# Chris10M/Lip2Speech

Measured on AMD Instinct MI355X. Metric: mel-frames/sec at LRW batch=32, 29-frame clips (Lip2Speech.inference, S=300), higher is better.
Workload: dtype f32; 1 GPU; LRW single-word, batch=32 per step, 29x96x96 RGB mouth crops, S=300 decode steps, speaker embedding supplied (encoding=voice), random-init weights; every step is one full pass over one B=32 batch; frames=29, decode_steps=300, library=libl2s_hip.so, parallelism=dp1 (clip sharding, no collective), batches_per_launch_chain=8, launch_chains_in_flight_per_gpu=3, distinct_batches_per_gpu=24, ranks=1

## Files before the change

### lip2speech_amd/csrc/encoder_kernels.hip

```cpp
#include "l2s_common.h"
#include <type_traits>

namespace l2s {

constexpr int FE_PR = 6;
constexpr int FE_CR = 2 * FE_PR + 1;
constexpr int FE_XROWS = 2 * (FE_CR - 1) + 7 + 1;
constexpr int FE_XLD = 104;
constexpr int FE_KP = 50;
constexpr int FE_CO = 24;

template <int HW, int MODE>
__global__ __launch_bounds__(256, 3) void frontend3d_kernel(const FrontendW w, const FrameSrc vsrc,
                                                            int T, float* __restrict__ out, float* __restrict__ zout) {
    constexpr bool SAVE_Z = MODE == 1;
    constexpr int H = HW, W = HW, Hc = H / 2, Wc = W / 2, Hp = Hc / 2, Wp = Wc / 2;
    constexpr int P = FE_CR * Wc;
    constexpr int NT = (P + 31) / 32;
    constexpr int TPW = (NT + 3) / 4;
    constexpr int XS = FE_XROWS * FE_XLD;
    constexpr int WS = FE_KP * 32;
    constexpr int CS = MODE == 2 ? 0 : P * (FE_CO / 2);
    constexpr int SMEM = (XS + WS) > CS ? (XS + WS) : CS;
    __shared__ __attribute__((aligned(16))) float smem[SMEM];
// ... 493 lines not shown
                        if ((nt == 0 && !on0) || (nt == 2 && !on1)) continue;
                        f32x4 a = acc[j][nt];
                        a = __builtin_amdgcn_mfma_f32_16x16x32_bf16(al, bh[nt], a, 0, 0, 0);
                        a = __builtin_amdgcn_mfma_f32_16x16x32_bf16(ah, bl[nt], a, 0, 0, 0);
                        a = __builtin_amdgcn_mfma_f32_16x16x32_bf16(am, bm[nt], a, 0, 0, 0);
                        a = __builtin_amdgcn_mfma_f32_16x16x32_bf16(am, bh[nt], a, 0, 0, 0);
                        a = __builtin_amdgcn_mfma_f32_16x16x32_bf16(ah, bm[nt], a, 0, 0, 0);
                        a = __builtin_amdgcn_mfma_f32_16x16x32_bf16(ah, bh[nt], a, 0, 0, 0);
                        acc[j][nt] = a;
                    }
                }
            }
        }
        sl = nxt; ++nslab;
    }
    __syncthreads();

    float* Cs = reinterpret_cast<float*>(smem);
    constexpr int CH = FE_CO / 2;
    float sc[3], sh[3], slp[3];
#pragma unroll
    for (int nt = 0; nt < 3; ++nt) {
        const int q = nt * 16 + li, ch = q >= FE_CO ? q - FE_CO : q;
        sc[nt] = w.scale[ch]; sh[nt] = w.shift[ch]; slp[nt] = w.slope[ch];
    }
    for (int pass = 0; pass < (has1 ? 4 : 2); ++pass) {
        const int o = pass >> 1, half = pass & 1;
#pragma unroll
        for (int nt = 0; nt < 3; ++nt) {
            const int q = nt * 16 + li, qo = q >= FE_CO ? 1 : 0, ch = q - FE_CO * qo;
            if (qo == o && ch >= half * CH && ch < (half + 1) * CH) {
#pragma unroll
                for (int j = 0; j < TPW; ++j) {
                    if (wave + 4 * j < PT) {
#pragma unroll
                        for (int r = 0; r < 4; ++r) {
                            const int p = (wave + 4 * j) * 16 + 4 * kg + r;
                            if (p < P) {
                                float v = acc[j][nt][r] * sc[nt] + sh[nt];
                                v = v >= 0.f ? v : slp[nt] * v;
                                Cs[p * CH + (ch - half * CH)] = v;
                            }
                        }
                    }
                }
            }
        }
        __syncthreads();
        const int f = bg * T + t0 + o;
        for (int i = tid; i < FE_PR * Wp * CH; i += 256) {
            const int ch = i % CH;
            const int pw = (i / CH) % Wp;
            const int prl = i / (CH * Wp);
            const int pr = p0 + prl;
            if (pr >= Hp) continue;
            float m = -INFINITY;
#pragma unroll
            for (int dr = 0; dr < 3; ++dr) {
                const int crow = 2 * pr - 1 + dr;
                if (crow < 0 || crow >= Hc) continue;
                const int lrow = 2 * prl + dr;
#pragma unroll
                for (int dc = -1; dc <= 1; ++dc) {
                    const int cc = 2 * pw + dc;
                    if (cc < 0 || cc >= Wc) continue;
                    m = fmaxf(m, Cs[(lrow * Wc + cc) * CH + ch]);
                }
            }
            out[(((int64_t)f * Hp + pr) * Wp + pw) * FE_CO + half * CH + ch] = m;
        }
        __syncthreads();
    }
}

template <int HW>
__global__ __launch_bounds__(256, 2) void frontend3d_x3q_kernel(const FrontendW w, const FrameSrc vsrc, int T, float* __restrict__ out) {
    const int NPAIR = (T + 1) / 2;
    const int bg = blockIdx.y / NPAIR, t0 = 2 * (blockIdx.y - bg * NPAIR);
    const bool has1 = t0 + 1 < T;
    const int grp = bg / vsrc.per, b = bg - grp * vsrc.per;
    const float* __restrict__ video = vsrc.p[grp];
#define FE_X3Q_PITCH T
#define FE_X3Q_FRAME0 (bg * T)
#include "frontend_x3q_block.inc"
#undef FE_X3Q_PITCH
#undef FE_X3Q_FRAME0
}

template <int HW>
__global__ __launch_bounds__(256, 2) void frontend3d_x3q_ragged_kernel(const FrontendW w, const FrameSrc vsrc, const RaggedClip* __restrict__ clips,
                                                                       const int* __restrict__ pair_clip, float* __restrict__ out) {
    const RaggedClip k = clips[pair_clip[blockIdx.y]];
    const int T = k.len;
    const int t0 = 2 * ((int)blockIdx.y - k.pair0);
    const bool has1 = t0 + 1 < T;
    const int b = k.row;
    const float* __restrict__ video = vsrc.p[0];
#pragma unroll
    for (int g = 1; g < MAX_GROUP; ++g) video = k.g == g ? vsrc.p[g] : video;
#define FE_X3Q_PITCH k.T
#define FE_X3Q_FRAME0 k.frame0
#include "frontend_x3q_block.inc"
#undef FE_X3Q_PITCH
#undef FE_X3Q_FRAME0
}

int launch_frontend(const FrontendW& w, const FrameSrc& video, int B, int T, int H, int W, float* out, hipStream_t s, float* zout) {
    L2S_REQUIRE(H == W && (H == 96 || H == 88), "frontend supports 96x96 and 88x88 mouth crops");
    L2S_REQUIRE(video.per >= 1 && (B + video.per - 1) / video.per <= MAX_GROUP, "too many frame tensors in one launch");
    for (int g = 0; g < (B + video.per - 1) / video.per; ++g)
        L2S_REQUIRE(video.p[g] && (reinterpret_cast<uintptr_t>(video.p[g]) & 15u) == 0, "video must be non-null and 16-byte aligned");
    const int Hp = H / 4;
    dim3 grid((Hp + FE_PR - 1) / FE_PR, B * T);
    ProfScope ps("frontend3d_conv_bn_prelu_pool", s);
    if (!zout && w.w1) {
        if (H == 96) hipLaunchKernelGGL((frontend3d_x3_kernel<96, 1>), grid, dim3(256), 0, s, w, video, T, out);
        else hipLaunchKernelGGL((frontend3d_x3_kernel<88, 1>), grid, dim3(256), 0, s, w, video, T, out);
    } else if (!zout && w.w3 && w.pair) {
        dim3 gp((Hp + FE_PR - 1) / FE_PR, B * ((T + 1) / 2));
        if (w.pipe) {
            const unsigned pad = w.solo ? 4096u : 0u;
            if (H == 96) hipLaunchKernelGGL((frontend3d_x3q_kernel<96>), gp, dim3(256), pad, s, w, video, T, out);
            else hipLaunchKernelGGL((frontend3d_x3q_kernel<88>), gp, dim3(256), pad, s, w, video, T, out);
        } else if (H == 96) hipLaunchKernelGGL((frontend3d_x3p_kernel<96>), gp, dim3(256), 0, s, w, video, T, out);
        else hipLaunchKernelGGL((frontend3d_x3p_kernel<88>), gp, dim3(256), 0, s, w, video, T, out);
    } else if (!zout && w.w3) {
        if (H == 96) hipLaunchKernelGGL((frontend3d_x3_kernel<96, 3>), grid, dim3(256), 0, s, w, video, T, out);
        else hipLaunchKernelGGL((frontend3d_x3_kernel<88, 3>), grid, dim3(256), 0, s, w, video, T, out);
    } else if (zout) {
        if (H == 96) hipLaunchKernelGGL((frontend3d_kernel<96, 1>), grid, dim3(256), 0, s, w, video, T, out, zout);
        else hipLaunchKernelGGL((frontend3d_kernel<88, 1>), grid, dim3(256), 0, s, w, video, T, out, zout);
    } else {
        if (H == 96) hipLaunchKernelGGL((frontend3d_kernel<96, 0>), grid, dim3(256), 0, s, w, video, T, out, zout);
        else hipLaunchKernelGGL((frontend3d_kernel<88, 0>), grid, dim3(256), 0, s, w, video, T, out, zout);
    }
    L2S_CHECK_HIP(hipGetLastError());
    return 0;
}

int launch_frontend_ragged(const FrontendW& w, const FrameSrc& video, const RaggedTab& rg, int H, int W, float* out, hipStream_t s) {
    L2S_REQUIRE(H == W && (H == 96 || H == 88), "frontend supports 96x96 and 88x88 mouth crops");
    L2S_REQUIRE(w.w3 && !w.w1 && w.pair && w.pipe && !w.solo, "the ragged front-end exists in the default form only (frontend_x3 = 3, no infer_bf16)");
    L2S_REQUIRE(rg.clips && rg.pair_clip && rg.NP >= 1 && rg.NF >= 1, "ragged front-end: empty table");
    const int Hp = H / 4;
    dim3 gp((Hp + FE_PR - 1) / FE_PR, rg.NP);
    prof_count("frontend3d_ragged_pair_blocks", rg.NP);
    ProfScope ps("frontend3d_conv_bn_prelu_pool_ragged", s);
    if (H == 96) hipLaunchKernelGGL((frontend3d_x3q_ragged_kernel<96>), gp, dim3(256), 0, s, w, video, rg.clips, rg.pair_clip, out);
    else hipLaunchKernelGGL((frontend3d_x3q_ragged_kernel<88>), gp, dim3(256), 0, s, w, video, rg.clips, rg.pair_clip, out);
    L2S_CHECK_HIP(hipGetLastError());
    return 0;
}

__global__ __launch_bounds__(256) void frontend_pool_kernel(const float* __restrict__ z, const float* __restrict__ slope, int NF, int Hc, int Wc, float* __restrict__ out) {
    const int Hp = Hc / 2, Wp = Wc / 2;
    const unsigned total = (unsigned)NF * Hp * Wp * FE_CO;
    for (unsigned idx = blockIdx.x * 256u + threadIdx.x; idx < total; idx += gridDim.x * 256u) {
        const int ch = idx % FE_CO;
        unsigned r = idx / FE_CO;
        const int pw = r % Wp; r /= Wp;
        const int pr = r % Hp;
        const unsigned f = r / Hp;
        const float sl = slope[ch];
        float m = -INFINITY;
#pragma unroll
        for (int dr = -1; dr <= 1; ++dr) {
            const int crow = 2 * pr + dr;
            if (crow < 0 || crow >= Hc) continue;
#pragma unroll
            for (int dc = -1; dc <= 1; ++dc) {
                const int cc = 2 * pw + dc;
                if (cc < 0 || cc >= Wc) continue;
                float v = z[((size_t)(f * Hc + crow) * Wc + cc) * FE_CO + ch];
                v = v >= 0.f ? v : sl * v;
                m = fmaxf(m, v);
            }
        }
        out[idx] = m;
    }
}
int launch_frontend_pool(const float* z, const float* slope, int NF, int Hc, int Wc, float* out, hipStream_t s) {
    const int64_t total = (int64_t)NF * (Hc / 2) * (Wc / 2) * FE_CO;
    L2S_REQUIRE(total < (int64_t)1 << 31, "front-end pool: map too large for 32-bit indexing");
    ProfScope ps("train_frontend_prelu_pool", s);
    hipLaunchKernelGGL(frontend_pool_kernel, dim3((unsigned)std::min<int64_t>((total + 255) / 256, 16384)), dim3(256), 0, s, z, slope, NF, Hc, Wc, out);
    L2S_CHECK_HIP(hipGetLastError());
    return 0;
}

int launch_frontend_stats(const FrontendW& w, const float* video1, int B, int T, int H, int W, float* partials, int* nblocks, hipStream_t s, float* raw_out) {
    L2S_REQUIRE(H == W && (H == 96 || H == 88), "frontend supports 96x96 and 88x88 mouth crops");
    FrameSrc video{}; video.p[0] = video1; video.per = B;
    const int Hp = H / 4;
    dim3 grid((Hp + FE_PR - 1) / FE_PR, B * T);
    *nblocks = (int)(grid.x * grid.y);
    ProfScope ps("train_frontend3d_stats", s);
    if (H == 96) hipLaunchKernelGGL((frontend3d_kernel<96, 2>), grid, dim3(256), 0, s, w, video, T, raw_out, partials);
    else hipLaunchKernelGGL((frontend3d_kernel<88, 2>), grid, dim3(256), 0, s, w, video, T, raw_out, partials);
    L2S_CHECK_HIP(hipGetLastError());
    return 0;
}

struct ClipTab { int64_t off[MAX_COLLATE_CLIPS]; int frames[MAX_COLLATE_CLIPS]; };

__global__ __launch_bounds__(256) void normalise_pad_kernel(const uint8_t* __restrict__ packed, const ClipTab tab, int b0, int T, int HW4,
                                                            float* __restrict__ video) {
    const int q = blockIdx.x * 256 + threadIdx.x, t = blockIdx.y, bl = blockIdx.z;
    if (q >= HW4) return;
    const int b = b0 + bl;
    const int64_t plane = (int64_t)HW4 * 4;
    float* out = video + (((int64_t)b * 3) * T + t) * plane + (int64_t)q * 4;
    float4 r = make_float4(0.f, 0.f, 0.f, 0.f), g = r, bl4 = r;
    if (t < tab.frames[bl]) {
        const uint32_t* src = reinterpret_cast<const uint32_t*>(packed + tab.off[bl] + ((int64_t)t * plane + (int64_t)q * 4) * 3);
        const uint32_t w0 = src[0], w1 = src[1], w2 = src[2];
        const float mean[3] = {0.485f, 0.456f, 0.406f}, stdv[3] = {0.229f, 0.224f, 0.225f};
        auto nrm = [&](uint32_t byte, int c) { return __fdiv_rn(__fsub_rn(__fdiv_rn((float)byte, 255.0f), mean[c]), stdv[c]); };
        r = make_float4(nrm(w0 & 255u, 0), nrm(w0 >> 24, 0), nrm((w1 >> 16) & 255u, 0), nrm((w2 >> 8) & 255u, 0));
        g = make_float4(nrm((w0 >> 8) & 255u, 1), nrm(w1 & 255u, 1), nrm(w1 >> 24, 1), nrm((w2 >> 16) & 255u, 1));
        bl4 = make_float4(nrm((w0 >> 16) & 255u, 2), nrm((w1 >> 8) & 255u, 2), nrm(w2 & 255u, 2), nrm(w2 >> 24, 2));
    }
    *reinterpret_cast<float4*>(out) = r;
    *reinterpret_cast<float4*>(out + (int64_t)T * plane) = g;
    *reinterpret_cast<float4*>(out + 2 * (int64_t)T * plane) = bl4;
}

int launch_normalise_pad(const uint8_t* packed, const int64_t* offsets, const int* frames, int B, int T, int H, int W, float* video, hipStream_t s) {
    L2S_REQUIRE((H * W) % 4 == 0 && (reinterpret_cast<uintptr_t>(packed) & 3u) == 0 && (reinterpret_cast<uintptr_t>(video) & 15u) == 0,
                "frames: H*W must be a multiple of 4, buffers aligned");
    const int HW4 = H * W / 4;
    ProfScope ps("normalise_pad_frames", s);
    for (int b0 = 0; b0 < B; b0 += MAX_COLLATE_CLIPS) {
        const int nb = B - b0 < MAX_COLLATE_CLIPS ? B - b0 : MAX_COLLATE_CLIPS;
        ClipTab tab{};
        for (int i = 0; i < nb; ++i) {
            L2S_REQUIRE(frames[b0 + i] >= 0 && frames[b0 + i] <= T && offsets[b0 + i] % 4 == 0, "clip table: 0 <= frames <= T, 4-byte aligned offsets");
            tab.off[i] = offsets[b0 + i]; tab.frames[i] = frames[b0 + i];
        }
        hipLaunchKernelGGL(normalise_pad_kernel, dim3((HW4 + 255) / 256, T, nb), dim3(256), 0, s, packed, tab, b0, T, HW4, video);
    }
    L2S_CHECK_HIP(hipGetLastError());
    return 0;
}

__global__ __launch_bounds__(256) void dwconv3x3_kernel(const float* __restrict__ in, int N, int Hi, int Wi, int ldi,
                                                        int ci_off, int C, int stride, const float* __restrict__ w9,
                                                        const float* __restrict__ scale, const float* __restrict__ shift,
                                                        float* __restrict__ out, int Ho, int Wo, int ldo, int co_off) {
    const int64_t total = (int64_t)N * Ho * Wo * C;
    for (int64_t idx = (int64_t)blockIdx.x * 256 + threadIdx.x; idx < total; idx += (int64_t)gridDim.x * 256) {
        const int c = idx % C;
        int64_t r = idx / C;
        const int ow = r % Wo;
        r /= Wo;
        const int oh = r % Ho;
        const int n = r / Ho;
        float acc = 0.f;
#pragma unroll
        for (int kh = 0; kh < 3; ++kh) {
            const int ih = oh * stride + kh - 1;
            if (ih < 0 || ih >= Hi) continue;
#pragma unroll
            for (int kw = 0; kw < 3; ++kw) {
                const int iw = ow * stride + kw - 1;
                if (iw < 0 || iw >= Wi) continue;
                acc = fmaf(in[(((int64_t)n * Hi + ih) * Wi + iw) * ldi + ci_off + c], w9[(kh * 3 + kw) * C + c], acc);
            }
        }
        out[(((int64_t)n * Ho + oh) * Wo + ow) * ldo + co_off + c] = acc * scale[c] + shift[c];
    }
}

int launch_dwconv(const float* in, int N, int Hi, int Wi, int ldi, int ci_off, int C, int stride, const float* w9,
                  const float* scale, const float* shift, float* out, int ldo, int co_off, hipStream_t s) {
    const int Ho = (Hi + 2 - 3) / stride + 1, Wo = (Wi + 2 - 3) / stride + 1;
    const int64_t total = (int64_t)N * Ho * Wo * C;
    int blocks = (int)((total + 255) / 256);
    if (blocks > 8192) blocks = 8192;
    ProfScope ps("dwconv3x3_bn", s);
    hipLaunchKernelGGL(dwconv3x3_kernel, dim3(blocks), dim3(256), 0, s, in, N, Hi, Wi, ldi, ci_off, C, stride, w9, scale,
                       shift, out, Ho, Wo, ldo, co_off);
    L2S_CHECK_HIP(hipGetLastError());
    return 0;
}


__device__ __forceinline__ f32x4 su_mfma4(const float4& a, const float4& w, f32x4 acc) {
    acc = __builtin_amdgcn_mfma_f32_16x16x4f32(a.x, w.x, acc, 0, 0, 0);
    acc = __builtin_amdgcn_mfma_f32_16x16x4f32(a.y, w.y, acc, 0, 0, 0);
    acc = __builtin_amdgcn_mfma_f32_16x16x4f32(a.z, w.z, acc, 0, 0, 0);
    acc = __builtin_amdgcn_mfma_f32_16x16x4f32(a.w, w.w, acc, 0, 0, 0);
    return acc;
}

constexpr int su_pad16(int v) { return (v + 15) / 16 * 16; }
constexpr int su_group(int mt) { return (mt + (mt + 4) / 5 - 1) / ((mt + 4) / 5); }

template <int N_, int NC_, int MT_>
struct SuGemm {
    static constexpr int N = N_, NC = NC_, MT = MT_, G = su_group(MT_);
    static constexpr int NT = (N + 15) / 16, MG = (MT + G - 1) / G, ITEMS = NT * MG, IT = (ITEMS + 7) / 8;
};

template <class GM, int LDA>
__device__ __forceinline__ void su_gemm(float* __restrict__ buf, const float* __restrict__ Wf,
                                        const float* __restrict__ scale, const float* __restrict__ shift) {
    constexpr int NC = GM::NC, G = GM::G, IT = GM::IT, NT = GM::NT;
    const int lane = threadIdx.x & 63;
    const int wave = __builtin_amdgcn_readfirstlane(threadIdx.x >> 6);
    const int li = lane & 15, lg = lane >> 4;
    f32x4 acc[IT][G];
#pragma unroll
    for (int it = 0; it < IT; ++it) {
        const int item = wave + 8 * it;
#pragma unroll
        for (int j = 0; j < G; ++j) acc[it][j] = {0.f, 0.f, 0.f, 0.f};
        if (item < GM::ITEMS) {
            const int nt = item % NT, mg = item / NT;
            const int mt0 = min(mg * G, GM::MT - G);
            const float4* wb = reinterpret_cast<const float4*>(Wf) + nt * (NC * 64) + lane;
            const float* ab = buf + (mt0 * 16 + li) * LDA + 4 * lg;
            float4 b4[NC];
#pragma unroll
            for (int c = 0; c < NC; ++c) b4[c] = wb[c * 64];
#pragma unroll
            for (int c = 0; c < NC; ++c) {
#pragma unroll
                for (int j = 0; j < G; ++j) {
                    const float4 a4 = *reinterpret_cast<const float4*>(ab + j * 16 * LDA + 16 * c);
                    acc[it][j] = su_mfma4(a4, b4[c], acc[it][j]);
                }
                __builtin_amdgcn_sched_barrier(0);
            }
        }
    }
    __syncthreads();
#pragma unroll
    for (int it = 0; it < IT; ++it) {
        const int item = wave + 8 * it;
        if (item < GM::ITEMS) {
            const int nt = item % NT, mg = item / NT;
            const int mt0 = min(mg * G, GM::MT - G);
            const int n = nt * 16 + li;
            if (n < GM::N) {
                const float sc = scale[n], sh = shift[n];
#pragma unroll
                for (int j = 0; j < G; ++j) {
#pragma unroll
                    for (int r = 0; r < 4; ++r) {
                        const float v = acc[it][j][r] * sc + sh;
                        buf[((mt0 + j) * 16 + 4 * lg + r) * LDA + n] = v > 0.f ? v : 0.f;
                    }
                }
            }
        }
    }
    __syncthreads();
}

template <int H, int HALF, int F>
struct S1Geo {
    static constexpr int HH = H * H, C = 2 * HALF, KP = su_pad16(HALF), LDA = KP + 4, PX = F * HH;
    static constexpr int MT = (PX + 15) / 16, ROWS = MT * 16, PPW = (PX + 7) / 8, CIT = (C + 63) / 64, CH = (HALF + 63) / 64;
    using GM = SuGemm<HALF, KP / 16, MT>;
    static constexpr size_t SMEM = (size_t)ROWS * LDA * sizeof(float);
};

#ifdef L2S_DIAG
static unsigned long long* g_su_ts = nullptr;
static int g_su_ts_h = 0;
void shuffle_set_timeline(unsigned long long* ts, int h) { g_su_ts = ts; g_su_ts_h = h; }
#endif
#define SU_STAMP(k) do { if (TIMED && threadIdx.x == 0) ts[blockIdx.x * 10 + (k)] = wall_clock64(); } while (0)

template <int H, int HALF, int F, bool TIMED>
__global__ __launch_bounds__(512, 4) void shuffle_s1_kernel(const ShuffleS1P p, unsigned long long* __restrict__ ts) {
    using Q = S1Geo<H, HALF, F>;
    constexpr int HH = Q::HH, C = Q::C, KP = Q::KP, LDA = Q::LDA, ROWS = Q::ROWS, PPW = Q::PPW, CIT = Q::CIT;
    extern __shared__ __attribute__((aligned(16))) float su_smem[];
    const int tid = threadIdx.x, lane = tid & 63;
    const int wave = __builtin_amdgcn_readfirstlane(tid >> 6);
    SU_STAMP(0);
    const int f0 = blockIdx.x * F;
    const int Mv = min(F, p.NF - f0) * HH;
    float* buf = su_smem;
    const float* xb = p.x + (int64_t)f0 * HH * C;
    float* ob = p.out + (int64_t)f0 * HH * C;

    const __amdgpu_buffer_rsrc_t rsrc = __builtin_amdgcn_make_buffer_rsrc(const_cast<float*>(xb), 0, Mv * C * 4, 0x00020000);
    int voff[CIT];
#pragma unroll
    for (int j = 0; j < CIT; ++j) voff[j] = (lane + 64 * j < C) ? (lane + 64 * j) * 4 : 0x7ffffff0;
    float xr[PPW][CIT];
#pragma unroll
    for (int i = 0; i < PPW; ++i) {
        const int soff = (wave + 8 * i) * C * 4;
#pragma unroll
        for (int j = 0; j < CIT; ++j)
            xr[i][j] = __builtin_bit_cast(float, __builtin_amdgcn_raw_buffer_load_b32(rsrc, voff[j], soff, 0));
    }
    if (KP > HALF) {
        for (int idx = tid; idx < ROWS * (KP - HALF); idx += 512) {
            const int m = idx / (KP - HALF), k = HALF + idx - m * (KP - HALF);
            buf[m * LDA + k] = 0.f;
        }
    }
    for (int idx = tid; idx < (ROWS - Mv) * HALF; idx += 512) {
        const int m = Mv + idx / HALF, k = idx - (m - Mv) * HALF;
        buf[m * LDA + k] = 0.f;
    }
#pragma unroll
    for (int i = 0; i < PPW; ++i) {
        const int m = wave + 8 * i;
#pragma unroll
        for (int j = 0; j < CIT; ++j) {
            const int c = lane + 64 * j;
            if (m < Mv && c >= HALF && c < C) buf[m * LDA + (c - HALF)] = xr[i][j];
        }
    }
    SU_STAMP(1);
    __syncthreads();
    SU_STAMP(2);
    su_gemm<typename Q::GM, LDA>(buf, p.w1f, p.s1, p.b1);
    SU_STAMP(3);
    constexpr bool PAIRS = HALF > 64;
    constexpr int NROW = F * H, RPW = (NROW + 7) / 8;
    typedef float su_f2 __attribute__((ext_vector_type(2)));
    using DV = std::conditional_t<PAIRS, su_f2, float>;
    constexpr int DW = PAIRS ? 2 : 1;
    constexpr int CHD = (HALF + 64 * DW - 1) / (64 * DW);
    DV dv[CHD][RPW][H];
    const DV zero = DV{};
#pragma unroll
    for (int jc = 0; jc < CHD; ++jc) {
        const int c = min(DW * lane + 64 * DW * jc, HALF - DW);
        DV wk[9];
#pragma unroll
        for (int t = 0; t < 9; ++t) wk[t] = *reinterpret_cast<const DV*>(p.wd + t * HALF + c);
        const DV sd = *reinterpret_cast<const DV*>(p.sd + c), bd = *reinterpret_cast<const DV*>(p.bd + c);
#pragma unroll
        for (int r = 0; r < RPW; ++r) {
            const int R = wave + 8 * r;
            if (R * H < Mv) {
                const int y = R % H;
                const bool up = y > 0, dn = y < H - 1;
                const float* rm = buf + (R * H) * LDA + c;
                const float* ru = rm - (up ? H * LDA : 0);
                const float* rd = rm + (dn ? H * LDA : 0);
                DV wu[3], wdn[3];
#pragma unroll
                for (int k = 0; k < 3; ++k) { wu[k] = up ? wk[k] : zero; wdn[k] = dn ? wk[6 + k] : zero; }
                DV a0 = zero, a1 = zero, a2 = zero;
                DV b0 = *reinterpret_cast<const DV*>(ru), b1 = *reinterpret_cast<const DV*>(rm), b2 = *reinterpret_cast<const DV*>(rd);
                DV c0 = zero, c1 = zero, c2 = zero;
                if constexpr (H > 1) { c0 = *reinterpret_cast<const DV*>(ru + LDA); c1 = *reinterpret_cast<const DV*>(rm + LDA); c2 = *reinterpret_cast<const DV*>(rd + LDA); }
#pragma unroll
                for (int x = 0; x < H; ++x) {
                    DV acc = zero;
                    if (x > 0) acc = __builtin_elementwise_fma(a0, wu[0], acc);
                    acc = __builtin_elementwise_fma(b0, wu[1], acc);
                    if (x < H - 1) acc = __builtin_elementwise_fma(c0, wu[2], acc);
                    if (x > 0) acc = __builtin_elementwise_fma(a1, wk[3], acc);
                    acc = __builtin_elementwise_fma(b1, wk[4], acc);
                    if (x < H - 1) acc = __builtin_elementwise_fma(c1, wk[5], acc);
                    if (x > 0) acc = __builtin_elementwise_fma(a2, wdn[0], acc);
                    acc = __builtin_elementwise_fma(b2, wdn[1], acc);
                    if (x < H - 1) acc = __builtin_elementwise_fma(c2, wdn[2], acc);
                    dv[jc][r][x] = acc * sd + bd;
                    a0 = b0; a1 = b1; a2 = b2; b0 = c0; b1 = c1; b2 = c2;
                    if (x + 2 < H) {
                        c0 = *reinterpret_cast<const DV*>(ru + (x + 2) * LDA); c1 = *reinterpret_cast<const DV*>(rm + (x + 2) * LDA);
                        c2 = *reinterpret_cast<const DV*>(rd + (x + 2) * LDA);
                    }
                }
            }
        }
    }
    SU_STAMP(4);
    __syncthreads();
#pragma unroll
    for (int jc = 0; jc < CHD; ++jc) {
        const int c = DW * lane + 64 * DW * jc;
#pragma unroll
        for (int r = 0; r < RPW; ++r) {
            const int R = wave + 8 * r;
            if (R * H < Mv && c < HALF) {
#pragma unroll
                for (int x = 0; x < H; ++x) *reinterpret_cast<DV*>(buf + (R * H + x) * LDA + c) = dv[jc][r][x];
            }
        }
    }
    __syncthreads();
    SU_STAMP(5);
    su_gemm<typename Q::GM, LDA>(buf, p.w2f, p.s2, p.b2);
    SU_STAMP(6);
#pragma unroll
    for (int i = 0; i < PPW; ++i) {
        const int m = wave + 8 * i;
#pragma unroll
        for (int j = 0; j < CIT; ++j) {
            const int c = lane + 64 * j;
            if (m < Mv && c < HALF) {
                float2 o;
                o.x = xr[i][j];
                o.y = buf[m * LDA + c];
                *reinterpret_cast<float2*>(ob + (int64_t)m * C + 2 * c) = o;
            }
        }
    }
    if (TIMED) {
        __builtin_amdgcn_s_waitcnt(0);
        SU_STAMP(7);
        unsigned hw;
        asm volatile("s_getreg_b32 %0, hwreg(HW_REG_HW_ID)" : "=s"(hw));
        unsigned xcc;
        asm volatile("s_getreg_b32 %0, hwreg(HW_REG_XCC_ID)" : "=s"(xcc));
        if (threadIdx.x == 0) { ts[blockIdx.x * 10 + 8] = hw; ts[blockIdx.x * 10 + 9] = xcc; }
    }
}

template <int H, int HALF, int F>
static int launch_s1_inst(const ShuffleS1P& p, hipStream_t s) {
    using Q = S1Geo<H, HALF, F>;
    static_assert(Q::SMEM <= 80 * 1024, "two blocks per CU");
    static bool attr_set = false;
    if (!attr_set) {
        L2S_CHECK_HIP(hipFuncSetAttribute(reinterpret_cast<const void*>(shuffle_s1_kernel<H, HALF, F, false>),
                                          hipFuncAttributeMaxDynamicSharedMemorySize, (int)Q::SMEM));
#ifdef L2S_DIAG
        L2S_CHECK_HIP(hipFuncSetAttribute(reinterpret_cast<const void*>(shuffle_s1_kernel<H, HALF, F, true>),
                                          hipFuncAttributeMaxDynamicSharedMemorySize, (int)Q::SMEM));
#endif
        attr_set = true;
    }
#ifdef L2S_DIAG
    if (g_su_ts && g_su_ts_h == H) hipLaunchKernelGGL((shuffle_s1_kernel<H, HALF, F, true>), dim3((p.NF + F - 1) / F), dim3(512), Q::SMEM, s, p, g_su_ts);
    else
#endif
    hipLaunchKernelGGL((shuffle_s1_kernel<H, HALF, F, false>), dim3((p.NF + F - 1) / F), dim3(512), Q::SMEM, s, p, (unsigned long long*)nullptr);
    return 0;
}

typedef __bf16 su_bf16x8 __attribute__((ext_vector_type(8)));
constexpr int su_pad32(int v) { return (v + 31) / 32 * 32; }
constexpr int su_pitch(int kp32) { return kp32 * 2 + 32; }
__device__ __forceinline__ void su_split2(float a, float b, unsigned& hi, unsigned& mid, unsigned& lo) {
    const unsigned xa = __float_as_uint(a), xb = __float_as_uint(b);
    const float ra = a - __uint_as_float(xa & 0xFFFF0000u), rb = b - __uint_as_float(xb & 0xFFFF0000u);
    const float qa = ra - __uint_as_float(__float_as_uint(ra) & 0xFFFF0000u), qb = rb - __uint_as_float(__float_as_uint(rb) & 0xFFFF0000u);
    hi = __builtin_amdgcn_perm(xb, xa, 0x07060302u);
    mid = __builtin_amdgcn_perm(__float_as_uint(rb), __float_as_uint(ra), 0x07060302u);
    lo = __builtin_amdgcn_perm(__float_as_uint(qb), __float_as_uint(qa), 0x07060302u);
}

__global__ __launch_bounds__(256) void su_planes_kernel(const float* __restrict__ W, int N, int K, int NT, int NCH, uint4* __restrict__ out) {
    const int idx = blockIdx.x * 256 + threadIdx.x;
    if (idx >= NT * NCH * 64) return;
    const int lane = idx & 63, ch = (idx >> 6) % NCH, nt = (idx >> 6) / NCH;
    const int n = nt * 16 + (lane & 15), k0 = ch * 32 + 8 * (lane >> 4);
    unsigned h[4], m[4], l[4];
#pragma unroll
    for (int e = 0; e < 4; ++e) {
        const int k = k0 + 2 * e;
        const float a = (n < N && k < K) ? W[(int64_t)n * K + k] : 0.f, b = (n < N && k + 1 < K) ? W[(int64_t)n * K + k + 1] : 0.f;
        su_split2(a, b, h[e], m[e], l[e]);
    }
    uint4* o = out + ((int64_t)(nt * NCH + ch) * 3) * 64 + lane;
    o[0] = make_uint4(h[0], h[1], h[2], h[3]);
    o[64] = make_uint4(m[0], m[1], m[2], m[3]);
    o[128] = make_uint4(l[0], l[1], l[2], l[3]);
}
int64_t su_planes_bytes(int N, int K) { return (int64_t)((N + 15) / 16) * (su_pad32(K) / 32) * 3 * 1024; }
int launch_su_planes(const float* W, int N, int K, void* out, hipStream_t s) {
    const int NT = (N + 15) / 16, NCH = su_pad32(K) / 32;
    ProfScope ps("shuffle_unit_weight_planes", s);
    hipLaunchKernelGGL(su_planes_kernel, dim3((NT * NCH * 64 + 255) / 256), dim3(256), 0, s, W, N, K, NT, NCH, reinterpret_cast<uint4*>(out));
    L2S_CHECK_HIP(hipGetLastError());
    return 0;
}

template <class GM, int NCH, int PITCH, int PLANE, int LDA, bool OPQ = false>
__device__ __forceinline__ void su_gemm_x3(unsigned char* __restrict__ pl, const uint4* __restrict__ Wp,
                                           const float* __restrict__ scale, const float* __restrict__ shift, int mrows = 1 << 30) {
    constexpr int G = GM::G, IT = GM::IT, NT = GM::NT, BD = NCH <= 4 ? NCH : 3;
    int tx = threadIdx.x;
    if constexpr (OPQ) asm volatile("" : "+v"(tx));
    const int lane = tx & 63;
    const int wave = __builtin_amdgcn_readfirstlane(threadIdx.x >> 6);
    const int li = lane & 15, lg = lane >> 4;
    float* const buf = reinterpret_cast<float*>(pl);
    f32x4 acc[IT][G];
#pragma unroll
    for (int it = 0; it < IT; ++it) {
        const int item = wave + 8 * it;
#pragma unroll
        for (int j = 0; j < G; ++j) acc[it][j] = {0.f, 0.f, 0.f, 0.f};
        if (item < GM::ITEMS) {
            const int nt = item % NT, mg = item / NT;
            const int mt0 = min(mg * G, GM::MT - G);
            const uint4* wb = Wp + (int64_t)nt * NCH * 192 + lane;
            const unsigned char* ab = pl + (mt0 * 16 + li) * PITCH + 16 * lg;
            uint4 b[BD][3];
#pragma unroll
            for (int c = 0; c < BD; ++c) {
#pragma unroll
                for (int q = 0; q < 3; ++q) b[c][q] = wb[(c * 3 + q) * 64];
            }
#pragma unroll
            for (int c = 0; c < NCH; ++c) {
                const int sl = c % BD;
                const su_bf16x8 bh = __builtin_bit_cast(su_bf16x8, b[sl][0]), bm = __builtin_bit_cast(su_bf16x8, b[sl][1]), bl = __builtin_bit_cast(su_bf16x8, b[sl][2]);
#pragma unroll
                for (int j = 0; j < G; ++j) {
                    const unsigned char* ap = ab + j * 16 * PITCH + 64 * c;
                    const su_bf16x8 ah = *reinterpret_cast<const su_bf16x8*>(ap), am = *reinterpret_cast<const su_bf16x8*>(ap + PLANE),
                                    al = *reinterpret_cast<const su_bf16x8*>(ap + 2 * PLANE);
                    f32x4 a = acc[it][j];
                    a = __builtin_amdgcn_mfma_f32_16x16x32_bf16(al, bh, a, 0, 0, 0);
                    a = __builtin_amdgcn_mfma_f32_16x16x32_bf16(ah, bl, a, 0, 0, 0);
                    a = __builtin_amdgcn_mfma_f32_16x16x32_bf16(am, bm, a, 0, 0, 0);
                    a = __builtin_amdgcn_mfma_f32_16x16x32_bf16(am, bh, a, 0, 0, 0);
                    a = __builtin_amdgcn_mfma_f32_16x16x32_bf16(ah, bm, a, 0, 0, 0);
                    a = __builtin_amdgcn_mfma_f32_16x16x32_bf16(ah, bh, a, 0, 0, 0);
                    acc[it][j] = a;
                }
                __builtin_amdgcn_sched_barrier(0);
                if (c + BD < NCH) {
#pragma unroll
                    for (int q = 0; q < 3; ++q) b[sl][q] = wb[((c + BD) * 3 + q) * 64];
                }
            }
        }
    }
    __syncthreads();
#pragma unroll
    for (int it = 0; it < IT; ++it) {
        const int item = wave + 8 * it;
        if (item < GM::ITEMS) {
            const int nt = item % NT, mg = item / NT;
            const int mt0 = min(mg * G, GM::MT - G);
            const int n = nt * 16 + li;
            if (n < GM::N) {
                const float sc = scale[n], sh = shift[n];
#pragma unroll
                for (int j = 0; j < G; ++j) {
#pragma unroll
                    for (int r = 0; r < 4; ++r) {
                        const float v = acc[it][j][r] * sc + sh;
                        const int row = (mt0 + j) * 16 + 4 * lg + r;
                        if (row < mrows) buf[row * LDA + n] = v > 0.f ? v : 0.f;
                    }
                }
            }
        }
    }
    __syncthreads();
}

template <int H, int HALF, int F>
struct S1XGeo {
    static constexpr int HH = H * H, C = 2 * HALF, KP = su_pad16(HALF), LDA = KP + 4, PX = F * HH;
    static constexpr int MT = (PX + 15) / 16, ROWS = MT * 16;
    static constexpr int KP32 = su_pad32(HALF), NCH = KP32 / 32, PITCH = su_pitch(KP32), PLANE = ROWS * PITCH;
    static constexpr int NPAIR = HALF / 2, KPAIR = KP32 / 2;
    static constexpr int PPI = KPAIR <= 32 ? 2 : 1;
    static constexpr int QIT = PPI == 2 ? 1 : KPAIR / 64, PPW = (PX + 8 * PPI - 1) / (8 * PPI);
    using GM = SuGemm<HALF, KP / 16, MT>;
    static constexpr size_t SMEM = 3 * (size_t)PLANE > (size_t)ROWS * LDA * 4 ? 3 * (size_t)PLANE : (size_t)ROWS * LDA * 4;
    static_assert(HALF % 2 == 0 && (PPI == 2 || KPAIR % 64 == 0), "channel pairs; a pixel's pairs fill whole wave instructions");
};

template <int H, int HALF, int F, bool TIMED>
__global__ __launch_bounds__(512, 4) void shuffle_s1x_kernel(const ShuffleS1P p, unsigned long long* __restrict__ ts) {
    using Q = S1XGeo<H, HALF, F>;
    constexpr int HH = Q::HH, C = Q::C, LDA = Q::LDA, PPW = Q::PPW, QIT = Q::QIT, PPI = Q::PPI, PITCH = Q::PITCH, PLANE = Q::PLANE;
    extern __shared__ __attribute__((aligned(16))) float su_smem[];
    const int tid = threadIdx.x, lane = tid & 63;
    const int wave = __builtin_amdgcn_readfirstlane(tid >> 6);
    SU_STAMP(0);
    const int f0 = blockIdx.x * F;
    const int Mv = min(F, p.NF - f0) * HH;
    float* buf = su_smem;
    unsigned char* const pl = reinterpret_cast<unsigned char*>(su_smem);
    const float* xb = p.x + (int64_t)f0 * HH * C;
    float* ob = p.out + (int64_t)f0 * HH * C;

    const __amdgpu_buffer_rsrc_t rsrc = __builtin_amdgcn_make_buffer_rsrc(const_cast<float*>(xb), 0, Mv * C * 4, 0x00020000);
    const int sub = PPI == 2 ? lane >> 5 : 0;
    typedef unsigned su_u2 __attribute__((ext_vector_type(2)));
    float2 xr[PPW][QIT];
    su_u2 br[PPW][QIT];
#pragma unroll
    for (int i = 0; i < PPW; ++i) {
        const int soff = (wave + 8 * i) * PPI * C * 4;
#pragma unroll
        for (int j = 0; j < QIT; ++j) {
            const int q = PPI == 2 ? (lane & 31) : lane + 64 * j;
            const int voff = q < Q::NPAIR ? (sub * C + 2 * q) * 4 : 0x7ffffff0;
            const su_u2 a = __builtin_amdgcn_raw_buffer_load_b64(rsrc, voff, soff, 0);
            br[i][j] = __builtin_amdgcn_raw_buffer_load_b64(rsrc, q < Q::NPAIR ? voff + HALF * 4 : 0x7ffffff0, soff, 0);
            xr[i][j] = make_float2(__uint_as_float(a.x), __uint_as_float(a.y));
        }
    }
#pragma unroll
    for (int i = 0; i < PPW; ++i) {
        const int m = (wave + 8 * i) * PPI + sub;
#pragma unroll
        for (int j = 0; j < QIT; ++j) {
            const int q = PPI == 2 ? (lane & 31) : lane + 64 * j;
            unsigned hi, mid, lo;
            su_split2(__uint_as_float(br[i][j].x), __uint_as_float(br[i][j].y), hi, mid, lo);
            if (m < Q::ROWS) {
                unsigned* d = reinterpret_cast<unsigned*>(pl + m * PITCH + q * 4);
                d[0] = hi; d[PLANE / 4] = mid; d[2 * (PLANE / 4)] = lo;
            }
        }
    }
    SU_STAMP(1);
    __syncthreads();
    SU_STAMP(2);
    su_gemm_x3<typename Q::GM, Q::NCH, PITCH, PLANE, LDA>(pl, reinterpret_cast<const uint4*>(p.w1p), p.s1, p.b1);
    SU_STAMP(3);
    constexpr bool PAIRS = HALF > 64;
    constexpr int NROW = F * H, RPW = (NROW + 7) / 8;
    typedef float su_f2 __attribute__((ext_vector_type(2)));
    using DV = std::conditional_t<PAIRS, su_f2, float>;
    constexpr int DW = PAIRS ? 2 : 1;
    constexpr int CHD = Q::KP32 / (64 * DW);
    DV dv[CHD][RPW][H];
    const DV zero = DV{};
#pragma unroll
    for (int jc = 0; jc < CHD; ++jc) {
        const int c = min(DW * lane + 64 * DW * jc, HALF - DW);
        DV wk[9];
#pragma unroll
        for (int t = 0; t < 9; ++t) wk[t] = *reinterpret_cast<const DV*>(p.wd + t * HALF + c);
        const DV sd = *reinterpret_cast<const DV*>(p.sd + c), bd = *reinterpret_cast<const DV*>(p.bd + c);
#pragma unroll
        for (int r = 0; r < RPW; ++r) {
            const int R = wave + 8 * r;
            if (R * H < Mv) {
                const int y = R % H;
                const bool up = y > 0, dn = y < H - 1;
                const float* rm = buf + (R * H) * LDA + c;
                const float* ru = rm - (up ? H * LDA : 0);
                const float* rd = rm + (dn ? H * LDA : 0);
                DV wu[3], wdn[3];
#pragma unroll
                for (int k = 0; k < 3; ++k) { wu[k] = up ? wk[k] : zero; wdn[k] = dn ? wk[6 + k] : zero; }
                DV a0 = zero, a1 = zero, a2 = zero;
                DV b0 = *reinterpret_cast<const DV*>(ru), b1 = *reinterpret_cast<const DV*>(rm), b2 = *reinterpret_cast<const DV*>(rd);
                DV c0 = zero, c1 = zero, c2 = zero;
                if constexpr (H > 1) { c0 = *reinterpret_cast<const DV*>(ru + LDA); c1 = *reinterpret_cast<const DV*>(rm + LDA); c2 = *reinterpret_cast<const DV*>(rd + LDA); }
#pragma unroll
                for (int x = 0; x < H; ++x) {
                    DV acc = zero;
                    if (x > 0) acc = __builtin_elementwise_fma(a0, wu[0], acc);
                    acc = __builtin_elementwise_fma(b0, wu[1], acc);
                    if (x < H - 1) acc = __builtin_elementwise_fma(c0, wu[2], acc);
                    if (x > 0) acc = __builtin_elementwise_fma(a1, wk[3], acc);
                    acc = __builtin_elementwise_fma(b1, wk[4], acc);
                    if (x < H - 1) acc = __builtin_elementwise_fma(c1, wk[5], acc);
                    if (x > 0) acc = __builtin_elementwise_fma(a2, wdn[0], acc);
                    acc = __builtin_elementwise_fma(b2, wdn[1], acc);
                    if (x < H - 1) acc = __builtin_elementwise_fma(c2, wdn[2], acc);
                    dv[jc][r][x] = acc * sd + bd;
                    a0 = b0; a1 = b1; a2 = b2; b0 = c0; b1 = c1; b2 = c2;
                    if (x + 2 < H) {
                        c0 = *reinterpret_cast<const DV*>(ru + (x + 2) * LDA); c1 = *reinterpret_cast<const DV*>(rm + (x + 2) * LDA);
                        c2 = *reinterpret_cast<const DV*>(rd + (x + 2) * LDA);
                    }
                }
            }
        }
    }
    SU_STAMP(4);
    __syncthreads();
#pragma unroll
    for (int jc = 0; jc < CHD; ++jc) {
        const int c = DW * lane + 64 * DW * jc;
#pragma unroll
        for (int r = 0; r < RPW; ++r) {
            const int R = wave + 8 * r;
            if (R * H < Mv) {
#pragma unroll
                for (int x = 0; x < H; ++x) {
                    unsigned char* d = pl + (R * H + x) * PITCH + c * 2;
                    if constexpr (PAIRS) {
                        unsigned hi, mid, lo;
                        su_split2(c < HALF ? dv[jc][r][x][0] : 0.f, c < HALF ? dv[jc][r][x][1] : 0.f, hi, mid, lo);
                        *reinterpret_cast<unsigned*>(d) = hi; *reinterpret_cast<unsigned*>(d + PLANE) = mid; *reinterpret_cast<unsigned*>(d + 2 * PLANE) = lo;
                    } else {
                        const float v = c < HALF ? dv[jc][r][x] : 0.f;
                        const float r1 = v - __uint_as_float(__float_as_uint(v) & 0xFFFF0000u);
                        const float r2 = r1 - __uint_as_float(__float_as_uint(r1) & 0xFFFF0000u);
                        *reinterpret_cast<unsigned short*>(d) = (unsigned short)(__float_as_uint(v) >> 16);
                        *reinterpret_cast<unsigned short*>(d + PLANE) = (unsigned short)(__float_as_uint(r1) >> 16);
                        *reinterpret_cast<unsigned short*>(d + 2 * PLANE) = (unsigned short)(__float_as_uint(r2) >> 16);
                    }
                }
            }
        }
    }
    __syncthreads();
    SU_STAMP(5);
    su_gemm_x3<typename Q::GM, Q::NCH, PITCH, PLANE, LDA>(pl, reinterpret_cast<const uint4*>(p.w2p), p.s2, p.b2);
    SU_STAMP(6);
#pragma unroll
    for (int i = 0; i < PPW; ++i) {
        const int m = (wave + 8 * i) * PPI + sub;
#pragma unroll
        for (int j = 0; j < QIT; ++j) {
            const int q = PPI == 2 ? (lane & 31) : lane + 64 * j;
            if (m < Mv && q < Q::NPAIR) {
                const float2 bv = *reinterpret_cast<const float2*>(buf + m * LDA + 2 * q);
                *reinterpret_cast<float4*>(ob + (int64_t)m * C + 4 * q) = make_float4(xr[i][j].x, bv.x, xr[i][j].y, bv.y);
            }
        }
    }
    if (TIMED) {
        __builtin_amdgcn_s_waitcnt(0);
        SU_STAMP(7);
        unsigned hw;
        asm volatile("s_getreg_b32 %0, hwreg(HW_REG_HW_ID)" : "=s"(hw));
        unsigned xcc;
        asm volatile("s_getreg_b32 %0, hwreg(HW_REG_XCC_ID)" : "=s"(xcc));
        if (threadIdx.x == 0) { ts[blockIdx.x * 10 + 8] = hw; ts[blockIdx.x * 10 + 9] = xcc; }
    }
}

template <int H, int HALF, int F>
static int launch_s1x_inst(const ShuffleS1P& p, hipStream_t s) {
    using Q = S1XGeo<H, HALF, F>;
    static_assert(Q::SMEM <= 80 * 1024, "two blocks per CU");
    static bool attr_set = false;
    if (!attr_set) {
        L2S_CHECK_HIP(hipFuncSetAttribute(reinterpret_cast<const void*>(shuffle_s1x_kernel<H, HALF, F, false>),
                                          hipFuncAttributeMaxDynamicSharedMemorySize, (int)Q::SMEM));
#ifdef L2S_DIAG
        L2S_CHECK_HIP(hipFuncSetAttribute(reinterpret_cast<const void*>(shuffle_s1x_kernel<H, HALF, F, true>),
                                          hipFuncAttributeMaxDynamicSharedMemorySize, (int)Q::SMEM));
#endif
        attr_set = true;
    }
#ifdef L2S_DIAG
    if (g_su_ts && g_su_ts_h == H) hipLaunchKernelGGL((shuffle_s1x_kernel<H, HALF, F, true>), dim3((p.NF + F - 1) / F), dim3(512), Q::SMEM, s, p, g_su_ts);
    else
#endif
    hipLaunchKernelGGL((shuffle_s1x_kernel<H, HALF, F, false>), dim3((p.NF + F - 1) / F), dim3(512), Q::SMEM, s, p, (unsigned long long*)nullptr);
    return 0;
}

struct S1UnitW {
    const void* w1p; const float* s1; const float* b1;
    const float* wd; const float* sd; const float* bd;
    const void* w2p; const float* s2; const float* b2;
};
struct ShuffleS1ChainP {
    const float* x; float* out;
    int NF, n;
    S1UnitW u[S1_CHAIN_MAX];
};

template <int H, int HALF, int F>
__global__ __launch_bounds__(512, 4) void shuffle_s1xc_kernel(const ShuffleS1ChainP p) {
    using Q = S1XGeo<H, HALF, F>;
    constexpr int HH = Q::HH, C = Q::C, LDA = Q::LDA, PPW = Q::PPW, QIT = Q::QIT, PPI = Q::PPI, PITCH = Q::PITCH, PLANE = Q::PLANE;
    static_assert(HALF % 2 == 0 && (Q::KPAIR - Q::NPAIR) <= 32, "a lane's four output channels are two whole pairs; the K padding is at most 32 pairs");
    extern __shared__ __attribute__((aligned(16))) float su_smem[];
    const int tid = threadIdx.x, lane = tid & 63;
    const int wave = __builtin_amdgcn_readfirstlane(tid >> 6);
    const int f0 = blockIdx.x * F;
    const int Mv = min(F, p.NF - f0) * HH;
    float* buf = su_smem;
    unsigned char* const pl = reinterpret_cast<unsigned char*>(su_smem);
    const float* xb = p.x + (int64_t)f0 * HH * C;
    float* ob = p.out + (int64_t)f0 * HH * C;
    const int nu = p.n;

    const __amdgpu_buffer_rsrc_t rsrc = __builtin_amdgcn_make_buffer_rsrc(const_cast<float*>(xb), 0, Mv * C * 4, 0x00020000);
    const int sub = PPI == 2 ? lane >> 5 : 0;
    typedef unsigned su_u2 __attribute__((ext_vector_type(2)));
    float2 xr[PPW][QIT];
    {
        su_u2 br[PPW][QIT];
#pragma unroll
        for (int i = 0; i < PPW; ++i) {
            const int soff = (wave + 8 * i) * PPI * C * 4;
#pragma unroll
            for (int j = 0; j < QIT; ++j) {
                const int q = PPI == 2 ? (lane & 31) : lane + 64 * j;
                const int voff = q < Q::NPAIR ? (sub * C + 2 * q) * 4 : 0x7ffffff0;
                const su_u2 a = __builtin_amdgcn_raw_buffer_load_b64(rsrc, voff, soff, 0);
                br[i][j] = __builtin_amdgcn_raw_buffer_load_b64(rsrc, q < Q::NPAIR ? voff + HALF * 4 : 0x7ffffff0, soff, 0);
                xr[i][j] = make_float2(__uint_as_float(a.x), __uint_as_float(a.y));
            }
        }
#pragma unroll
        for (int i = 0; i < PPW; ++i) {
            const int m = (wave + 8 * i) * PPI + sub;
#pragma unroll
            for (int j = 0; j < QIT; ++j) {
                const int q = PPI == 2 ? (lane & 31) : lane + 64 * j;
                unsigned hi, mid, lo;
                su_split2(__uint_as_float(br[i][j].x), __uint_as_float(br[i][j].y), hi, mid, lo);
                if (m < Q::ROWS) {
                    unsigned* d = reinterpret_cast<unsigned*>(pl + m * PITCH + q * 4);
                    d[0] = hi; d[PLANE / 4] = mid; d[2 * (PLANE / 4)] = lo;
                }
            }
        }
    }
    __syncthreads();

    for (int u = 0; u < nu; ++u) {
        const S1UnitW& U = p.u[u];
        const void* const w1p = U.w1p; const float* const s1 = U.s1; const float* const b1 = U.b1;
        const float* const wd = U.wd; const float* const sdp = U.sd; const float* const bdp = U.bd;
        const void* const w2p = U.w2p; const float* const s2 = U.s2; const float* const b2 = U.b2;
        su_gemm_x3<typename Q::GM, Q::NCH, PITCH, PLANE, LDA, true>(pl, reinterpret_cast<const uint4*>(w1p), s1, b1);
        {
            constexpr bool PAIRS = HALF > 64;
            constexpr int NROW = F * H, RPW = (NROW + 7) / 8;
            typedef float su_f2 __attribute__((ext_vector_type(2)));
            using DV = std::conditional_t<PAIRS, su_f2, float>;
            constexpr int DW = PAIRS ? 2 : 1;
            constexpr int CHD = Q::KP32 / (64 * DW);
            DV dv[CHD][RPW][H];
            const DV zero = DV{};
            int lane_d = lane;
            asm volatile("" : "+v"(lane_d));
#pragma unroll
            for (int jc = 0; jc < CHD; ++jc) {
                const int c = min(DW * lane_d + 64 * DW * jc, HALF - DW);
                DV wk[9];
#pragma unroll
                for (int t = 0; t < 9; ++t) wk[t] = *reinterpret_cast<const DV*>(wd + t * HALF + c);
                const DV sd = *reinterpret_cast<const DV*>(sdp + c), bd = *reinterpret_cast<const DV*>(bdp + c);
#pragma unroll
                for (int r = 0; r < RPW; ++r) {
                    const int R = wave + 8 * r;
                    if (R * H < Mv) {
                        const int y = R % H;
                        const bool up = y > 0, dn = y < H - 1;
                        const float* rm = buf + (R * H) * LDA + c;
                        const float* ru = rm - (up ? H * LDA : 0);
                        const float* rd = rm + (dn ? H * LDA : 0);
                        DV wu[3], wdn[3];
#pragma unroll
                        for (int k = 0; k < 3; ++k) { wu[k] = up ? wk[k] : zero; wdn[k] = dn ? wk[6 + k] : zero; }
                        DV a0 = zero, a1 = zero, a2 = zero;
                        DV b0 = *reinterpret_cast<const DV*>(ru), b1v = *reinterpret_cast<const DV*>(rm), b2v = *reinterpret_cast<const DV*>(rd);
                        DV c0 = zero, c1 = zero, c2 = zero;
                        if constexpr (H > 1) { c0 = *reinterpret_cast<const DV*>(ru + LDA); c1 = *reinterpret_cast<const DV*>(rm + LDA); c2 = *reinterpret_cast<const DV*>(rd + LDA); }
#pragma unroll
                        for (int x = 0; x < H; ++x) {
                            DV acc = zero;
                            if (x > 0) acc = __builtin_elementwise_fma(a0, wu[0], acc);
                            acc = __builtin_elementwise_fma(b0, wu[1], acc);
                            if (x < H - 1) acc = __builtin_elementwise_fma(c0, wu[2], acc);
                            if (x > 0) acc = __builtin_elementwise_fma(a1, wk[3], acc);
                            acc = __builtin_elementwise_fma(b1v, wk[4], acc);
                            if (x < H - 1) acc = __builtin_elementwise_fma(c1, wk[5], acc);
                            if (x > 0) acc = __builtin_elementwise_fma(a2, wdn[0], acc);
                            acc = __builtin_elementwise_fma(b2v, wdn[1], acc);
                            if (x < H - 1) acc = __builtin_elementwise_fma(c2, wdn[2], acc);
                            dv[jc][r][x] = acc * sd + bd;
                            a0 = b0; a1 = b1v; a2 = b2v; b0 = c0; b1v = c1; b2v = c2;
                            if (x + 2 < H) {
                                c0 = *reinterpret_cast<const DV*>(ru + (x + 2) * LDA); c1 = *reinterpret_cast<const DV*>(rm + (x + 2) * LDA);
                                c2 = *reinterpret_cast<const DV*>(rd + (x + 2) * LDA);
                            }
                        }
                    }
                }
            }
            __syncthreads();
#pragma unroll
            for (int jc = 0; jc < CHD; ++jc) {
                const int c = DW * lane_d + 64 * DW * jc;
#pragma unroll
                for (int r = 0; r < RPW; ++r) {
                    const int R = wave + 8 * r;
                    if (R * H < Mv) {
#pragma unroll
                        for (int x = 0; x < H; ++x) {
                            unsigned char* d = pl + (R * H + x) * PITCH + c * 2;
                            if constexpr (PAIRS) {
                                unsigned hi, mid, lo;
                                su_split2(c < HALF ? dv[jc][r][x][0] : 0.f, c < HALF ? dv[jc][r][x][1] : 0.f, hi, mid, lo);
                                *reinterpret_cast<unsigned*>(d) = hi; *reinterpret_cast<unsigned*>(d + PLANE) = mid; *reinterpret_cast<unsigned*>(d + 2 * PLANE) = lo;
                            } else {
                                const float v = c < HALF ? dv[jc][r][x] : 0.f;
                                const float r1 = v - __uint_as_float(__float_as_uint(v) & 0xFFFF0000u);
                                const float r2 = r1 - __uint_as_float(__float_as_uint(r1) & 0xFFFF0000u);
                                *reinterpret_cast<unsigned short*>(d) = (unsigned short)(__float_as_uint(v) >> 16);
                                *reinterpret_cast<unsigned short*>(d + PLANE) = (unsigned short)(__float_as_uint(r1) >> 16);
                                *reinterpret_cast<unsigned short*>(d + 2 * PLANE) = (unsigned short)(__float_as_uint(r2) >> 16);
                            }
                        }
                    }
                }
            }
            __syncthreads();
        }
        su_gemm_x3<typename Q::GM, Q::NCH, PITCH, PLANE, LDA, true>(pl, reinterpret_cast<const uint4*>(w2p), s2, b2);
        if (u + 1 == nu) {
#pragma unroll
            for (int i = 0; i < PPW; ++i) {
                const int m = (wave + 8 * i) * PPI + sub;
#pragma unroll
                for (int j = 0; j < QIT; ++j) {
                    const int q = PPI == 2 ? (lane & 31) : lane + 64 * j;
                    if (m < Mv && q < Q::NPAIR) {
                        const float2 bv = *reinterpret_cast<const float2*>(buf + m * LDA + 2 * q);
                        *reinterpret_cast<float4*>(ob + (int64_t)m * C + 4 * q) = make_float4(xr[i][j].x, bv.x, xr[i][j].y, bv.y);
                    }
                }
            }
        } else {
            int lane_v = lane;
            asm volatile("" : "+v"(lane_v));
            const int sub_v = PPI == 2 ? lane_v >> 5 : 0;
            float2 bv[PPW][QIT];
#pragma unroll
            for (int i = 0; i < PPW; ++i) {
                const int m = (wave + 8 * i) * PPI + sub_v;
#pragma unroll
                for (int j = 0; j < QIT; ++j) {
                    const int q = PPI == 2 ? (lane_v & 31) : lane_v + 64 * j;
                    bv[i][j] = make_float2(0.f, 0.f);
                    if (m < Q::ROWS && q < Q::NPAIR) bv[i][j] = *reinterpret_cast<const float2*>(buf + m * LDA + 2 * q);
                }
            }
            __syncthreads();
#pragma unroll
            for (int i = 0; i < PPW; ++i) {
                const int m = (wave + 8 * i) * PPI + sub_v;
#pragma unroll
                for (int j = 0; j < QIT; ++j) {
                    const int q = PPI == 2 ? (lane_v & 31) : lane_v + 64 * j;
                    if (m < Q::ROWS && q < Q::NPAIR) {
#pragma unroll
                        for (int e = 0; e < 2; ++e) {
                            const int c = 4 * q + 2 * e;
                            if (c >= HALF) {
                                unsigned hi, mid, lo;
                                su_split2(e ? xr[i][j].y : xr[i][j].x, e ? bv[i][j].y : bv[i][j].x, hi, mid, lo);
                                unsigned* d = reinterpret_cast<unsigned*>(pl + m * PITCH + (c - HALF) * 2);
                                d[0] = hi; d[PLANE / 4] = mid; d[2 * (PLANE / 4)] = lo;
                            }
                        }
                    }
                    if (j == 0 && m < Q::ROWS && q < Q::KPAIR - Q::NPAIR) {
                        unsigned* d = reinterpret_cast<unsigned*>(pl + m * PITCH + (Q::NPAIR + q) * 4);
                        d[0] = 0u; d[PLANE / 4] = 0u; d[2 * (PLANE / 4)] = 0u;
                    }
                }
                float2 nx[QIT];
#pragma unroll
                for (int j = 0; j < QIT; ++j) {
                    const int q = PPI == 2 ? (lane_v & 31) : lane_v + 64 * j;
                    const int srcq = q >> 1;
                    const int src = PPI == 2 ? ((lane_v & 32) | srcq) : srcq;
                    const float ex = __shfl(xr[i][0].x, src), ey = __shfl(bv[i][0].x, src), ez = __shfl(xr[i][0].y, src), ew = __shfl(bv[i][0].y, src);
                    nx[j] = (q & 1) ? make_float2(ez, ew) : make_float2(ex, ey);
                }
#pragma unroll
                for (int j = 0; j < QIT; ++j) xr[i][j] = nx[j];
            }
            __syncthreads();
        }
    }
}

template <int H, int HALF, int F>
static int launch_s1xc_inst(const ShuffleS1ChainP& p, hipStream_t s) {
    using Q = S1XGeo<H, HALF, F>;
    static_assert(Q::SMEM <= 80 * 1024, "two blocks per CU");
    static bool attr_set = false;
    if (!attr_set) {
        L2S_CHECK_HIP(hipFuncSetAttribute(reinterpret_cast<const void*>(shuffle_s1xc_kernel<H, HALF, F>), hipFuncAttributeMaxDynamicSharedMemorySize, (int)Q::SMEM));
        attr_set = true;
    }
    hipLaunchKernelGGL((shuffle_s1xc_kernel<H, HALF, F>), dim3((p.NF + F - 1) / F), dim3(512), Q::SMEM, s, p);
    return 0;
}

int launch_shuffle_s1_chain(const ShuffleS1P* units, int n, hipStream_t s) {
    L2S_REQUIRE(n >= 1 && n <= S1_CHAIN_MAX, "shuffle_s1 chain: 1..7 units");
    ShuffleS1ChainP c{};
    c.x = units[0].x; c.out = units[n - 1].out; c.NF = units[0].NF; c.n = n;
    const int h = units[0].h, half = units[0].half;
    for (int i = 0; i < n; ++i) {
        const ShuffleS1P& p = units[i];
        L2S_REQUIRE(p.w1p && p.w2p && p.h == h && p.half == half && p.NF == c.NF && p.Kpad == su_pad16(p.half), "shuffle_s1 chain: units of one stage with operand planes");
        c.u[i] = S1UnitW{p.w1p, p.s1, p.b1, p.wd, p.sd, p.bd, p.w2p, p.s2, p.b2};
    }
    ProfScope ps(h >= 11 ? "shuffle_stage_s1_chain_h12" : h == 6 ? "shuffle_stage_s1_chain_h6" : "shuffle_stage_s1_chain_h3", s);
    int rc = 1;
    if (h == 12 && half == 58) rc = launch_s1xc_inst<12, 58, 1>(c, s);
    else if (h == 11 && half == 58) rc = launch_s1xc_inst<11, 58, 1>(c, s);
    else if (h == 6 && half == 116) rc = launch_s1xc_inst<6, 116, 2>(c, s);
    else if (h == 3 && half == 232) rc = c.NF >= 2048 ? launch_s1xc_inst<3, 232, 5>(c, s) : launch_s1xc_inst<3, 232, 2>(c, s);
    else set_error("shuffle_s1 chain: unsupported unit geometry");
    if (rc) return 1;
    L2S_CHECK_HIP(hipGetLastError());
    return 0;
}

int launch_shuffle_s1(const ShuffleS1P& p, hipStream_t s) {
    L2S_REQUIRE(p.Kpad == su_pad16(p.half), "shuffle_s1: weight fragments are packed for K = pad16(half)");
    ProfScope ps(p.h >= 11 ? "shuffle_unit_s1_fused_h12" : p.h == 6 ? "shuffle_unit_s1_fused_h6" : "shuffle_unit_s1_fused_h3", s);
    int rc = 1;
    if (p.w1p && p.w2p) {
        if (p.h == 12 && p.half == 58) rc = launch_s1x_inst<12, 58, 1>(p, s);
        else if (p.h == 11 && p.half == 58) rc = launch_s1x_inst<11, 58, 1>(p, s);
        else if (p.h == 6 && p.half == 116) rc = launch_s1x_inst<6, 116, 2>(p, s);
        else if (p.h == 3 && p.half == 232) rc = p.NF >= 2048 ? launch_s1x_inst<3, 232, 5>(p, s) : launch_s1x_inst<3, 232, 2>(p, s);
        else set_error("shuffle_s1: unsupported unit geometry");
    }
    else if (p.h == 12 && p.half == 58) rc = launch_s1_inst<12, 58, 1>(p, s);
    else if (p.h == 11 && p.half == 58) rc = launch_s1_inst<11, 58, 1>(p, s);
    else if (p.h == 6 && p.half == 116) rc = launch_s1_inst<6, 116, 2>(p, s);
    else if (p.h == 3 && p.half == 232) rc = p.NF >= 2048 ? launch_s1_inst<3, 232, 5>(p, s) : launch_s1_inst<3, 232, 2>(p, s);
    else set_error("shuffle_s1: unsupported unit geometry");
    if (rc) return 1;
    L2S_CHECK_HIP(hipGetLastError());
    return 0;
}

template <int H, int CIN, int HALF, int RO>
struct S2Geo {
    static constexpr int HO = (H + 1) / 2, KIN = su_pad16(CIN), KH = su_pad16(HALF), LDA = (KIN > KH ? KIN : KH) + 4;
    static constexpr int RIN = 2 * RO + 1, MTI = (RIN * H + 15) / 16, MTO = (RO * HO + 15) / 16, STRIPS = (HO + RO - 1) / RO;
    using G1 = SuGemm<HALF, KIN / 16, MTI>;
    using G2 = SuGemm<HALF, KIN / 16, MTO>;
    using G3 = SuGemm<HALF, KH / 16, MTO>;
    static constexpr size_t SMEM = (size_t)(MTI + 2 * MTO) * 16 * LDA * sizeof(float);
    static_assert(CIN % 4 == 0 && CIN <= HALF, "float4 tile rows; pw1 runs in place over the input tile");
};

template <int H, int HO, int LDA, int CN, int PITCH = 0, int PLANE = 0>
__device__ __forceinline__ void su_dw_s2(const float* __restrict__ src, float* __restrict__ dst, int iy0, int outv,
                                         const float* __restrict__ w9, const float* __restrict__ sc, const float* __restrict__ sh) {
    const int lane = threadIdx.x & 63;
    const int wave = __builtin_amdgcn_readfirstlane(threadIdx.x >> 6);
    if constexpr (CN > 64) {
        typedef float su_f2 __attribute__((ext_vector_type(2)));
        static_assert(CN % 2 == 0 && LDA % 2 == 0, "channel pairs");
#pragma unroll
        for (int jc = 0; jc < (CN + 127) / 128; ++jc) {
            const int c = 2 * lane + 128 * jc;
            if (c < CN) {
                su_f2 wk[9];
#pragma unroll
                for (int t = 0; t < 9; ++t) wk[t] = *reinterpret_cast<const su_f2*>(w9 + t * CN + c);
                const su_f2 s = *reinterpret_cast<const su_f2*>(sc + c), b = *reinterpret_cast<const su_f2*>(sh + c);
                const su_f2 zero2 = {0.f, 0.f};
                for (int m = wave; m < outv; m += 8) {
                    const int oyl = m / HO, ox = m - oyl * HO;
                    su_f2 acc = zero2;
#pragma unroll
                    for (int ky = 0; ky < 3; ++ky) {
#pragma unroll
                        for (int kx = 0; kx < 3; ++kx) {
                            const int r = 2 * oyl + ky, iy = iy0 + r, ix = 2 * ox + kx - 1;
                            const bool in = (unsigned)iy < (unsigned)H && (unsigned)ix < (unsigned)H;
                            const su_f2 v = *reinterpret_cast<const su_f2*>(src + (in ? r * H + ix : (2 * oyl + 1) * H + 2 * ox) * LDA + c);
                            acc = __builtin_elementwise_fma(v, in ? wk[ky * 3 + kx] : zero2, acc);
                        }
                    }
                    const su_f2 o = acc * s + b;
                    if constexpr (PITCH > 0) {
                        unsigned hi, mid, lo;
                        su_split2(o[0], o[1], hi, mid, lo);
                        unsigned char* d = reinterpret_cast<unsigned char*>(dst) + m * PITCH + c * 2;
                        *reinterpret_cast<unsigned*>(d) = hi; *reinterpret_cast<unsigned*>(d + PLANE) = mid; *reinterpret_cast<unsigned*>(d + 2 * PLANE) = lo;
                    } else {
                        *reinterpret_cast<su_f2*>(dst + m * LDA + c) = o;
                    }
                }
            }
        }
        return;
    }
#pragma unroll
    for (int jc = 0; jc < (CN + 63) / 64; ++jc) {
        const int c = lane + 64 * jc;
        if (c < CN) {
            float wk[9];
#pragma unroll
            for (int t = 0; t < 9; ++t) wk[t] = w9[t * CN + c];
            const float s = sc[c], b = sh[c];
            for (int m = wave; m < outv; m += 8) {
                const int oyl = m / HO, ox = m - oyl * HO;
                float acc = 0.f;
#pragma unroll
                for (int ky = 0; ky < 3; ++ky) {
#pragma unroll
                    for (int kx = 0; kx < 3; ++kx) {
                        const int r = 2 * oyl + ky, iy = iy0 + r, ix = 2 * ox + kx - 1;
                        const bool in = (unsigned)iy < (unsigned)H && (unsigned)ix < (unsigned)H;
                        acc = fmaf(src[(in ? r * H + ix : (2 * oyl + 1) * H + 2 * ox) * LDA + c], in ? wk[ky * 3 + kx] : 0.f, acc);
                    }
                }
                const float o = acc * s + b;
                if constexpr (PITCH > 0) {
                    const float r1 = o - __uint_as_float(__float_as_uint(o) & 0xFFFF0000u);
                    const float r2 = r1 - __uint_as_float(__float_as_uint(r1) & 0xFFFF0000u);
                    unsigned char* d = reinterpret_cast<unsigned char*>(dst) + m * PITCH + c * 2;
                    *reinterpret_cast<unsigned short*>(d) = (unsigned short)(__float_as_uint(o) >> 16);
                    *reinterpret_cast<unsigned short*>(d + PLANE) = (unsigned short)(__float_as_uint(r1) >> 16);
                    *reinterpret_cast<unsigned short*>(d + 2 * PLANE) = (unsigned short)(__float_as_uint(r2) >> 16);
                } else {
                    dst[m * LDA + c] = o;
                }
            }
        }
    }
}

#define S2_STAMP(k) do { if (TIMED && threadIdx.x == 0) ts[(blockIdx.y * gridDim.x + blockIdx.x) * 10 + (k)] = wall_clock64(); } while (0)
template <int H, int CIN, int HALF, int RO, bool TIMED>
__global__ __launch_bounds__(512, 4) void shuffle_s2_kernel(const ShuffleS2P p, unsigned long long* __restrict__ ts) {
    using Q = S2Geo<H, CIN, HALF, RO>;
    constexpr int HO = Q::HO, KIN = Q::KIN, KH = Q::KH, LDA = Q::LDA, MTI = Q::MTI, MTO = Q::MTO, CIN4 = CIN / 4;
    extern __shared__ __attribute__((aligned(16))) float su_smem[];
    const int tid = threadIdx.x, lane = tid & 63;
    const int wave = __builtin_amdgcn_readfirstlane(tid >> 6);
    const int f = blockIdx.y;
    const int oy0 = blockIdx.x * RO;
    const int ro = min(RO, HO - oy0);
    const int iy0 = 2 * oy0 - 1;
    const int outv = ro * HO;
    float* X = su_smem;
    float* D1 = X + MTI * 16 * LDA;
    float* D2 = D1 + MTO * 16 * LDA;
    S2_STAMP(0);

    const int iy_lo = max(iy0, 0), iy_hi = min(iy0 + 2 * ro + 1, H);
    const int n4 = (iy_hi - iy_lo) * (H * CIN4);
    const float4* src4 = reinterpret_cast<const float4*>(p.x + ((int64_t)f * H + iy_lo) * (H * CIN));
    float* xt = X + (iy_lo - iy0) * (H * LDA);
    constexpr int NLD = (Q::RIN * H * CIN4 + 511) / 512;
    float4 xin[NLD];
#pragma unroll
    for (int i = 0; i < NLD; ++i) {
        const int idx = tid + 512 * i;
        xin[i] = idx < n4 ? src4[idx] : make_float4(0.f, 0.f, 0.f, 0.f);
    }
#pragma unroll
    for (int i = 0; i < NLD; ++i) {
        const int idx = tid + 512 * i;
        if (idx < n4) {
            const int px = idx / CIN4, c4 = idx - px * CIN4;
            *reinterpret_cast<float4*>(xt + px * LDA + 4 * c4) = xin[i];
        }
    }
    if (KIN > CIN) {
        for (int idx = tid; idx < (MTI + MTO) * 16 * (KIN - CIN); idx += 512) {
            const int m = idx / (KIN - CIN), k = CIN + idx - m * (KIN - CIN);
            X[m * LDA + k] = 0.f;
        }
    }
    if (KH > HALF) {
        for (int idx = tid; idx < MTO * 16 * (KH - HALF); idx += 512) {
            const int m = idx / (KH - HALF), k = HALF + idx - m * (KH - HALF);
            D2[m * LDA + k] = 0.f;
        }
    }
    S2_STAMP(1);
    __syncthreads();
    S2_STAMP(2);
    su_dw_s2<H, HO, LDA, CIN>(X, D1, iy0, outv, p.wd1, p.sd1, p.bd1);
    S2_STAMP(3);
    su_gemm<typename Q::G1, LDA>(X, p.w1f, p.s1, p.b1);
    S2_STAMP(4);
    su_dw_s2<H, HO, LDA, HALF>(X, D2, iy0, outv, p.wd, p.sd, p.bd);
    __syncthreads();
    S2_STAMP(5);
    su_gemm<typename Q::G2, LDA>(D1, p.wb1f, p.sb1, p.bb1);
    S2_STAMP(6);
    su_gemm<typename Q::G3, LDA>(D2, p.w2f, p.s2, p.b2);
    S2_STAMP(7);
    float* ob = p.out + ((int64_t)f * HO + oy0) * (HO * 2 * HALF);
    for (int m = wave; m < outv; m += 8) {
#pragma unroll
        for (int jc = 0; jc < (HALF + 63) / 64; ++jc) {
            const int c = lane + 64 * jc;
            if (c < HALF) {
                float2 o;
                o.x = D1[m * LDA + c];
                o.y = D2[m * LDA + c];
                *reinterpret_cast<float2*>(ob + m * (2 * HALF) + 2 * c) = o;
            }
        }
    }
    if (TIMED) { __builtin_amdgcn_s_waitcnt(0); S2_STAMP(8); }
}

template <int H, int CIN, int HALF, int RO>
struct S2XGeo {
    using B = S2Geo<H, CIN, HALF, RO>;
    static constexpr int HO = B::HO, LDA = B::LDA, MTI = B::MTI, MTO = B::MTO, RX = B::RIN * H;
    static constexpr int KI32 = su_pad32(CIN), KH32 = su_pad32(HALF), PIN = su_pitch(KI32), PH = su_pitch(KH32);
    static constexpr int RV = RO * HO;
    static constexpr int XPLANE = RX * PIN, D1PLANE = RV * PIN, D2PLANE = RV * PH;
    static constexpr int XBYTES = 3 * XPLANE > MTI * 16 * LDA * 4 ? 3 * XPLANE : MTI * 16 * LDA * 4;
    static constexpr int TAIL = (MTO * 16 - RV) * PIN + 16;
    static constexpr size_t SMEM = (size_t)XBYTES + 3 * D2PLANE + 3 * D1PLANE + TAIL;
    static_assert(3 * D1PLANE >= RV * LDA * 4 && 3 * D2PLANE >= RV * LDA * 4, "a GEMM's fp32 rows fit in place of its operand planes");
    static_assert(XBYTES % 16 == 0 && D1PLANE % 16 == 0 && D2PLANE % 16 == 0 && TAIL % 16 == 0, "16-byte aligned regions");
    using G1 = SuGemm<HALF, 1, MTI>;
    using G2 = SuGemm<HALF, 1, MTO>;
};

template <int H, int CIN, int HALF, int RO, bool TIMED>
__global__ __launch_bounds__(512, 4) void shuffle_s2x_kernel(const ShuffleS2P p, unsigned long long* __restrict__ ts) {
    using Q = S2XGeo<H, CIN, HALF, RO>;
    constexpr int HO = Q::HO, LDA = Q::LDA, CIN4 = CIN / 4, PIN = Q::PIN, PH = Q::PH;
    extern __shared__ __attribute__((aligned(16))) float su_smem[];
    const int tid = threadIdx.x, lane = tid & 63;
    const int wave = __builtin_amdgcn_readfirstlane(tid >> 6);
    const int f = blockIdx.y;
    const int oy0 = blockIdx.x * RO;
    const int ro = min(RO, HO - oy0);
    const int iy0 = 2 * oy0 - 1;
    const int outv = ro * HO;
    float* X = su_smem;
    unsigned char* const XP = reinterpret_cast<unsigned char*>(su_smem);
    unsigned char* const D2P = XP + Q::XBYTES;
    unsigned char* const D1P = D2P + 3 * Q::D2PLANE;
    float* D1 = reinterpret_cast<float*>(D1P);
    float* D2 = reinterpret_cast<float*>(D2P);
    S2_STAMP(0);

    const int iy_lo = max(iy0, 0), iy_hi = min(iy0 + 2 * ro + 1, H);
    const int n4 = (iy_hi - iy_lo) * (H * CIN4);
    const int row0 = (iy_lo - iy0) * H;
    const float4* src4 = reinterpret_cast<const float4*>(p.x + ((int64_t)f * H + iy_lo) * (H * CIN));
    float* xt = X + row0 * LDA;
    constexpr int NLD = (Q::RX * CIN4 + 511) / 512;
    float4 xin[NLD];
#pragma unroll
    for (int i = 0; i < NLD; ++i) {
        const int idx = tid + 512 * i;
        xin[i] = idx < n4 ? src4[idx] : make_float4(0.f, 0.f, 0.f, 0.f);
    }
    for (int idx = tid; idx < (3 * Q::D1PLANE + 3 * Q::D2PLANE + Q::TAIL) / 16; idx += 512) reinterpret_cast<uint4*>(D2P)[idx] = make_uint4(0u, 0u, 0u, 0u);
#pragma unroll
    for (int i = 0; i < NLD; ++i) {
        const int idx = tid + 512 * i;
        if (idx < n4) {
            const int px = idx / CIN4, c4 = idx - px * CIN4;
            *reinterpret_cast<float4*>(xt + px * LDA + 4 * c4) = xin[i];
        }
    }
    S2_STAMP(1);
    __syncthreads();
    S2_STAMP(2);
    su_dw_s2<H, HO, LDA, CIN, PIN, Q::D1PLANE>(X, D1, iy0, outv, p.wd1, p.sd1, p.bd1);
    __syncthreads();
#pragma unroll
    for (int i = 0; i < NLD; ++i) {
        const int idx = tid + 512 * i;
        if (idx < n4) {
            const int px = idx / CIN4, c4 = idx - px * CIN4;
            unsigned h0, m0, l0, h1, m1, l1;
            su_split2(xin[i].x, xin[i].y, h0, m0, l0);
            su_split2(xin[i].z, xin[i].w, h1, m1, l1);
            unsigned char* d = XP + (row0 + px) * PIN + c4 * 8;
            *reinterpret_cast<uint2*>(d) = make_uint2(h0, h1);
            *reinterpret_cast<uint2*>(d + Q::XPLANE) = make_uint2(m0, m1);
            *reinterpret_cast<uint2*>(d + 2 * Q::XPLANE) = make_uint2(l0, l1);
        }
    }
    if constexpr (Q::KI32 > CIN) {
        constexpr int PS = (Q::KI32 - CIN) / 4;
        for (int idx = tid; idx < Q::RX * PS; idx += 512) {
            const int m = idx / PS, k4 = idx - m * PS;
            unsigned char* d = XP + m * PIN + (CIN4 + k4) * 8;
            *reinterpret_cast<uint2*>(d) = make_uint2(0u, 0u);
            *reinterpret_cast<uint2*>(d + Q::XPLANE) = make_uint2(0u, 0u);
            *reinterpret_cast<uint2*>(d + 2 * Q::XPLANE) = make_uint2(0u, 0u);
        }
    }
    S2_STAMP(3);
    __syncthreads();
    su_gemm_x3<typename Q::G1, Q::KI32 / 32, PIN, Q::XPLANE, LDA>(XP, reinterpret_cast<const uint4*>(p.w1p), p.s1, p.b1);
    S2_STAMP(4);
    su_dw_s2<H, HO, LDA, HALF, PH, Q::D2PLANE>(X, D2, iy0, outv, p.wd, p.sd, p.bd);
    __syncthreads();
    S2_STAMP(5);
    su_gemm_x3<typename Q::G2, Q::KI32 / 32, PIN, Q::D1PLANE, LDA>(D1P, reinterpret_cast<const uint4*>(p.wb1p), p.sb1, p.bb1, Q::RV);
    S2_STAMP(6);
    su_gemm_x3<typename Q::G2, Q::KH32 / 32, PH, Q::D2PLANE, LDA>(D2P, reinterpret_cast<const uint4*>(p.w2p), p.s2, p.b2, Q::RV);
    S2_STAMP(7);
    float* ob = p.out + ((int64_t)f * HO + oy0) * (HO * 2 * HALF);
    for (int m = wave; m < outv; m += 8) {
#pragma unroll
        for (int jc = 0; jc < (HALF + 63) / 64; ++jc) {
            const int c = lane + 64 * jc;
            if (c < HALF) {
                float2 o;
                o.x = D1[m * LDA + c];
                o.y = D2[m * LDA + c];
                *reinterpret_cast<float2*>(ob + m * (2 * HALF) + 2 * c) = o;
            }
        }
    }
    if (TIMED) { __builtin_amdgcn_s_waitcnt(0); S2_STAMP(8); }
}

template <int H, int CIN, int HALF, int RO>
static int launch_s2x_inst(const ShuffleS2P& p, hipStream_t s) {
    using Q = S2XGeo<H, CIN, HALF, RO>;
    static_assert(Q::SMEM <= 80 * 1024, "two blocks per CU");
    static bool attr_set = false;
    if (!attr_set) {
        L2S_CHECK_HIP(hipFuncSetAttribute(reinterpret_cast<const void*>(shuffle_s2x_kernel<H, CIN, HALF, RO, false>),
                                          hipFuncAttributeMaxDynamicSharedMemorySize, (int)Q::SMEM));
#ifdef L2S_DIAG
        L2S_CHECK_HIP(hipFuncSetAttribute(reinterpret_cast<const void*>(shuffle_s2x_kernel<H, CIN, HALF, RO, true>),
                                          hipFuncAttributeMaxDynamicSharedMemorySize, (int)Q::SMEM));
#endif
        attr_set = true;
    }
#ifdef L2S_DIAG
    if (g_su_ts && g_su_ts_h == -H) hipLaunchKernelGGL((shuffle_s2x_kernel<H, CIN, HALF, RO, true>), dim3(Q::B::STRIPS, p.NF), dim3(512), Q::SMEM, s, p, g_su_ts);
    else
#endif
    hipLaunchKernelGGL((shuffle_s2x_kernel<H, CIN, HALF, RO, false>), dim3(Q::B::STRIPS, p.NF), dim3(512), Q::SMEM, s, p, (unsigned long long*)nullptr);
    return 0;
}

template <int H, int CIN, int HALF, int RO>
static int launch_s2_inst(const ShuffleS2P& p, hipStream_t s) {
    using Q = S2Geo<H, CIN, HALF, RO>;
    static_assert(Q::SMEM <= 80 * 1024, "two blocks per CU");
    static bool attr_set = false;
    if (!attr_set) {
        L2S_CHECK_HIP(hipFuncSetAttribute(reinterpret_cast<const void*>(shuffle_s2_kernel<H, CIN, HALF, RO, false>),
                                          hipFuncAttributeMaxDynamicSharedMemorySize, (int)Q::SMEM));
#ifdef L2S_DIAG
        L2S_CHECK_HIP(hipFuncSetAttribute(reinterpret_cast<const void*>(shuffle_s2_kernel<H, CIN, HALF, RO, true>),
                                          hipFuncAttributeMaxDynamicSharedMemorySize, (int)Q::SMEM));
#endif
        attr_set = true;
    }
#ifdef L2S_DIAG
    if (g_su_ts && g_su_ts_h == -H) hipLaunchKernelGGL((shuffle_s2_kernel<H, CIN, HALF, RO, true>), dim3(Q::STRIPS, p.NF), dim3(512), Q::SMEM, s, p, g_su_ts);
    else
#endif
    hipLaunchKernelGGL((shuffle_s2_kernel<H, CIN, HALF, RO, false>), dim3(Q::STRIPS, p.NF), dim3(512), Q::SMEM, s, p, (unsigned long long*)nullptr);
    return 0;
}

int launch_shuffle_s2(const ShuffleS2P& p, hipStream_t s) {
    L2S_REQUIRE(p.Kin == su_pad16(p.cin) && p.Kh == su_pad16(p.half) && p.ho == (p.h + 1) / 2, "shuffle_s2: fragment packing / geometry mismatch");
    L2S_REQUIRE((reinterpret_cast<uintptr_t>(p.x) & 15u) == 0, "shuffle_s2 input must be 16-byte aligned");
    ProfScope ps(p.cin == 24 ? "shuffle_unit_s2_fused_st2" : p.cin == 116 ? "shuffle_unit_s2_fused_st3" : "shuffle_unit_s2_fused_st4", s);
    int rc = 1;
    const bool x3 = p.w1p && p.w2p && p.wb1p && p.cin != 232;
    if (x3 && p.h == 24 && p.cin == 24 && p.half == 58) rc = launch_s2x_inst<24, 24, 58, 2>(p, s);
    else if (x3 && p.h == 22 && p.cin == 24 && p.half == 58) rc = launch_s2x_inst<22, 24, 58, 2>(p, s);
    else if (x3 && p.h == 12 && p.cin == 116 && p.half == 116) rc = launch_s2x_inst<12, 116, 116, 2>(p, s);
    else if (x3 && p.h == 11 && p.cin == 116 && p.half == 116) rc = launch_s2x_inst<11, 116, 116, 2>(p, s);
    else if (p.h == 24 && p.cin == 24 && p.half == 58) rc = launch_s2_inst<24, 24, 58, 2>(p, s);
    else if (p.h == 22 && p.cin == 24 && p.half == 58) rc = launch_s2_inst<22, 24, 58, 2>(p, s);
    else if (p.h == 12 && p.cin == 116 && p.half == 116) rc = launch_s2_inst<12, 116, 116, 2>(p, s);
    else if (p.h == 11 && p.cin == 116 && p.half == 116) rc = launch_s2_inst<11, 116, 116, 2>(p, s);
    else if (p.h == 6 && p.cin == 232 && p.half == 232) rc = launch_s2_inst<6, 232, 232, 3>(p, s);
    else set_error("shuffle_s2: unsupported unit geometry");
    if (rc) return 1;
    L2S_CHECK_HIP(hipGetLastError());
    return 0;
}

__global__ __launch_bounds__(256) void copy_cols_kernel(const float* __restrict__ in, int ldi, int off_i,
                                                        float* __restrict__ out, int ldo, int off_o, int cs_o,
                                                        int64_t rows, int cols) {
    const int64_t total = rows * cols;
    for (int64_t idx = (int64_t)blockIdx.x * 256 + threadIdx.x; idx < total; idx += (int64_t)gridDim.x * 256) {
        const int c = idx % cols;
        const int64_t r = idx / cols;
        out[r * ldo + off_o + (int64_t)c * cs_o] = in[r * ldi + off_i + c];
    }
}

int launch_copy_cols(const float* in, int ldi, int off_i, float* out, int ldo, int off_o, int cs_o, int64_t rows,
                     int cols, hipStream_t s) {
    const int64_t total = rows * cols;
    int blocks = (int)((total + 255) / 256);
    if (blocks > 8192) blocks = 8192;
    if (blocks < 1) blocks = 1;
    ProfScope ps("copy_cols", s);
    hipLaunchKernelGGL(copy_cols_kernel, dim3(blocks), dim3(256), 0, s, in, ldi, off_i, out, ldo, off_o, cs_o, rows, cols);
    L2S_CHECK_HIP(hipGetLastError());
    return 0;
}

__device__ __forceinline__ void pool_norm_cat_frame(const float* __restrict__ x, int P, int C, const float* __restrict__ emb, int E, int b, int fin, int fout,
                                                    float* __restrict__ vis, int ldv, float* __restrict__ feat) {
    const int tid = threadIdx.x;
    __shared__ float red[4];
    float vals[4];
    float ss = 0.f;
    int cnt = 0;
    for (int c = tid; c < C; c += 256, ++cnt) {
        float acc = 0.f;
        for (int p = 0; p < P; ++p) acc += x[((int64_t)fin * P + p) * C + c];
        acc = acc / (float)P;
        vals[cnt] = acc;
        ss += acc * acc;
    }
#pragma unroll
    for (int o = 32; o > 0; o >>= 1) ss += __shfl_xor(ss, o);
    if ((tid & 63) == 0) red[tid >> 6] = ss;
    __syncthreads();
    const float tot = red[0] + red[1] + red[2] + red[3];
    const float denom = fmaxf(sqrtf(tot), 1e-12f);
    cnt = 0;
    for (int c = tid; c < C; c += 256, ++cnt) {
        const float v = vals[cnt] / denom;
        if (vis) vis[(int64_t)fout * ldv + c] = v;
        if (feat) feat[(int64_t)fout * C + c] = v;
    }
    if (vis && emb)
        for (int e = tid; e < E; e += 256) vis[(int64_t)fout * ldv + C + e] = emb[(int64_t)b * E + e];
}

__global__ __launch_bounds__(256) void pool_norm_cat_kernel(const float* __restrict__ x, int P, int C,
                                                            const float* __restrict__ emb, int E, int T,
                                                            float* __restrict__ vis, int ldv, float* __restrict__ feat) {
    const int f = blockIdx.x;
    pool_norm_cat_frame(x, P, C, emb, E, f / T, f, f, vis, ldv, feat);
}

__global__ __launch_bounds__(256) void pool_norm_cat_ragged_kernel(const float* __restrict__ x, const RaggedClip* __restrict__ clips, int Tmax, int P, int C,
                                                                   const float* __restrict__ emb, int E, float* __restrict__ vis, int ldv) {
    const int row = blockIdx.x, c = row / Tmax, t = row - c * Tmax;
    const RaggedClip k = clips[c];
    if (t < k.len) {
        pool_norm_cat_frame(x, P, C, emb, E, c, k.frame0 + t, row, vis, ldv, nullptr);
    } else {
        for (int i = threadIdx.x; i < ldv; i += 256) vis[(int64_t)row * ldv + i] = 0.f;
    }
}

int launch_pool_norm_cat(const float* x, int NF, int P, int C, const float* emb, int E, int T, float* vis, int ldv,
                         float* feat, hipStream_t s) {
    L2S_REQUIRE(C <= 1024, "pool_norm_cat: C <= 1024");
    ProfScope ps("avgpool_l2norm_cat", s);
    hipLaunchKernelGGL(pool_norm_cat_kernel, dim3(NF), dim3(256), 0, s, x, P, C, emb, E, T, vis, ldv, feat);
    L2S_CHECK_HIP(hipGetLastError());
    return 0;
}

int launch_pool_norm_cat_ragged(const float* x, const RaggedTab& rg, int P, int C, const float* emb, int E, float* vis, int ldv, hipStream_t s) {
    L2S_REQUIRE(C <= 1024 && C + E <= ldv && x && emb && vis && rg.clips, "pool_norm_cat (ragged): bad arguments");
    ProfScope ps("avgpool_l2norm_cat_ragged", s);
    hipLaunchKernelGGL(pool_norm_cat_ragged_kernel, dim3(rg.N * rg.Tmax), dim3(256), 0, s, x, rg.clips, rg.Tmax, P, C, emb, E, vis, ldv);
    L2S_CHECK_HIP(hipGetLastError());
    return 0;
}

}
```

### lip2speech_amd/csrc/l2s_api.hip

```cpp
#include "../../include/l2s.h"
#ifdef L2S_DIAG
#include "../../include/l2s_diag.h"
#endif
#include "l2s_common.h"
#include "l2s_model.h"
#include "pdecode.h"

#include <algorithm>
#include <cmath>
#include <cstdio>
#include <cstdlib>
#ifdef L2S_DIAG
#include <cxxabi.h>
#include <dlfcn.h>
#endif
#include <functional>
#include <cstring>
#include <map>
#include <memory>
#include <mutex>
#include <string>
#include <unordered_map>
#include <vector>

namespace l2s {

static thread_local std::string g_err;
void set_error(const std::string& msg) { g_err = msg; }

static Options g_default_opt;
int set_option_field(Options& o, const char* name, int value) {
    struct Row { const char* name; int Options::*field; };
    static const Row product[] = {
        {"persist_decode", &Options::persist}, {"use_graph", &Options::graph}, {"fold_step_weights", &Options::fold}, {"refresh_map", &Options::refresh_map},
        {"infer_bf16", &Options::infer_bf16}, {"train_bf16", &Options::train_bf16}, {"gemm_x3", &Options::gemm_x3}, {"frontend_x3", &Options::frontend_x3},
        {"trunk_x3", &Options::trunk_x3}, {"lstm_x3", &Options::lstm_x3}, {"early_stop", &Options::early_stop},
        {"persist_frames", &Options::persist_frames}, {"persist_masked", &Options::persist_masked}};
    for (auto& t : product)
        if (!std::strcmp(name, t.name)) { o.*(t.field) = value; return 0; }
#ifdef L2S_DIAG
    static const Row diag[] = {
        {"overlap_postnet", &Options::overlap_postnet}, {"fuse_trunk", &Options::fuse_trunk}, {"fuse_s2", &Options::fuse_s2},
        {"skinny_static", &Options::skinny_static}, {"skinny_sized", &Options::skinny_sized}, {"skinny_split", &Options::skinny_split},
        {"skinny_split8", &Options::skinny_split8}, {"skinny_rc", &Options::rc_shape}, {"skinny_rc_jb", &Options::rc_jb}, {"skinny_rc_multi", &Options::rc_shape_multi},
        {"skinny_flat", &Options::skinny_flat}, {"hoist_vproj", &Options::hoist_vproj}, {"attn_lds", &Options::attn_lds}, {"flat_half", &Options::flat_half},
        {"half_min_mts", &Options::half_min_mts}, {"gemm_x3_dma", &Options::gemm_x3_dma}, {"trunk_chain", &Options::trunk_chain}, {"frontend_solo", &Options::frontend_solo}, {"flat_xcd", &Options::flat_xcd}, {"attn_skip0", &Options::attn_skip0}};
    for (auto& t : diag)
        if (!std::strcmp(name, t.name)) { o.*(t.field) = value; return 0; }
#endif
    return 1;
}

struct ProfEntry { std::string name; int64_t launches = 0; double total_ms = 0; std::vector<std::pair<hipEvent_t, hipEvent_t>> pending; };
bool g_prof_on = false;
static std::vector<ProfEntry> g_prof;
static std::map<std::string, int> g_prof_idx;
static thread_local int g_prof_cur = -1;
static thread_local hipEvent_t g_prof_start;
static std::mutex g_prof_mu;

void prof_begin(const char* name, hipStream_t s) {
    if (!g_prof_on) return;
    std::lock_guard<std::mutex> lk(g_prof_mu);
    auto it = g_prof_idx.find(name);
    int idx;
    if (it == g_prof_idx.end()) {
        idx = (int)g_prof.size();
        g_prof.push_back(ProfEntry{name});
        g_prof_idx[name] = idx;
    } else {
        idx = it->second;
    }
    g_prof_cur = idx;
    (void)hipEventCreate(&g_prof_start);
    (void)hipEventRecord(g_prof_start, s);
}
void prof_end(hipStream_t s) {
    if (!g_prof_on || g_prof_cur < 0) return;
    hipEvent_t stop;
    (void)hipEventCreate(&stop);
    (void)hipEventRecord(stop, s);
    std::lock_guard<std::mutex> lk(g_prof_mu);
    g_prof[g_prof_cur].pending.emplace_back(g_prof_start, stop);
    g_prof[g_prof_cur].launches++;
    g_prof_cur = -1;
}
void prof_count(const char* name, int64_t n) {
    if (!g_prof_on) return;
    std::lock_guard<std::mutex> lk(g_prof_mu);
    auto it = g_prof_idx.find(name);
    if (it == g_prof_idx.end()) {
        g_prof_idx[name] = (int)g_prof.size();
        g_prof.push_back(ProfEntry{name});
        it = g_prof_idx.find(name);
    }
    g_prof[it->second].launches += n;
}
static void prof_drain() {
    std::lock_guard<std::mutex> lk(g_prof_mu);
    for (auto& e : g_prof) {
        for (auto& pr : e.pending) {
            (void)hipEventSynchronize(pr.second);
            float ms = 0.f;
            if (hipEventElapsedTime(&ms, pr.first, pr.second) == hipSuccess) e.total_ms += ms;
            (void)hipEventDestroy(pr.first);
            (void)hipEventDestroy(pr.second);
        }
        e.pending.clear();
    }
}

}

namespace l2s {

struct EncPlan {
    int NF, Hp;
    int64_t act_a, act_b, t1, t2, last;
};
static EncPlan enc_plan(int NF, int H) {
    EncPlan p{};
    p.NF = NF;
    p.Hp = H / 4;
    int64_t hw = (int64_t)p.Hp * p.Hp;
    int64_t amax = (int64_t)p.NF * hw * STAGE_CH[0], t1 = 0, t2 = 0;
    int cin = STAGE_CH[0];
    int h = p.Hp;
    for (int st = 0; st < 3; ++st) {
        int cout = STAGE_CH[st + 1], half = cout / 2;
        int ho = (h + 1) / 2;
        int64_t in_px = (int64_t)p.NF * h * h, out_px = (int64_t)p.NF * ho * ho;
        t1 = std::max(t1, std::max(in_px * half, out_px * half));
        t2 = std::max(t2, std::max(out_px * cin, out_px * half));
        amax = std::max(amax, out_px * cout);
        cin = cout;
        h = ho;
    }
    p.act_a = amax; p.act_b = amax; p.t1 = t1; p.t2 = t2;
    p.last = (int64_t)p.NF * h * h * LAST_CH;
    return p;
}
static int64_t enc_ws_floats(int NF, int H) {
    EncPlan p = enc_plan(NF, H);
    return p.act_a + p.act_b + p.t1 + p.t2 + p.last + 64 * 8;
}

static int64_t prologue_ws_floats(int B, int T) {
    int L[4];
    int m = content_lens(T, L);
    int64_t BT = (int64_t)B * T, n = 0;
    n += BT * 4096;
    n += BT * 1024;
    n += BT * 512;
    n += (int64_t)B * 512 * 2;
    n += (int64_t)pad16(B) * 512 * 6;
    n += (int64_t)B * 1024;
    n += BT * 4608;
    for (int j = 0; j < 4; ++j) n += (int64_t)B * L[j] * 512;
    n += (int64_t)B * m * 2560;
    n += (int64_t)B * m * 256 * 4;
    n += (int64_t)B * m * (VOC + VOCP);
    n += 8 * std::max((int64_t)B * m * 256, (int64_t)B * 512);
    for (int j = 1; j < 4; ++j) n += (int64_t)CT_KS[j] * B * L[j] * 512;
    n += 8 * BT * 512;
    if (B <= 2) n += pbilstm_ws_bytes() / 4 + 64;
    return n + 64 * 44;
}
static int64_t decode_ws_floats(int B) {
    int64_t Bp = pad16(B);
    return Bp * (512 * 4 + 512 * 2 + 512 + 256 * 4 + 96) + (int64_t)B * (512 + 256 + 256) + 64 * 24 + (B + 2 + 64)  + (B <= 8 ? pdecode_ws_bytes(B) / 4 + 64 : 0);
}
constexpr int POST_TAPSPLIT_ROWS = 640;
static int64_t postnet_ws_floats(int B, int S) { return (int64_t)B * S * 512 * ((int64_t)B * S <= POST_TAPSPLIT_ROWS * MAX_GROUP ? 9 : 4) + 64 * 7; }


static GemmP pw_gemm(const float* A, int lda, int a_off, const ConvW& c, float* C, int ldc, int c_off, int cstride,
                     int64_t M, int N, int K, int act) {
    GemmP p = gemm_plain(A + a_off, lda, c.W, C + c_off, ldc, (int)M, N, K);
    p.scale = c.scale; p.shift = c.shift; p.actw = c.actw; p.act = act; p.c_cstride = cstride;
    p.W3 = c.W3;
    return p;
}

static FrameSrc frame_src(const float* video, int B) { FrameSrc f{}; f.p[0] = video; f.per = B; return f; }

#define S1_RUN_CHAINED(m, U, run, h) \
    ((m)->opt.trunk_chain && ((h) >= 6 || (m)->opt.trunk_chain >= 2) && (m)->opt.trunk_x3 && (U).pw1_p3 && (U).pw2_p3 && (run) >= 2 && (run) <= S1_CHAIN_MAX)
#ifdef L2S_DIAG
static int enc_tap(float* const* taps, int i, const float* src, int64_t n, hipStream_t s) {
    if (taps && taps[i]) L2S_CHECK_HIP(hipMemcpyAsync(taps[i], src, (size_t)n * sizeof(float), hipMemcpyDeviceToDevice, s));
    return 0;
}
static int enc_tap_interior(int u) {
    set_error("l2s: encoder tap of unit " + std::to_string(u) + " asked for, but the unit is interior to a stage-chain launch and its output never reaches memory (option \"trunk_chain\")");
    return 1;
}
static int enc_taps_check(const l2s_model* m, float* const* taps, int h) {
    if (!taps || !m->opt.fuse_trunk) return 0;
    for (int u = 0; u < N_UNITS; ++u) {
        const UnitW& U = m->w.unit[u];
        if (U.stride2) { h = (h + 1) / 2; continue; }
        int run = 1;
        while (u + run < N_UNITS && !m->w.unit[u + run].stride2 && m->w.unit[u + run].half == U.half) ++run;
        if (!S1_RUN_CHAINED(m, U, run, h)) continue;
        for (int i = 0; i < run - 1; ++i)
            if (taps[1 + u + i]) return enc_tap_interior(u + i);
        u += run - 1;
    }
    return 0;
}
#define L2S_ENC_TAP(i, src, n) do { if (enc_tap(taps, i, src, n, s)) return 1; } while (0)
#define L2S_ENC_TAPS_ARG , float* const* taps = nullptr
#else
#define L2S_ENC_TAP(i, src, n) do {} while (0)
#define L2S_ENC_TAPS_ARG
#endif
static int encoder_run(l2s_model* m, const FrameSrc& video, int B, int T, int H, int W, const float* emb, float* vis,
                       float* feat, void* ws, int64_t ws_bytes, hipStream_t s, const RaggedTab* rg = nullptr L2S_ENC_TAPS_ARG) {
    X3Scope x3scope(m->opt.infer_bf16 ? 0 : m->opt.gemm_x3);
    Bf16Scope bf16scope(m->opt.infer_bf16);
    const Weights& w = m->w;
    EncPlan pl = enc_plan(rg ? rg->NF : B * T, H);
    Bump bp(ws, ws_bytes);
    float* a = bp.f(pl.act_a); float* b = bp.f(pl.act_b); float* t1 = bp.f(pl.t1); float* t2 = bp.f(pl.t2); float* last = bp.f(pl.last);
    L2S_REQUIRE(!bp.overflow, "encoder workspace too small");
#ifdef L2S_DIAG
    if (enc_taps_check(m, taps, pl.Hp)) return 1;
#endif
    FrontendW fe = w.fe;
    if (!m->opt.frontend_x3) fe.w3 = nullptr;
    fe.pair = m->opt.frontend_x3 >= 2; fe.pipe = m->opt.frontend_x3 == 3;
    fe.solo = m->opt.frontend_solo && (m->opt.frontend_solo >= 2 || chains_hint() >= 2);
    if (!m->opt.infer_bf16) fe.w1 = nullptr;
    if (rg ? launch_frontend_ragged(fe, video, *rg, H, W, a, s) : launch_frontend(fe, video, B, T, H, W, a, s)) return 1;
    L2S_ENC_TAP(0, a, (int64_t)pl.NF * pl.Hp * pl.Hp * STAGE_CH[0]);
    float* x = a; float* y = b;
    int h = pl.Hp;
    const int NF = pl.NF;
    for (int u = 0; u < N_UNITS; ++u) {
        const UnitW& U = w.unit[u];
        const int half = U.half, cout = 2 * half;
        if (U.stride2 && m->opt.fuse_trunk && m->opt.fuse_s2) {
            ShuffleS2P sp{};
            sp.x = x; sp.out = y;
            sp.wd1 = U.b1_dw.w9; sp.sd1 = U.b1_dw.scale; sp.bd1 = U.b1_dw.shift;
            sp.wb1f = U.b1_frag; sp.sb1 = U.b1_pw.scale; sp.bb1 = U.b1_pw.shift;
            sp.w1f = U.pw1_frag; sp.s1 = U.pw1.scale; sp.b1 = U.pw1.shift;
            sp.wd = U.dw.w9; sp.sd = U.dw.scale; sp.bd = U.dw.shift;
            sp.w2f = U.pw2_frag; sp.s2 = U.pw2.scale; sp.b2 = U.pw2.shift;
            sp.NF = NF; sp.h = h; sp.ho = (h + 1) / 2; sp.cin = U.cin; sp.half = half; sp.Kin = U.kin; sp.Kh = U.kpad;
            sp.Ro = U.cin == 232 ? 3 : 2;
            if (m->opt.trunk_x3) { sp.wb1p = U.b1_p3; sp.w1p = U.pw1_p3; sp.w2p = U.pw2_p3; }
            if (launch_shuffle_s2(sp, s)) return 1;
            h = sp.ho;
        } else if (U.stride2) {
            const int cin = U.cin, ho = (h + 1) / 2;
            const int64_t in_px = (int64_t)NF * h * h, out_px = (int64_t)NF * ho * ho;
            if (launch_dwconv(x, NF, h, h, cin, 0, cin, 2, U.b1_dw.w9, U.b1_dw.scale, U.b1_dw.shift, t2, cin, 0, s)) return 1;
            if (launch_gemm1(pw_gemm(t2, cin, 0, U.b1_pw, y, cout, 0, 2, out_px, half, cin, ACT_RELU), s, "shuffle_pw_gemm")) return 1;
            if (launch_gemm1(pw_gemm(x, cin, 0, U.pw1, t1, half, 0, 1, in_px, half, cin, ACT_RELU), s, "shuffle_pw_gemm")) return 1;
            if (launch_dwconv(t1, NF, h, h, half, 0, half, 2, U.dw.w9, U.dw.scale, U.dw.shift, t2, half, 0, s)) return 1;
            if (launch_gemm1(pw_gemm(t2, half, 0, U.pw2, y, cout, 1, 2, out_px, half, half, ACT_RELU), s, "shuffle_pw_gemm")) return 1;
            h = ho;
        } else if (m->opt.fuse_trunk) {
            auto s1_params = [&](const UnitW& V, const float* in, float* outp) {
                ShuffleS1P sp{};
                sp.x = in; sp.out = outp;
                sp.w1f = V.pw1_frag; sp.s1 = V.pw1.scale; sp.b1 = V.pw1.shift;
                sp.wd = V.dw.w9; sp.sd = V.dw.scale; sp.bd = V.dw.shift;
                sp.w2f = V.pw2_frag; sp.s2 = V.pw2.scale; sp.b2 = V.pw2.shift;
                sp.NF = NF; sp.h = h; sp.half = V.half; sp.Kpad = V.kpad;
                sp.F = h >= 11 ? 1 : 2;
                if (m->opt.trunk_x3) { sp.w1p = V.pw1_p3; sp.w2p = V.pw2_p3; }
                return sp;
            };
            int run = 1;
            while (u + run < N_UNITS && !w.unit[u + run].stride2 && w.unit[u + run].half == half) ++run;
            if (S1_RUN_CHAINED(m, U, run, h)) {
                ShuffleS1P chain[S1_CHAIN_MAX];
                for (int i = 0; i < run; ++i) chain[i] = s1_params(w.unit[u + i], x, y);
                if (launch_shuffle_s1_chain(chain, run, s)) return 1;
                u += run - 1;
            } else {
                const ShuffleS1P sp = s1_params(U, x, y);
                if (launch_shuffle_s1(sp, s)) return 1;
            }
        } else {
            const int64_t px = (int64_t)NF * h * h;
            if (launch_copy_cols(x, cout, 0, y, cout, 0, 2, px, half, s)) return 1;
            if (launch_gemm1(pw_gemm(x, cout, half, U.pw1, t1, half, 0, 1, px, half, half, ACT_RELU), s, "shuffle_pw_gemm")) return 1;
            if (launch_dwconv(t1, NF, h, h, half, 0, half, 1, U.dw.w9, U.dw.scale, U.dw.shift, t2, half, 0, s)) return 1;
            if (launch_gemm1(pw_gemm(t2, half, 0, U.pw2, y, cout, 1, 2, px, half, half, ACT_RELU), s, "shuffle_pw_gemm")) return 1;
        }
        L2S_ENC_TAP(1 + u, y, (int64_t)NF * h * h * cout);
        std::swap(x, y);
    }
    const int64_t px = (int64_t)NF * h * h;
    {
        GemmP pc = pw_gemm(x, STAGE_CH[3], 0, w.conv_last, last, LAST_CH, 0, 1, px, LAST_CH, STAGE_CH[3], ACT_RELU);
        if (!m->opt.gemm_x3_dma) pc.W3 = nullptr;
        if (launch_gemm1(pc, s, "conv_last_gemm")) return 1;
    }
    L2S_ENC_TAP(N_UNITS + 1, last, px * LAST_CH);
    if (rg) return launch_pool_norm_cat_ragged(last, *rg, h * h, LAST_CH, emb, L2S_D_EMB, vis, L2S_D_VIS, s);
    if (launch_pool_norm_cat(last, NF, h * h, LAST_CH, emb, L2S_D_EMB, T, vis, L2S_D_VIS, feat, s)) return 1;
    return 0;
}

static GemmP conv_gemm(const float* X, int lda, int B, int Tin, int Cin, const ConvW& c, int Cout, int taps, int stride, int pad,
                       float* out, int ldc, int act) {
    const int Tout = (Tin + 2 * pad - taps) / stride + 1;
    GemmP p = gemm_plain(X, lda, c.W, out, ldc, B * Tout, Cout, taps * Cin);
    p.Tout = Tout; p.Tin = Tin; p.taps = taps; p.stride = stride; p.pad = pad; p.Cin = Cin;
    p.scale = c.scale; p.shift = c.shift; p.actw = c.actw; p.act = act;
    p.W3 = c.W3;
    return p;
}

static SkinnyP sk_base(const SkW& sw, int B) {
    SkinnyP p{};
    p.W = sw.W; p.W3 = sw.W3; p.bias = sw.bias; p.actw = sw.actw;
    p.B = B; p.N = sw.N; p.K = sw.K;
    p.act = ACT_NONE; p.epi = SK_PLAIN;
    return p;
}

static int check_lengths(const int32_t* video_lengths, int B, int T) {
    L2S_REQUIRE(video_lengths, "video_lengths is null");
    for (int b = 0; b < B; ++b)
        if (video_lengths[b] < 7 || video_lengths[b] > T) {
            set_error("l2s: video_lengths[" + std::to_string(b) + "] = " + std::to_string(video_lengths[b]) + " is outside [7, T = " + std::to_string(T) + "]");
            return 1;
        }
    return 0;
}
static void masked_bilstm_plan(const int32_t* video_lengths, int B, int T, std::vector<int>& capture, std::vector<int>& reset) {
    capture.clear(); reset.clear();
    for (int b = 0; b < B; ++b) {
        capture.push_back(video_lengths[b] - 1);
        if (video_lengths[b] < T) reset.push_back(T - video_lengths[b]);
    }
    for (std::vector<int>* v : {&capture, &reset}) { std::sort(v->begin(), v->end()); v->erase(std::unique(v->begin(), v->end()), v->end()); }
}
static int64_t len_table_bytes(int B) { return align_up((int64_t)2 * B * (int64_t)sizeof(int), 256); }

static bool persist_envelope(const l2s_model* m, bool masked, int B, int T, int mT) {
    return (!masked || m->opt.persist_masked > 0) && m->opt.persist > 0 && B <= m->opt.persist && !grouped_entry() && pdecode_supported(B, T, mT, m->opt.persist_frames);
}

static int prologue_run(l2s_model* m, const float* vis, const float* emb, const float* gumbel, int B, int T,
                        float* state, float* content_dis, void* ws, int64_t ws_bytes, hipStream_t s, ClipLens lens = {},
                        bool free_running = true) {
    X3Scope x3scope(m->opt.infer_bf16 ? 0 : m->opt.gemm_x3);
    Bf16Scope bf16scope(m->opt.infer_bf16);
    const Weights& w = m->w;
    StateLayout sl = state_layout(B, T);
    int L[4];
    const int mT = content_lens(T, L);
    L2S_REQUIRE(T >= 7 && T <= L2S_MAX_STEPS, "T must be in [7, 300] (Content.agg stride-7 branch; positional table)");
    const int BT = B * T, Bp = pad16(B);
    Bump bp(ws, ws_bytes);
    float* gin = bp.f((int64_t)BT * 4096);
    float* rnn = bp.f((int64_t)BT * 1024);
    float* resid = bp.f((int64_t)BT * 512);
    float* s_e = bp.f((int64_t)B * 512);
    float* s_a = bp.f((int64_t)B * 512);
    float* hf[2][2]; float* cf[2];
    for (int d = 0; d < 2; ++d) { hf[d][0] = bp.f((int64_t)Bp * 512); hf[d][1] = bp.f((int64_t)Bp * 512); cf[d] = bp.f((int64_t)Bp * 512); }
    float* cellcat = bp.f((int64_t)B * 1024);
    float* cat = bp.f((int64_t)BT * 4608);
    float* cmap[4];
    for (int j = 0; j < 4; ++j) cmap[j] = bp.f((int64_t)B * L[j] * 512);
    float* pooled = bp.f((int64_t)B * mT * 2560);
    float* wv = bp.f((int64_t)B * mT * 256);
    float* tA = bp.f((int64_t)B * mT * 256);
    float* tB = bp.f((int64_t)B * mT * 256);
    float* tC = bp.f((int64_t)B * mT * 256);
    float* logits = bp.f((int64_t)B * mT * VOC);
    float* z = bp.f((int64_t)B * mT * VOCP);
    float* part = bp.f(8 * std::max((int64_t)B * mT * 256, (int64_t)B * 512));
    int64_t tap_floats = 0;
    for (int j = 1; j < 4; ++j) tap_floats += (int64_t)CT_KS[j] * B * L[j] * 512;
    float* tap_part = bp.f(tap_floats);
    float* bott_part = bp.f((int64_t)8 * BT * 512);
    const int pgate = (persist_envelope(m, (bool)lens, B, T, mT) && pbilstm_supported(B, T) && (!lens || free_running)) ? pdecode_gate(T) : 0;
    if (pgate < 0) return 1;
    const bool pbi = pgate > 0;
    float* pbx = pbi ? bp.f(pbilstm_ws_bytes() / 4 + 64) : nullptr;
    L2S_REQUIRE(!bp.overflow, "prologue workspace too small");

    {
        GemmP p = gemm_plain(vis, 1024, w.resid.W, resid, 512, BT, 512, 1024);
        p.shift = w.resid.shift;
        if (launch_gemm_splitk(p, 4, bott_part, s, "prologue_gemm")) return 1;
        GemmBatch gb{};
        gb.p[0] = gemm_plain(emb, 256, w.enc_site.W, s_e, 512, B, 512, 256);
        gb.p[0].shift = w.enc_site.shift; gb.p[0].act = ACT_PSINE; gb.p[0].actw = w.enc_site.actw;
        gb.p[1] = gemm_plain(emb, 256, w.attn_site.W, s_a, 512, B, 512, 256);
        gb.p[1].shift = w.attn_site.shift; gb.p[1].act = ACT_PSINE; gb.p[1].actw = w.attn_site.actw;
        gb.count = 2;
        if (launch_gemm(gb, s, "prologue_gemm")) return 1;
    }
    {
        GemmP p = gemm_plain(vis, 1024, w.wih_cat, gin, 4096, BT, 4096, 1024);
        p.shift = w.bih_cat;
        if (m->opt.gemm_x3_dma) p.W3 = w.wih_cat3;
        if (launch_gemm1(p, s, "bilstm_input_gemm")) return 1;
    }
    if (pbi) {
        PBiP q{};
        q.Whh0 = w.whh[0].W; q.Whh1 = w.whh[1].W; q.gin = gin; q.s_e = s_e; q.rnn = rnn; q.h_state = state + sl.h; q.cellcat = cellcat; q.B = B; q.T = T;
        q.lens = lens.dev;
        if (launch_pbilstm(q, pbx, pbilstm_ws_bytes(), s)) return 1;
    } else {
    for (int d = 0; d < 2; ++d) {
        if (launch_to_frag(s_e, 512, B, 512, hf[d][0], 512, 0, 0, s)) return 1;
        if (launch_to_frag(s_e, 512, B, 512, cf[d], 512, 0, 0, s)) return 1;
        if (launch_fill(hf[d][1], (int64_t)Bp * 512, 0.f, s)) return 1;
    }
    std::vector<int> cap_steps, rst_steps;
    size_t cap_i = 0, rst_i = 0;
    if (lens) {
        masked_bilstm_plan(lens.host, B, T, cap_steps, rst_steps);
        if (launch_fill(state + sl.h, (int64_t)Bp * 512, 0.f, s)) return 1;
    }
    for (int step = 0; step < T; ++step) {
        SkinnyBatch sb{};
        const int cur = step & 1, nxt = cur ^ 1;
        if (rst_i < rst_steps.size() && rst_steps[rst_i] == step) {
            ++rst_i;
            if (launch_bilstm_reset(hf[1][cur], cf[1], lens.dev, B, T - 1 - step, s_e, s)) return 1;
        }
        for (int d = 0; d < 2; ++d) {
            const int t = d == 0 ? step : T - 1 - step;
            SkinnyP p = sk_base(w.whh[d], B);
            p.seg[0] = {hf[d][cur], 32}; p.nseg = 1;
            p.epi = SK_LSTM; p.H = 512;
            p.pre = gin + (int64_t)t * 4096 + d * 2048; p.ld_pre = (int64_t)T * 4096;
            p.c_in = cf[d]; p.c_out = cf[d];
            p.h_out = hf[d][nxt]; p.h_out_K = 512; p.h_out_off = 0;
            p.h_seq = rnn + (int64_t)t * 1024 + d * 512; p.ld_hseq = (int64_t)T * 1024;
            sb.p[d] = p; sb.ntiles[d] = w.whh[d].tiles;
        }
        sb.count = 2;
        if (launch_skinny(sb, s, "bilstm_step", m->opt)) return 1;
        if (cap_i < cap_steps.size() && cap_steps[cap_i] == step) {
            ++cap_i;
            if (launch_bilstm_capture(hf[0][nxt], cf[0], lens.dev, B, step, state + sl.h, cellcat, 1024, s)) return 1;
        }
    }
    const int fin = T & 1;
    if (!lens) L2S_CHECK_HIP(hipMemcpyAsync(state + sl.h, hf[0][fin], sizeof(float) * Bp * 512, hipMemcpyDeviceToDevice, s));
    L2S_CHECK_HIP(hipMemcpyAsync(state + sl.h + (int64_t)Bp * 512, hf[1][fin], sizeof(float) * Bp * 512, hipMemcpyDeviceToDevice, s));
    if (!lens && launch_from_frag(cf[0], 512, B, 512, cellcat, 1024, 0, s)) return 1;
    if (launch_from_frag(cf[1], 512, B, 512, cellcat, 1024, 512, s)) return 1;
    }
    {
        GemmP p = gemm_plain(cellcat, 1024, w.e_c.W, state + sl.ecell, 512, B, 512, 1024);
        p.shift = w.e_c.shift;
        if (launch_gemm_splitk(p, 8, part, s, "prologue_gemm")) return 1;
        if (launch_stop_const(state + sl.ecell, w.stop_tail, w.stop_bias, B, state + sl.stopc, s)) return 1;
    }
    {
        GemmP p = gemm_plain(rnn, 1024, w.enc_proj.W, cat, 4608, BT, 512, 1024);
        p.shift = w.enc_proj.shift;
        p.R1 = resid; p.ldr1 = 512; p.r1_mod = 0;
        p.R2 = s_a; p.ldr2 = 512; p.r2_div = T;
        if (launch_gemm_splitk(p, 4, bott_part, s, "prologue_gemm")) return 1;
        if (lens ? launch_mask_copy_rows(cat, 4608, state + sl.enc, 512, lens.dev, B, T, 512, s)
                 : launch_copy_cols(cat, 4608, 0, state + sl.enc, 512, 0, 1, BT, 512, s)) return 1;
    }
    {
        GemmBatch gb{};
        int g = 0;
        for (int j = 3; j >= 0; --j)
            for (int kv = 0; kv < 2; ++kv)
                gb.p[g++] = conv_gemm(cat, 4608, B, T, 512, w.mh_branch[kv][j], 512, MH_KS[j], 1, MH_KS[j] / 2,
                                      cat + 512 + (kv * 4 + j) * 512, 4608, ACT_SILU);
        gb.count = 8;
        if (!m->opt.gemm_x3_dma) for (int i = 0; i < 8; ++i) gb.p[i].W3 = nullptr;
        if (launch_gemm(gb, s, "multihop_conv_gemm")) return 1;
        GemmBatch bb{};
        for (int kv = 0; kv < 2; ++kv) {
            GemmP p = gemm_plain(cat, 4608, w.mh_bott[kv].W, state + (kv == 0 ? sl.k : sl.v), 512, BT, 512, 2560);
            if (kv == 1) { p.a_split = 512; p.a_gap = 2048; }
            p.shift = w.mh_bott[kv].shift; p.act = ACT_PSINE; p.actw = w.mh_bott[kv].actw;
            p.R1 = w.pos; p.ldr1 = 512; p.r1_mod = T;
            bb.p[kv] = p;
        }
        bb.count = 2;
        if (launch_gemm_splitk_group(bb, 4, bott_part, s, "multihop_bottleneck_gemm")) return 1;
        if (w.vproj.W) {
            GemmP p = gemm_plain(state + sl.v, 512, w.vproj.W, state + sl.vp, 256, BT, 256, 512);
            p.shift = w.vproj.shift;
            if (launch_gemm1(p, s, "prologue_gemm")) return 1;
        }
    }
    {
        GemmBatch gb{};
        for (int j = 0; j < 4; ++j)
            gb.p[j] = conv_gemm(cat, 4608, B, T, 512, w.ct_branch[j], 512, CT_KS[j], CT_KS[j], 0, cmap[j], 512, ACT_SILU);
        gb.count = 4;
        if (launch_gemm_tapsplit(gb, tap_part, s, "content_agg_gemm")) return 1;
        PoolCatP pc{};
        pc.x[0] = cat; pc.L[0] = T; pc.ld[0] = 4608;
        for (int j = 0; j < 4; ++j) { pc.x[j + 1] = cmap[j]; pc.L[j + 1] = L[j]; pc.ld[j + 1] = 512; }
        pc.nmaps = 5; pc.B = B; pc.m = mT; pc.C = 512; pc.out = pooled;
        if (lens) {
            PoolDiv pd{};
            pd.div[0] = 1;
            for (int j = 0; j < 4; ++j) pd.div[j + 1] = CT_KS[j];
            if (launch_pool_cat_masked(pc, pd, lens.dev, s)) return 1;
        } else if (launch_pool_cat(pc, s)) return 1;
        const int R = B * mT;
        GemmP p = gemm_plain(pooled, 2560, w.ct_bott.W, wv, 256, R, 256, 2560);
        p.shift = w.ct_bott.shift;
        if (launch_gemm_splitk(p, 8, part, s, "content_gemm")) return 1;
        GemmBatch g1{};
        g1.p[0] = gemm_plain(wv, 256, w.ct_k0.W, tA, 256, R, 256, 256); g1.p[0].shift = w.ct_k0.shift; g1.p[0].act = ACT_SILU;
        g1.p[1] = gemm_plain(wv, 256, w.ct_fc0.W, tB, 256, R, 256, 256); g1.p[1].shift = w.ct_fc0.shift; g1.p[1].act = ACT_SILU;
        g1.count = 2;
        if (launch_gemm(g1, s, "content_gemm")) return 1;
        GemmBatch g2{};
        g2.p[0] = gemm_plain(tA, 256, w.ct_k2.W, state + sl.ckey, 256, R, 256, 256); g2.p[0].shift = w.ct_k2.shift; g2.p[0].act = ACT_SILU;
        g2.p[1] = gemm_plain(tB, 256, w.ct_fc2.W, tC, 256, R, 256, 256); g2.p[1].shift = w.ct_fc2.shift; g2.p[1].act = ACT_SILU;
        g2.count = 2;
        if (launch_gemm(g2, s, "content_gemm")) return 1;
        GemmP p3 = gemm_plain(tC, 256, w.ct_fc4.W, logits, VOC, R, VOC, 256);
        p3.shift = w.ct_fc4.shift; p3.act = ACT_SILU;
        if (launch_gemm1(p3, s, "content_gemm")) return 1;
        if (launch_gumbel_softmax(logits, gumbel, R, VOC, 0.1f, z, VOCP, content_dis, s)) return 1;
        if (lens && launch_zero_slot_rows(z, VOCP, content_dis, VOC, B, mT, lens.dev, s)) return 1;
        GemmP p4 = gemm_plain(z, VOCP, w.ct_emb.W, state + sl.cval, 256, R, 256, VOCP);
        if (launch_gemm1(p4, s, "content_gemm")) return 1;
    }
    if (launch_fill(state + sl.c, (int64_t)Bp * 512 * 2, 0.f, s)) return 1;
    return 0;
}


struct DecodeBufs {
    float *h0[2], *h1[2], *c0, *c1, *av, *p1, *cc, *uu, *yf, *p2f, *q, *qc, *p2;
};

static int decode_launches(l2s_model* m, float* state, int B, int T, int S, const float* teacher, const uint8_t* teacher_mask,
                           float* mel, float* stop, float* attn, int attn_logits, void* ws, int64_t ws_bytes, hipStream_t s, bool fold,
                           const std::function<int(int)>* on_frames = nullptr, bool early = false, ClipLens lens = {}) {
    const Weights& w = m->w;
    StateLayout sl = state_layout(B, T);
    const int Bp = pad16(B);
    const bool vhoist = fold && m->opt.hoist_vproj && w.lstm0v.W && w.vproj.W;
    const bool vsum = vhoist && m->opt.hoist_vproj >= 2 && skinny_sum_supported(m->opt);
    Bump bp(ws, ws_bytes);
    DecodeBufs d;
    for (int i = 0; i < 2; ++i) d.h0[i] = bp.f((int64_t)Bp * 512);
    for (int i = 0; i < 2; ++i) d.h1[i] = bp.f((int64_t)Bp * 512);
// ... 1319 lines not shown
```

### lip2speech_amd/csrc/l2s_common.h

```cpp
#pragma once
#include <hip/hip_runtime.h>
#include <stdint.h>
#include <string>

#define L2S_WAVE 64

typedef float f32x4 __attribute__((ext_vector_type(4)));
typedef float f32x16 __attribute__((ext_vector_type(16)));

struct l2s_resize_job;

namespace l2s {

void set_error(const std::string& msg);
#define L2S_CHECK_HIP(expr)                                                                   \
    do {                                                                                      \
        hipError_t _e = (expr);                                                               \
        if (_e != hipSuccess) {                                                               \
            l2s::set_error(std::string(#expr) + ": " + hipGetErrorString(_e));                \
            return 1;                                                                         \
        }                                                                                     \
    } while (0)
#define L2S_REQUIRE(cond, msg)                                                                \
    do {                                                                                      \
        if (!(cond)) {                                                                        \
            l2s::set_error(std::string("l2s: ") + (msg) + " [" #cond "]");                    \
            return 1;                                                                         \
        }                                                                                     \
    } while (0)

void prof_begin(const char* name, hipStream_t s);
void prof_end(hipStream_t s);
void prof_count(const char* name, int64_t n);
struct ProfScope {
    hipStream_t s;
    ProfScope(const char* name, hipStream_t st) : s(st) { prof_begin(name, st); }
    ~ProfScope() { prof_end(s); }
};

struct Options {
    int fold = 1;
    int graph = 0;
    int overlap_postnet = 0;
    int fuse_trunk = 1;
    int fuse_s2 = 1;
    int trunk_x3 = 1;
    int refresh_map = 0;
    int skinny_static = 0;
    int skinny_sized = 1;
    int skinny_split = 2;
    int skinny_split8 = 1;
    int rc_shape = 0;
    int rc_jb = 0;
    int gemm_x3_dma = 1;
    int lstm_x3 = 4;
    int half_min_mts = 12;
    int flat_half = 1;
    int attn_lds = 1;
    int hoist_vproj = 2;
    int skinny_flat = 1;
    int rc_shape_multi = 0;
    int gemm_x3 = 1;
    int frontend_x3 = 3;
    int train_bf16 = 0;
    int persist = 4;
    int persist_frames = 32;
    int persist_masked = 0;
    int frontend_solo = 0;
    int trunk_chain = 1;
    int flat_xcd = 1;
    int attn_skip0 = 1;
    int early_stop = 0;
    int infer_bf16 = 0;
};
int set_option_field(Options& o, const char* name, int value);

enum Act { ACT_NONE = 0, ACT_RELU = 1, ACT_SILU = 2, ACT_PSINE = 3, ACT_PRELU = 4  };

struct GemmP {
    const float* A;
    const float* W;
    const float* scale;
    const float* shift;
    const float* actw;
    const float* R1;
    const float* R2;
    float* C;
    int M, N, K;
    int lda, Tout, Tin, taps, stride, pad, Cin;
    int a_split, a_gap;
    int act;
    int ldr1, r1_mod, ldr2, r2_mod;
    int r2_div;
    int ldc, c_cstride;
    int c_tr_T;
    float* Zout;
    int win_T, win_off;
    int vec;
    const float* mask;
    int ldmask, mask_pre;
    int ldw;
    const void* W3;
    int x3;
    int x3_group;
    float* stats;
    int stats_raw;
};
inline int64_t gemm_stats_floats(int M, int N) { return (int64_t)((M + 63) / 64) * 2 * N; }
constexpr int GEMM_MAX_GROUP = 8;
struct GemmBatch {
    GemmP p[GEMM_MAX_GROUP];
    int count;
};
GemmP gemm_plain(const float* A, int lda, const float* W, float* C, int ldc, int M, int N, int K);
int& gemm_x3_mode();
int& gemm_x3_group();
struct X3Scope { int prev; explicit X3Scope(int on) : prev(gemm_x3_mode()) { gemm_x3_mode() = on; } ~X3Scope() { gemm_x3_mode() = prev; } };
int& chains_hint();
bool& grouped_entry();
struct X3Group {
    int prev; bool prev_grouped;
    explicit X3Group(int g) : prev(gemm_x3_group()), prev_grouped(grouped_entry()) { gemm_x3_group() = g; grouped_entry() = true; }
    ~X3Group() { gemm_x3_group() = prev; grouped_entry() = prev_grouped; }
};
int& gemm_bf16_mode();
struct Bf16Scope { int prev; explicit Bf16Scope(int on) : prev(gemm_bf16_mode()) { gemm_bf16_mode() = on; } ~Bf16Scope() { gemm_bf16_mode() = prev; } };
bool gemm_x3_eligible(const GemmBatch& b);
bool gemm_x3_member_ok(const GemmP& p);
int64_t gemm_planes_bytes(int N, int K);
int launch_gemm_planes(const float* W, int N, int K, void* planes, hipStream_t s);
int launch_gemm_x3(const GemmBatch& b, hipStream_t s, const char* name);
void gemm_x3_set_timeline(unsigned long long* ts, int block);
int launch_gemm_splitk(const GemmP& p, int ksplit, float* part, hipStream_t s, const char* name);
int launch_gemm_splitk_group(const GemmBatch& g, int ksplit, float* part, hipStream_t s, const char* name);
int launch_gemm_tapsplit(const GemmBatch& convs, float* part, hipStream_t s, const char* name);
int launch_gemm(const GemmBatch& b, hipStream_t s, const char* name);
int launch_gemm_finish(const GemmBatch& b, hipStream_t s, const char* name);
int launch_gemm1(const GemmP& p, hipStream_t s, const char* name);

enum BwdMode { BWD_DX = 0, BWD_DW = 1 };
struct BwdGemmP {
    int mode;
    const float* A; int lda;
    const float* B; int ldb;
    float* C; int ldc;
    int M, N, K;
    int Tx, Tz, taps, stride, pad, padp, Nout, Cin;
    int c_T; int64_t c_seq_stride;
    float alpha; int accumulate;
    int vec;
    int ksplit; int64_t c_split_stride;
};
BwdGemmP bwd_dx(const float* dZ, int ldz, const float* Wp, float* dX, int ldx, int B, int Tz, int Tx, int Nout, int Cin, int taps, int pad, bool accumulate);
BwdGemmP bwd_dw(const float* dZ, int ldz, const float* X, int ldx, float* dWp, int B, int Tz, int Tx, int Nout, int Cin, int taps, int stride, int pad, bool accumulate);
int launch_gemm_bwd(const BwdGemmP& p, hipStream_t s, const char* name);
int64_t gemm_bwd_splitk_floats(const BwdGemmP& p, int splits);
int launch_gemm_bwd_splitk(const BwdGemmP& p, int splits, float* partials, hipStream_t s, const char* name);
int launch_gemm_bwd_dw_dx(const BwdGemmP& pdw, int splits, float* partials, const BwdGemmP& pdx, hipStream_t s, const char* name);

constexpr int AB_RS = 1024;
struct ActBwdP {
    const float* dy; const float* z; float* dconv;
    int ld_dy, ld_z, ld_dconv;
    int64_t rows; int C;
    int act;
    const float* actw;
    const float* scale;
    const float* gamma; const float* beta;
    float* partials;
    int cs_dy, co_dy, cs_z, co_z;
};
int act_bwd(const ActBwdP& p, float* d_shift, float* d_gamma, float* d_actw, float* d_convbias, bool accumulate, hipStream_t s, float* totals = nullptr);

struct BnLayer {
    const float* gamma; const float* beta; float* rmean; float* rvar; const float* conv_bias;
    float* scale; float* shift;
    int C;
};
int bn_stats_finalize(const float* partials, int nblk, int blk_stride, int64_t count, const BnLayer& L, float momentum, hipStream_t s);
int bn_train_fix(float* dconv, int ld_dconv, const float* z, int ld_z, int cs_z, int co_z, const float* gamma, const float* beta, const float* scale,
                 const float* totals, int64_t rows, int C, hipStream_t s);
constexpr int DWS_RS = 1024;
int launch_dwconv_stats(const float* in, int N, int Hi, int Wi, int ldi, int ci_off, int C, int stride, const float* w9, float* partials, hipStream_t s,
                        float* raw_out = nullptr, int ldo = 0, int co_off = 0);
int launch_bn_apply(float* x, int64_t rows, int C, int ld, int co_off, const float* scale, const float* shift, hipStream_t s, bool fused = false);

struct FrontendW {
    const float* w;
    const float* scale;
    const float* shift;
    const float* slope;
    const float* w3;
    int pair = 0;
    int solo = 0;
    int pipe = 0;
    const float* w1;
};
constexpr int MAX_GROUP = 8;
struct FrameSrc { const float* p[MAX_GROUP]; int per; };
int launch_frontend(const FrontendW& w, const FrameSrc& video, int B, int T, int H, int W, float* out, hipStream_t s, float* zout = nullptr);
inline int launch_frontend(const FrontendW& w, const float* video, int B, int T, int H, int W, float* out, hipStream_t s, float* zout = nullptr) {
    FrameSrc f{}; f.p[0] = video; f.per = B;
    return launch_frontend(w, f, B, T, H, W, out, s, zout);
}
struct RaggedClip { int g, row, T, len, frame0, pair0; };
constexpr int RAGGED_CHUNK = 32;
struct RaggedChunk { RaggedClip c[RAGGED_CHUNK]; int n; };
struct RaggedTab { const RaggedClip* clips; const int* pair_clip; int N, Tmax, NF, NP; };
int launch_ragged_table(const RaggedClip* clips_host, int N, RaggedClip* clips_dev, int* pair_clip_dev, hipStream_t s);
int launch_frontend_ragged(const FrontendW& w, const FrameSrc& video, const RaggedTab& rg, int H, int W, float* out, hipStream_t s);
struct EvalClip { int S, T, row, mT, mel_off, stop_off, attn_off, dis_off; };
constexpr int EVAL_CHUNK = 32;
struct EvalChunk { EvalClip c[EVAL_CHUNK]; int n; };
struct EvalTab { const EvalClip* clips; int N, Smax, Tmax, mTmax; };
enum EvalField { EV_STOP = 0, EV_ATTN = 1, EV_DIS = 2, EV_MEL_POST = 3 };
int launch_eval_table(const EvalClip* clips_host, int N, EvalClip* clips_dev, hipStream_t s);
int launch_zero_rows_past_s(float* x, int cols, const EvalTab& ev, hipStream_t s);
int launch_eval_scatter(int field, const float* src, const EvalTab& ev, float* dst, hipStream_t s);
int launch_eval_mel_cf(const float* mel, const EvalTab& ev, float* mel_cf, hipStream_t s);
int launch_frontend_stats(const FrontendW& w, const float* video, int B, int T, int H, int W, float* partials , int* nblocks, hipStream_t s, float* raw_out = nullptr);
int launch_frontend_pool(const float* z, const float* slope, int NF, int Hc, int Wc, float* out, hipStream_t s);

constexpr int MAX_COLLATE_CLIPS = 64;
int launch_normalise_pad(const uint8_t* packed, const int64_t* offsets, const int* frames, int B, int T, int H, int W, float* video, hipStream_t s);
int resize_check(const ::l2s_resize_job* jobs, int n, int64_t packed_bytes, int mode, int B, int T, int oh, int ow);
int launch_resize_normalise(const uint8_t* packed, int64_t packed_bytes, const ::l2s_resize_job* jobs, int n, int mode, int B, int T, int oh, int ow, float* out,
                            hipStream_t s);
int launch_dwconv(const float* in, int N, int Hi, int Wi, int ldi, int ci_off, int C, int stride,
                  const float* w9 , const float* scale, const float* shift,
                  float* out, int ldo, int co_off, hipStream_t s);
struct ShuffleS1P {
    const float* x; float* out;
    const float* w1f; const float* s1; const float* b1;
    const float* wd; const float* sd; const float* bd;
    const float* w2f; const float* s2; const float* b2;
    int NF, h, half, Kpad, F;
    const void* w1p; const void* w2p;
};
int64_t su_planes_bytes(int N, int K);
int launch_su_planes(const float* W, int N, int K, void* out, hipStream_t s);
int launch_shuffle_s1(const ShuffleS1P& p, hipStream_t s);
constexpr int S1_CHAIN_MAX = 7;
int launch_shuffle_s1_chain(const ShuffleS1P* units, int n, hipStream_t s);
void shuffle_set_timeline(unsigned long long* ts, int h);
struct ShuffleS2P {
    const float* x; float* out;
    const float* wd1; const float* sd1; const float* bd1;
    const float* wb1f; const float* sb1; const float* bb1;
    const float* w1f; const float* s1; const float* b1;
    const float* wd; const float* sd; const float* bd;
    const float* w2f; const float* s2; const float* b2;
    int NF, h, ho, cin, half, Kin, Kh, Ro;
    const void* wb1p; const void* w1p; const void* w2p;
};
int launch_shuffle_s2(const ShuffleS2P& p, hipStream_t s);
int launch_copy_cols(const float* in, int ldi, int off_i, float* out, int ldo, int off_o, int cs_o,
                     int64_t rows, int cols, hipStream_t s);
int launch_pool_norm_cat(const float* x, int NF, int P, int C, const float* emb, int E, int T,
                         float* vis, int ldv, float* feat , hipStream_t s);
int launch_pool_norm_cat_ragged(const float* x, const RaggedTab& rg, int P, int C, const float* emb, int E, float* vis, int ldv, hipStream_t s);

__host__ __device__ inline int64_t frag16_index(int row, int k, int K) {
    int rt = row >> 4, i = row & 15, c = k >> 4, g = (k >> 2) & 3, e = k & 3;
    return ((int64_t)(rt * (K >> 4) + c) * 64 + (g * 16 + i)) * 4 + e;
}

enum SkinnyEpi {
    SK_PLAIN = 0,
    SK_FRAG = 1,
    SK_LSTM = 2,
    SK_MEL = 3,
};
struct SkinnySeg { const float* a; int nchunks; };
struct SkinnyP {
    SkinnySeg seg[4];
    int nseg;
    const float* a_sum;
    int layout;
    const float* W;
    const void* W3;
    const float* bias;
    const float* actw;
    const float* add;
    int ld_add;
    const float* addrow;
    float* out;
    int ldo;
    int B, N, K;
    int act;
    int epi;
    const float* pre;
    int64_t ld_pre;
    const float* c_in;
    float* c_out;
    float* h_out;
    int h_out_K, h_out_off;
    float* h_seq;
    int64_t ld_hseq;
    float* h_plain;
    int ld_hplain;
    int H;
    float* mel; int64_t ld_mel_b;
    float* stop; int64_t ld_stop_b;
    const float* stop_const;
    float* yfrag;
    int* es_ctl; int es_end;
};
struct EsCtl { int end_rel; int count; int crossed[1]; };
constexpr int ES_POST_LAYERS = 5, ES_POST_TAPS = 5;
constexpr int ES_MARGIN = ES_POST_LAYERS * (ES_POST_TAPS / 2);
constexpr int SKINNY_MAX_GROUP = 4;
struct SkinnyBatch { SkinnyP p[SKINNY_MAX_GROUP]; int ntiles[SKINNY_MAX_GROUP]; int count; const int* es_end; int es_step; };
#define L2S_ES_RETURN(arg) do { if ((arg).es_end && (arg).es_step >= *(arg).es_end) return; } while (0)
int launch_skinny(const SkinnyBatch& b, hipStream_t s, const char* name, const Options& o = Options());
int launch_skx_planes(const float* Wf, int ntiles, int K, void* out, hipStream_t s);
bool skinny_sum_supported(const Options& o);
void attn_set_timeline(unsigned long long* ts);
void skinny_set_flat_timeline(unsigned long long* ts);
void skinny_set_timeline(unsigned long long* ts);

int launch_probe(int kind, int blocks, int n_per_block, const float* in, float* out, hipStream_t s);
void skinny_set_flat_timeline(unsigned long long* ts);
int set_stamp_log(unsigned long long* log, long long cap);
const void* skinny_form_kernel(const SkinnyBatch& bl, const Options& o, int chains, bool stamped_skinny, bool stamped_flat, dim3& grid, int& block, int& lds);

struct AttnP {
    const float* q; int ldq;
    const float* k;
    const float* v;
    const float* vp;
    const float* tau;
    float* av_frag;
    float* attn_out; int64_t ld_attn_b; int attn_logits;
    const float* qc; int ldqc;
    const float* ckey;
    const float* cval;
    const float* tau_c;
    float* cc_frag;
    int B, T, m;
    const int* es_end; int es_step;
};
int launch_step_attn(const AttnP& at, const SkinnyP& pre2, int pre2_tiles, hipStream_t s, int lds_values = 1, int skip0 = 0);
struct PoolCatP { const float* x[5]; int L[5]; int ld[5]; int nmaps; int B, m, C; float* out; };
int launch_pool_cat(const PoolCatP& p, hipStream_t s);
int launch_gumbel_softmax(const float* logits, const float* gumbel, int rows, int n, float tau,
                          float* z, int ldz, float* dis, hipStream_t s);
int launch_to_frag(const float* x, int ldx, int B, int K, float* frag, int Kfrag, int koff, int broadcast_row, hipStream_t s);
int launch_fill(float* p, int64_t n, float v, hipStream_t s);
int launch_from_frag(const float* frag, int Kfrag, int B, int K, float* out, int ldo, int ooff, hipStream_t s);
int launch_tile_rows(const float* src, int lds, float* dst, int ldd, int B, int T, int C, hipStream_t s);
int launch_transpose_bsc(const float* in, int B, int S, int C, float* out, hipStream_t s);
int launch_output_lengths(const float* stop, int B, int S, int64_t* lengths, hipStream_t s);
int launch_mask_by_lengths(const int64_t* lengths, int B, int S, int T, float* mel_post, float* attn, hipStream_t s);
constexpr int LEN_CHUNK = 64;
struct LenChunk { int len[LEN_CHUNK]; int n; };
int launch_len_table(const int32_t* lens_host, int B, int* table, hipStream_t s);
int launch_bilstm_capture(const float* h_frag, const float* c_frag, const int* lens, int B, int t, float* h_dst_frag, float* c_dst, int ld_c, hipStream_t s);
int launch_bilstm_reset(float* h_frag, float* c_frag, const int* lens, int B, int t, const float* s_e, hipStream_t s);
int launch_mask_copy_rows(float* x, int ldx, float* out, int ldo, const int* lens, int B, int T, int cols, hipStream_t s);
struct PoolDiv { int div[5]; };
int launch_pool_cat_masked(const PoolCatP& p, const PoolDiv& d, const int* lens, hipStream_t s);
int launch_zero_slot_rows(float* z, int ldz, float* dis, int n, int B, int m, const int* lens, hipStream_t s);
int launch_step_attn_masked(const AttnP& at, const SkinnyP& pre2, int pre2_tiles, const int* lens, hipStream_t s, int lds_values = 1, int skip0 = 0);
int launch_frame_window(const float* audio, int B, int N, int L, int n_fft, int hop, const float* window, float* frames, hipStream_t s);
int launch_power(const float* spec, int lds, int64_t rows, int nf, float* power, int ldp, hipStream_t s);
struct SpkRank { int64_t off; int32_t n; int32_t b; };
constexpr int SPK_CHUNK = 512;
struct SpkChunk { int32_t v[SPK_CHUNK]; int n; };
int launch_spk_table(const int32_t* words_host, int64_t n_words, int32_t* table, hipStream_t s);
int launch_frame_window_packed(const float* audio_packed, const SpkRank* ranks, const int* step_row0, int B, int L_max, int n_fft, int hop, const float* window,
                               float* frames, hipStream_t s);
int launch_spk_last_hidden(const float* hseq, const SpkRank* ranks, const int* step_row0, int B, float* h_last, hipStream_t s);
constexpr int IM_MAXF = 576;
constexpr int IM_MAXM = 128;
constexpr int IM_NNZ = 2048;
int launch_mel_bands(const float* fb, int n_freqs, int n_mels, int* tab, float* fwd, float* bwd, hipStream_t s);
int launch_stop_const(const float* ecell, const float* w_tail, const float* bias, int B, float* out, hipStream_t s);

}
```

### lip2speech_amd/native.py

```python
from __future__ import annotations

import collections
import ctypes
import os
import threading
from typing import Dict, Iterable, Optional

import numpy as np
import torch

_HERE = os.path.dirname(os.path.abspath(__file__))
DIAG_LIB_PATH = os.path.join(_HERE, "csrc", "libl2s_diag.so")
LIB_PATH = os.environ.get("L2S_LIB") or os.path.join(_HERE, "csrc", "libl2s_hip.so")
if LIB_PATH == "diag":
    LIB_PATH = DIAG_LIB_PATH

ABI_SYMBOLS = (
    "l2s_abi_version", "l2s_last_error",
    "l2s_model_create", "l2s_model_set_tensor", "l2s_model_finalize", "l2s_model_destroy",
    "l2s_min_T", "l2s_workspace_bytes", "l2s_state_floats", "l2s_state_offset",
    "l2s_mel_frames", "l2s_mel_targets_workspace_bytes", "l2s_mel_targets",
    "l2s_resize_check", "l2s_resize_normalise",
    "l2s_encoder_fwd", "l2s_normalise_pad_frames", "l2s_build_visual", "l2s_decoder_prologue", "l2s_decode_steps", "l2s_postnet",
    "l2s_workspace_bytes_masked", "l2s_masked_bilstm_plan", "l2s_inference_masked", "l2s_forward_eval_masked", "l2s_decoder_prologue_masked", "l2s_decode_steps_masked",
    "l2s_ragged_plan", "l2s_workspace_bytes_ragged", "l2s_inference_ragged",
    "l2s_forward_eval_ragged_plan", "l2s_workspace_bytes_eval_ragged", "l2s_forward_eval_ragged",
    "l2s_output_lengths", "l2s_inference", "l2s_inference_multi", "l2s_workspace_bytes_multi", "l2s_forward_eval", "l2s_forward_eval_multi", "l2s_model_set_option", "l2s_persist_available", "l2s_persist_timeouts", "l2s_set_thread_chains", "l2s_speaker_workspace_bytes", "l2s_speaker_encoder_fwd",
    "l2s_speaker_packed_plan", "l2s_speaker_workspace_bytes_packed", "l2s_speaker_encoder_packed",
    "l2s_face_workspace_bytes", "l2s_face_encoder_fwd",
    "l2s_inverse_mel_workspace_bytes", "l2s_inverse_mel", "l2s_griffin_lim_workspace_bytes", "l2s_griffin_lim", "l2s_estoi_workspace_bytes", "l2s_estoi_workspace_bytes_long", "l2s_estoi",
    "l2s_set_option",
    "l2s_train_scratch_bytes", "l2s_loss", "l2s_grad_norm", "l2s_adamw_amsgrad_step",
    "l2s_train_steps_tape_floats", "l2s_train_steps_weights_floats", "l2s_train_steps_ws_bytes", "l2s_train_steps_pack_weights",
    "l2s_train_steps_fwd", "l2s_train_steps_bwd",
    "l2s_train_set_bn", "l2s_train_refresh_weights", "l2s_train_encoder_tape_floats", "l2s_train_encoder_ws_bytes", "l2s_train_encoder_fwd", "l2s_train_encoder_bwd",
    "l2s_train_prologue_tape_floats", "l2s_train_prologue_ws_bytes", "l2s_train_prologue_fwd", "l2s_train_prologue_bwd",
    "l2s_train_bind", "l2s_train_postnet_tape_floats", "l2s_train_postnet_ws_bytes", "l2s_train_postnet_fwd", "l2s_train_postnet_bwd",
    "l2s_profile_enable", "l2s_profile_reset", "l2s_profile_count", "l2s_profile_get",
)
DIAG_SYMBOLS = (
    "l2s_op_gemm", "l2s_op_conv1d", "l2s_op_gemm_ex", "l2s_op_conv1d_ex", "l2s_op_conv1d_bwd", "l2s_op_frontend", "l2s_op_launch_chain", "l2s_op_launch_chain2", "l2s_op_skinny_timeline", "l2s_op_attn_timeline", "l2s_op_flat_timeline", "l2s_op_pdecode_timeline", "l2s_op_gemm_x3_timeline", "l2s_op_fused_unit_timeline", "l2s_op_lstm_cell_chain", "l2s_op_step_attn_chain", "l2s_op_stamp_log", "l2s_op_skinny_form", "l2s_op_skinny",
    "l2s_op_face_conv2d", "l2s_op_face_taps", "l2s_op_speaker_taps", "l2s_op_speaker_taps_packed", "l2s_op_encoder_taps",
)

DIAG_OPTIONS = frozenset(("overlap_postnet", "fuse_trunk", "fuse_s2", "skinny_static", "skinny_sized", "skinny_split", "skinny_split8", "skinny_rc", "skinny_rc_jb",
                          "skinny_rc_multi", "skinny_flat", "hoist_vproj", "attn_lds", "flat_half", "half_min_mts", "gemm_x3_dma", "flat_xcd", "attn_skip0", "trunk_chain", "frontend_solo"))

ST_K, ST_V, ST_CKEY, ST_CVAL, ST_ECELL, ST_H, ST_C, ST_ENC, ST_STOPC = range(9)

_lib = None
_diag = None
_process_defaults: Dict[str, int] = {}
_vp, _i, _i64, _fp = ctypes.c_void_p, ctypes.c_int, ctypes.c_int64, ctypes.c_void_p


class ResizeJob(ctypes.Structure):
    _fields_ = [("offset", _i64)] + [(k, ctypes.c_int32) for k in ("H", "W", "y0", "x0", "h", "w", "flip", "slot")]


class SkinnyGroup(ctypes.Structure):
    _fields_ = ([("seg_a", _vp * 4)] + [(k, _vp) for k in ("a_sum", "W", "planes", "bias", "actw", "add", "addrow", "out", "pre", "c_in", "c_out", "h_out", "h_seq",
                                                            "h_plain", "mel", "stop", "stop_const", "yfrag")]
                + [(k, _i64) for k in ("ld_pre", "ld_hseq", "ld_mel_b", "ld_stop_b")] + [("nchunks", ctypes.c_int32 * 4)]
                + [(k, ctypes.c_int32) for k in ("ntiles", "epi", "N", "act", "ldo", "ld_add", "H", "h_out_K", "h_out_off", "ld_hplain")])


RESIZE_MOUTH, RESIZE_FACE = 0, 1
RESIZE_JOBS_PER_LAUNCH = 240


def _load(path: str) -> ctypes.CDLL:
    if not os.path.exists(path):
        raise RuntimeError(
            f"native library not built: {path} is missing. Build it with "
            "`python -c 'import __graft_entry__ as g; g.build()'` or `make -C lip2speech_amd/csrc` "
            "(hipcc --offload-arch=gfx950). There is no CPU fallback for the Lip2Speech hot path.")
    L = ctypes.CDLL(path)
    _bind(L)
    if hasattr(L, "l2s_op_gemm"):
        _bind_diag(L)
    return L


def lib() -> ctypes.CDLL:
    global _lib
    if _lib is None:
        _lib = _load(LIB_PATH)
    return _lib


def diag() -> ctypes.CDLL:
    global _diag
    if _diag is None:
        _diag = lib() if hasattr(lib(), "l2s_op_gemm") else _load(DIAG_LIB_PATH)
        if _diag is not _lib:
            for name, value in _process_defaults.items():
                check(_diag.l2s_set_option(name.encode(), value), _diag)
            _replay_thread_chains(_diag)
    return _diag


def _bind(L: ctypes.CDLL) -> None:
    L.l2s_last_error.restype = ctypes.c_char_p
    L.l2s_abi_version.restype = _i
    L.l2s_model_create.argtypes = [ctypes.POINTER(_vp)]
    L.l2s_model_set_tensor.argtypes = [_vp, ctypes.c_char_p, _vp, _i64]
    L.l2s_model_finalize.argtypes = [_vp, _vp]
    L.l2s_model_destroy.argtypes = [_vp]
    L.l2s_min_T.argtypes = [_i]
    L.l2s_workspace_bytes.argtypes = [_i] * 5
    L.l2s_workspace_bytes.restype = _i64
    L.l2s_state_floats.argtypes = [_i, _i]
    L.l2s_state_floats.restype = _i64
    L.l2s_state_offset.argtypes = [_i, _i, _i]
    L.l2s_state_offset.restype = _i64
    L.l2s_encoder_fwd.argtypes = [_vp, _fp, _i, _i, _i, _i, _fp, _vp, _i64, _vp]
    L.l2s_normalise_pad_frames.argtypes = [_vp, ctypes.POINTER(_i64), ctypes.POINTER(ctypes.c_int32), _i, _i, _i, _i, _fp, _vp]
    L.l2s_build_visual.argtypes = [_fp, _fp, _i, _i, _fp, _vp]
    L.l2s_decoder_prologue.argtypes = [_vp, _fp, _fp, _fp, _i, _i, _fp, _fp, _vp, _i64, _vp]
    L.l2s_decode_steps.argtypes = [_vp, _fp, _i, _i, _i, _fp, _vp, _fp, _fp, _fp, _i, _vp, _i64, _vp]
    L.l2s_postnet.argtypes = [_vp, _fp, _i, _i, _fp, _fp, _vp, _i64, _vp]
    L.l2s_output_lengths.argtypes = [_fp, _i, _i, _vp, _vp]
    L.l2s_speaker_workspace_bytes.argtypes = [_i, _i]
    L.l2s_speaker_workspace_bytes.restype = _i64
    L.l2s_speaker_encoder_fwd.argtypes = [_vp, _fp, _i, _i, _fp, _vp, _i64, _vp]
    L.l2s_face_workspace_bytes.argtypes = [_i, _i, _i]
    L.l2s_face_workspace_bytes.restype = _i64
    L.l2s_face_encoder_fwd.argtypes = [_vp, _fp, _i64, _i, _i, _i, _fp, _fp, _vp, _i64, _vp]
    L.l2s_inference.argtypes = [_vp, _fp, _fp, _fp, _i, _i, _i, _i, _i, _fp, _vp, _fp, _vp, _i64, _vp]
    L.l2s_workspace_bytes_multi.argtypes = [_i] * 6
    L.l2s_workspace_bytes_multi.restype = _i64
    L.l2s_inference_multi.argtypes = [_vp, _i, ctypes.POINTER(_vp), ctypes.POINTER(_vp), ctypes.POINTER(_vp), _i, _i, _i, _i, _i, _fp, _vp, _fp, _vp, _i64, _vp]
    L.l2s_forward_eval.argtypes = [_vp, _fp, _fp, _fp, _i, _i, _i, _i, _i, _fp, _vp, _fp, _fp, _fp, _fp, _fp, _vp, _i64, _vp]
    L.l2s_forward_eval_multi.argtypes = [_vp, _i, ctypes.POINTER(_vp), ctypes.POINTER(_vp), ctypes.POINTER(_vp), ctypes.POINTER(_vp), _vp,
                                         _i, _i, _i, _i, _i, _fp, _fp, _fp, _fp, _fp, _vp, _i64, _vp]
    L.l2s_model_set_option.argtypes = [_vp, ctypes.c_char_p, _i]
    L.l2s_set_option.argtypes = [ctypes.c_char_p, _i]
    L.l2s_train_bind.argtypes = [_vp, ctypes.c_char_p, _fp, _fp]
    L.l2s_train_postnet_tape_floats.argtypes = [_i, _i]
    L.l2s_train_postnet_tape_floats.restype = _i64
    L.l2s_train_postnet_ws_bytes.argtypes = [_i, _i]
    L.l2s_train_postnet_ws_bytes.restype = _i64
    L.l2s_train_postnet_fwd.argtypes = [_vp, _fp, _i, _i, _fp, _fp, _fp, _vp]
    L.l2s_train_postnet_bwd.argtypes = [_vp, _fp, _fp, _i, _i, _fp, _fp, _fp, _vp, _i64, _vp]
    L.l2s_train_steps_tape_floats.argtypes = [_i, _i]
    L.l2s_train_steps_tape_floats.restype = _i64
    L.l2s_train_steps_weights_floats.restype = _i64
    L.l2s_train_steps_ws_bytes.argtypes = [_i, _i]
    L.l2s_train_steps_ws_bytes.restype = _i64
    L.l2s_train_steps_pack_weights.argtypes = [_vp, _fp, _vp]
    L.l2s_train_steps_fwd.argtypes = [_vp, _fp, _i, _i, _i, _fp, _vp, _vp, _fp, _fp, _fp, _fp, _fp, _fp, _fp, _vp, _i64, _vp]
    L.l2s_train_steps_bwd.argtypes = [_vp, _fp, _i, _i, _i, _vp, _fp, _fp, _fp, _fp, _fp, _fp, _fp, _fp, _fp, _fp, _fp, _fp, _fp, _fp, _vp, _i64, _vp]
    L.l2s_train_set_bn.argtypes = [_vp, _i, ctypes.c_float]
    L.l2s_train_refresh_weights.argtypes = [_vp, _vp]
    L.l2s_train_encoder_tape_floats.argtypes = [_i, _i, _i]
    L.l2s_train_encoder_tape_floats.restype = _i64
    L.l2s_train_encoder_ws_bytes.argtypes = [_i, _i, _i]
    L.l2s_train_encoder_ws_bytes.restype = _i64
    L.l2s_train_encoder_fwd.argtypes = [_vp, _fp, _i, _i, _i, _i, _fp, _fp, _fp, _fp, _vp]
    L.l2s_train_encoder_bwd.argtypes = [_vp, _fp, _i, _i, _i, _i, _fp, _i, _fp, _vp, _i64, _vp]
    L.l2s_train_prologue_tape_floats.argtypes = [_i, _i]
    L.l2s_train_prologue_tape_floats.restype = _i64
    L.l2s_train_prologue_ws_bytes.argtypes = [_i, _i]
    L.l2s_train_prologue_ws_bytes.restype = _i64
    L.l2s_train_prologue_fwd.argtypes = [_vp, _fp, _fp, _fp, _i, _i, _fp, _fp, _fp, _vp, _i64, _vp]
    L.l2s_train_prologue_bwd.argtypes = [_vp, _fp, _fp, _i, _i, _fp, _fp, _fp, _fp, _fp, _fp, _fp, _fp, _fp, _fp, _fp, _vp, _i64, _vp]
    L.l2s_train_scratch_bytes.restype = _i64
    L.l2s_loss.argtypes = [_fp] * 6 + [_i, _i, _i] + [_fp] * 5 + [_vp, _vp]
    L.l2s_grad_norm.argtypes = [_fp, _i64, _vp, _fp, _vp]
    _f = ctypes.c_float
    L.l2s_adamw_amsgrad_step.argtypes = [_fp] * 5 + [_i64, _f, _f, _f, _f, _f, _i, _fp, _f, _f, _vp]
    L.l2s_inverse_mel_workspace_bytes.argtypes = [_i] * 6
    L.l2s_inverse_mel_workspace_bytes.restype = _i64
    L.l2s_inverse_mel.argtypes = [_fp, _i, _fp, _i, _fp, _i, _i, _i, _i, _i, _i, _fp, _fp, _vp, _vp, _i64, _vp]
    L.l2s_griffin_lim_workspace_bytes.argtypes = [_i, _i]
    L.l2s_griffin_lim_workspace_bytes.restype = _i64
    L.l2s_griffin_lim.argtypes = [_fp, _fp, _i, _i, _i, _i, _i, ctypes.c_float, _fp, _vp, _i64, _vp]
    L.l2s_estoi_workspace_bytes.argtypes = [_i]
    L.l2s_estoi_workspace_bytes.restype = _i64
    L.l2s_estoi.argtypes = [_fp, _fp, _i, _i, _fp, _i, _i, _i, _i, _i, ctypes.POINTER(ctypes.c_int), _fp, _vp, _i64, _vp]
    if hasattr(L, "l2s_estoi_workspace_bytes_long"):
        L.l2s_estoi_workspace_bytes_long.argtypes = [_i, _i]
        L.l2s_estoi_workspace_bytes_long.restype = _i64
    L.l2s_profile_enable.argtypes = [_i]
    L.l2s_profile_get.argtypes = [_i, ctypes.POINTER(ctypes.c_char_p), ctypes.POINTER(_i64), ctypes.POINTER(ctypes.c_double)]
    if hasattr(L, "l2s_inference_masked"):
        _lens = ctypes.POINTER(ctypes.c_int32)
        L.l2s_workspace_bytes_masked.argtypes = [_i] * 5
        L.l2s_workspace_bytes_masked.restype = _i64
        L.l2s_masked_bilstm_plan.argtypes = [_lens, _i, _i, _lens, _lens, ctypes.POINTER(_i), ctypes.POINTER(_i)]
        L.l2s_inference_masked.argtypes = L.l2s_inference.argtypes + [_lens]
        L.l2s_forward_eval_masked.argtypes = L.l2s_forward_eval.argtypes + [_lens]
        L.l2s_decoder_prologue_masked.argtypes = L.l2s_decoder_prologue.argtypes + [_lens]
        L.l2s_decode_steps_masked.argtypes = L.l2s_decode_steps.argtypes + [_lens]
    if hasattr(L, "l2s_inference_ragged"):
        _lens = ctypes.POINTER(ctypes.c_int32)
        L.l2s_ragged_plan.argtypes = [_i, _lens, _lens, _lens, _lens, _lens, ctypes.POINTER(_i), ctypes.POINTER(_i)]
        L.l2s_workspace_bytes_ragged.argtypes = [_i, _lens, _lens, _i, _i, _i]
        L.l2s_workspace_bytes_ragged.restype = _i64
        L.l2s_inference_ragged.argtypes = [_vp, _i, ctypes.POINTER(_vp), ctypes.POINTER(_vp), ctypes.POINTER(_vp), _lens, _lens, _lens, _i, _i, _i, _fp, _vp, _fp,
                                           _vp, _i64, _vp]
    if hasattr(L, "l2s_forward_eval_ragged"):
        _lens, _offs = ctypes.POINTER(ctypes.c_int32), ctypes.POINTER(_i64)
        L.l2s_forward_eval_ragged_plan.argtypes = [_i, _lens, _lens, _lens, _offs, _offs, _offs, _offs, ctypes.POINTER(_i), ctypes.POINTER(_i), ctypes.POINTER(_i)]
        L.l2s_workspace_bytes_eval_ragged.argtypes = [_i, _lens, _lens, _lens, _i, _i]
        L.l2s_workspace_bytes_eval_ragged.restype = _i64
        L.l2s_forward_eval_ragged.argtypes = [_vp, _i, ctypes.POINTER(_vp), ctypes.POINTER(_vp), ctypes.POINTER(_vp), _lens, _lens, _lens, _lens, _i, _i,
                                              _fp, _fp, _fp, _fp, _fp, _vp, _i64, _vp]
    if hasattr(L, "l2s_mel_targets"):
        L.l2s_mel_frames.argtypes = [_i64]
        L.l2s_mel_frames.restype = _i
        L.l2s_mel_targets_workspace_bytes.argtypes = [_i, _i]
        L.l2s_mel_targets_workspace_bytes.restype = _i64
        L.l2s_mel_targets.argtypes = [_fp, ctypes.POINTER(_i64), ctypes.POINTER(_i64), _i, _fp, _i, _i, _i, _i, _i, ctypes.c_float, _i, _i64, _fp, _fp, _fp, _vp,
                                      _vp, _i64, _vp]
    if hasattr(L, "l2s_resize_normalise"):
        _jobs = ctypes.POINTER(ResizeJob)
        L.l2s_resize_check.argtypes = [_jobs, _i, _i64, _i, _i, _i, _i, _i]
        L.l2s_resize_normalise.argtypes = [_vp, _i64, _jobs, _i, _i, _i, _i, _i, _i, _fp, _vp]
    if hasattr(L, "l2s_speaker_encoder_packed"):
        _lens, _ns = ctypes.POINTER(ctypes.c_int32), ctypes.POINTER(_i64)
        L.l2s_speaker_packed_plan.argtypes = [_ns, _i, _lens, _lens, _lens, ctypes.POINTER(_i), ctypes.POINTER(_i64)]
        L.l2s_speaker_workspace_bytes_packed.argtypes = [_ns, _i]
        L.l2s_speaker_workspace_bytes_packed.restype = _i64
        L.l2s_speaker_encoder_packed.argtypes = [_vp, _fp, _ns, _ns, _i, _fp, _vp, _i64, _vp]


def _bind_diag(L: ctypes.CDLL) -> None:
    L.l2s_op_gemm.argtypes = [_fp, _fp, _fp, _fp, _fp, _fp, _i, _i, _i, _i, _vp]
    L.l2s_op_conv1d.argtypes = [_fp, _fp, _fp, _fp, _fp, _fp, _i, _i, _i, _i, _i, _i, _i, _i, _vp]
    L.l2s_op_gemm_ex.argtypes = [_fp, _fp, _fp, _fp, _fp, _fp, _i, _i, _i, _i, _i, _vp]
    L.l2s_op_conv1d_ex.argtypes = [_fp, _fp, _fp, _fp, _fp, _fp, _i, _i, _i, _i, _i, _i, _i, _i, _i, _vp]
    L.l2s_op_conv1d_bwd.argtypes = [_fp, _fp, _fp, _fp, _fp, _i, _i, _i, _i, _i, _i, _i, _vp]
    L.l2s_op_frontend.argtypes = [_vp, _fp, _i, _i, _i, _i, _fp, _vp]
    L.l2s_op_launch_chain.argtypes = [_i, _i, _i, _i, _fp, _fp, _vp]
    L.l2s_op_skinny_timeline.argtypes = [_vp]
    L.l2s_op_attn_timeline.argtypes = [_vp]
    L.l2s_op_flat_timeline.argtypes = [_vp]
    L.l2s_op_pdecode_timeline.argtypes = [_vp, ctypes.c_int]
    L.l2s_op_gemm_x3_timeline.argtypes = [_vp, ctypes.c_int]
    L.l2s_op_fused_unit_timeline.argtypes = [_vp, _i]
    L.l2s_op_launch_chain2.argtypes = [_i, _i, _i, _i, _fp, _fp, _vp, _vp]
    L.l2s_op_step_attn_chain.argtypes = [_vp, _fp, _i, _i, _i, _vp, _i64, _vp]
    L.l2s_op_lstm_cell_chain.argtypes = [_vp, _i, _i, _vp, _i64, _vp, ctypes.POINTER(ctypes.c_double)]
    L.l2s_op_stamp_log.argtypes = [_vp, _i64]
    L.l2s_op_skinny_form.argtypes = [_vp, _i, ctypes.POINTER(ctypes.c_int), _i, _i, _i, _i, ctypes.c_char_p, _i]
    L.l2s_op_skinny.argtypes = [_vp, _i, ctypes.POINTER(SkinnyGroup), _i, _vp, _i, _vp]
    L.l2s_op_face_conv2d.argtypes = [_fp, _i64, _i, _i, _i, _i, _fp, _fp, _fp, _fp, _i, _fp, _i, _i, _i, _i, _i, _i, _vp]
    L.l2s_op_face_taps.argtypes = [_vp, _fp, _i64, _i, _vp, _fp, _fp, _vp, _i64, _vp]
    L.l2s_op_speaker_taps.argtypes = [_vp, _fp, _i, _i, _vp, _fp, _vp, _i64, _vp]
    L.l2s_op_speaker_taps_packed.argtypes = [_vp, _fp, ctypes.POINTER(_i64), ctypes.POINTER(_i64), _i, _vp, _fp, _vp, _i64, _vp]
    L.l2s_op_encoder_taps.argtypes = [_vp, _fp, _i, _i, _i, _i, _vp, _fp, _vp, _i64, _vp]


def check(rc: int, L: Optional[ctypes.CDLL] = None) -> None:
    if rc != 0:
        raise RuntimeError("libl2s_hip: " + (L or lib()).l2s_last_error().decode("utf-8", "replace"))


def _dcheck(rc: int) -> None:
    check(rc, diag())


def _stream() -> int:
    return torch.cuda.current_stream().cuda_stream


def _ptr(t: Optional[torch.Tensor]) -> Optional[int]:
    if t is None:
        return None
    assert t.is_cuda and t.is_contiguous(), "device-resident contiguous tensors only"
    return t.data_ptr()


def _f32(t: torch.Tensor) -> torch.Tensor:
    if not t.is_cuda:
        raise RuntimeError("the Lip2Speech hot path runs on the GPU: move inputs to cuda (no CPU fallback)")
    return t.detach().to(torch.float32).contiguous()


def min_T(T: int) -> int:
    return int(lib().l2s_min_T(T))


def video_lengths_array(video_lengths, B: int, T: int):
    if isinstance(video_lengths, torch.Tensor):
        if video_lengths.is_floating_point() or video_lengths.is_complex() or video_lengths.dtype == torch.bool:
            raise TypeError(f"video_lengths must hold integers, got {video_lengths.dtype}")
        arr = video_lengths.detach().cpu().numpy()
    else:
        arr = np.asarray(video_lengths)
        if arr.dtype.kind not in "iu":
            raise TypeError(f"video_lengths must hold integers, got {arr.dtype}")
    if arr.shape != (B,):
        raise ValueError(f"video_lengths must have shape ({B},) - one length per clip - got {tuple(arr.shape)}")
    bad = [(b, int(v)) for b, v in enumerate(arr) if v < 7 or v > T]
    if bad:
        raise ValueError(f"video_lengths outside [7, T = {T}]: " + ", ".join(f"clip {b}: {v}" for b, v in bad))
    return (ctypes.c_int32 * B)(*[int(v) for v in arr])


def masked_bilstm_plan(video_lengths, T: int):
    B = len(video_lengths)
    lens = (ctypes.c_int32 * B)(*[int(v) for v in video_lengths])
    cap, rst = (ctypes.c_int32 * B)(), (ctypes.c_int32 * B)()
    nc, nr = _i(), _i()
    check(lib().l2s_masked_bilstm_plan(lens, B, int(T), cap, rst, ctypes.byref(nc), ctypes.byref(nr)))
    return list(cap[:nc.value]), list(rst[:nr.value])


def workspace_bytes_ragged(batch_B, batch_T, H: int = 96, W: int = 96, S: int = 300) -> int:
    G, i32 = len(batch_B), ctypes.c_int32
    need = int(lib().l2s_workspace_bytes_ragged(G, (i32 * G)(*[int(b) for b in batch_B]), (i32 * G)(*[int(t) for t in batch_T]), H, W, S))
    if need < 0:
        check(1)
    return need


MAX_GROUP = 8
MAX_RAGGED_CLIPS = 256


def ragged_plan(batch_B, batch_T, video_lengths):
    G = len(batch_B)
    flat = [int(v) for v in video_lengths] if not (len(video_lengths) and hasattr(video_lengths[0], "__len__")) else [int(v) for b in video_lengths for v in b]
    n = sum(int(b) for b in batch_B)
    if len(flat) != n:
        raise ValueError(f"video_lengths must hold {n} lengths (sum of batch_B), got {len(flat)}")
    i32 = ctypes.c_int32
    f0, p0 = (i32 * (n + 1))(), (i32 * (n + 1))()
    N, Tmax = _i(), _i()
    check(lib().l2s_ragged_plan(G, (i32 * G)(*[int(b) for b in batch_B]), (i32 * G)(*[int(t) for t in batch_T]), (i32 * max(n, 1))(*flat), f0, p0,
                                ctypes.byref(N), ctypes.byref(Tmax)))
    return list(f0[:N.value + 1]), list(p0[:N.value + 1]), N.value, Tmax.value


def _i32s(vals):
    vals = [int(v) for v in vals]
    return (ctypes.c_int32 * max(len(vals), 1))(*vals)


def forward_eval_ragged_plan(batch_B, batch_T, batch_S):
    G = len(batch_B)
    if len(batch_T) != G or len(batch_S) != G:
        raise ValueError(f"batch_B, batch_T and batch_S hold one entry per batch ({G}), got {len(batch_T)} and {len(batch_S)}")
    offs = [(_i64 * (G + 1))() for _ in range(4)]
    N, Tmax, Smax = _i(), _i(), _i()
    check(lib().l2s_forward_eval_ragged_plan(G, _i32s(batch_B), _i32s(batch_T), _i32s(batch_S), *offs, ctypes.byref(N), ctypes.byref(Tmax), ctypes.byref(Smax)))
    return tuple(list(o) for o in offs) + (N.value, Tmax.value, Smax.value)
# ... 984 lines not shown
```

Baseline: 3.641 million mel-frames/s.

## Prefetch shuffle-unit stride-2 weights and BN params into registers ahead of use

```diff
diff --git a/lip2speech_amd/csrc/encoder_kernels.hip b/lip2speech_amd/csrc/encoder_kernels.hip
--- a/lip2speech_amd/csrc/encoder_kernels.hip
+++ b/lip2speech_amd/csrc/encoder_kernels.hip
@@ -819,9 +819,49 @@
     static constexpr int NT = (N + 15) / 16, MG = (MT + G - 1) / G, ITEMS = NT * MG, IT = (ITEMS + 7) / 8;
 };
 
-template <class GM, int LDA>
+struct SuNone {};
+template <class T> constexpr bool su_none = std::is_same<T, SuNone>::value;
+template <class GM, int NB>
+struct SuGemmHeld {
+    static constexpr int NBH = NB;
+    float sc[GM::IT], sh[GM::IT];
+    uint4 b[GM::IT][NB > 0 ? NB : 1][3];
+};
+template <class GM, int NB>
+__device__ __forceinline__ void su_request_bn(SuGemmHeld<GM, NB>& o, const float* __restrict__ scale, const float* __restrict__ shift) {
+    const int li = threadIdx.x & 15;
+    const int wave = __builtin_amdgcn_readfirstlane(threadIdx.x >> 6);
+#pragma unroll
+    for (int it = 0; it < GM::IT; ++it) {
+        const int n = min((wave + 8 * it) % GM::NT * 16 + li, GM::N - 1);
+        o.sc[it] = scale[n];
+        o.sh[it] = shift[n];
+    }
+}
+template <class GM, int NCH, int NB>
+__device__ __forceinline__ void su_request_w(SuGemmHeld<GM, NB>& o, const uint4* __restrict__ Wp) {
+    const int lane = threadIdx.x & 63;
+    const int wave = __builtin_amdgcn_readfirstlane(threadIdx.x >> 6);
+#pragma unroll
+    for (int it = 0; it < GM::IT; ++it) {
+        const int item = wave + 8 * it;
+        if (GM::ITEMS % 8 == 0 || item < GM::ITEMS) {
+            const uint4* wb = Wp + (int64_t)(item % GM::NT) * NCH * 192 + lane;
+#pragma unroll
+            for (int c = 0; c < NB; ++c) {
+#pragma unroll
+                for (int q = 0; q < 3; ++q) o.b[it][c][q] = wb[(c * 3 + q) * 64];
+            }
+        }
+    }
+}
+template <class GM> __device__ __forceinline__ void su_request_bn(SuNone&, const float*, const float*) {}
+template <class GM, int NCH> __device__ __forceinline__ void su_request_w(SuNone&, const uint4*) {}
+
+template <class GM, int LDA, class HELD = SuNone, class MID = SuNone>
 __device__ __forceinline__ void su_gemm(float* __restrict__ buf, const float* __restrict__ Wf,
-                                        const float* __restrict__ scale, const float* __restrict__ shift) {
+                                        const float* __restrict__ scale, const float* __restrict__ shift,
+                                        const HELD& held = HELD(), const MID& mid = MID()) {
     constexpr int NC = GM::NC, G = GM::G, IT = GM::IT, NT = GM::NT;
     const int lane = threadIdx.x & 63;
     const int wave = __builtin_amdgcn_readfirstlane(threadIdx.x >> 6);
@@ -851,6 +891,7 @@
             }
         }
     }
+    if constexpr (!su_none<MID>) mid();
     __syncthreads();
 #pragma unroll
     for (int it = 0; it < IT; ++it) {
@@ -860,7 +901,9 @@
             const int mt0 = min(mg * G, GM::MT - G);
             const int n = nt * 16 + li;
             if (n < GM::N) {
-                const float sc = scale[n], sh = shift[n];
+                float sc, sh;
+                if constexpr (su_none<HELD>) { sc = scale[n]; sh = shift[n]; }
+                else { sc = held.sc[it]; sh = held.sh[it]; }
 #pragma unroll
                 for (int j = 0; j < G; ++j) {
 #pragma unroll
@@ -1096,9 +1139,10 @@
     return 0;
 }
 
-template <class GM, int NCH, int PITCH, int PLANE, int LDA, bool OPQ = false>
+template <class GM, int NCH, int PITCH, int PLANE, int LDA, bool OPQ = false, class HELD = SuNone, class MID = SuNone>
 __device__ __forceinline__ void su_gemm_x3(unsigned char* __restrict__ pl, const uint4* __restrict__ Wp,
-                                           const float* __restrict__ scale, const float* __restrict__ shift, int mrows = 1 << 30) {
+                                           const float* __restrict__ scale, const float* __restrict__ shift, int mrows = 1 << 30,
+                                           const HELD& held = HELD(), const MID& mid = MID()) {
     constexpr int G = GM::G, IT = GM::IT, NT = GM::NT, BD = NCH <= 4 ? NCH : 3;
     int tx = threadIdx.x;
     if constexpr (OPQ) asm volatile("" : "+v"(tx));
@@ -1121,7 +1165,10 @@
 #pragma unroll
             for (int c = 0; c < BD; ++c) {
 #pragma unroll
-                for (int q = 0; q < 3; ++q) b[c][q] = wb[(c * 3 + q) * 64];
+                for (int q = 0; q < 3; ++q) {
+                    if constexpr (su_none<HELD>) b[c][q] = wb[(c * 3 + q) * 64];
+                    else b[c][q] = c < HELD::NBH ? held.b[it][c < HELD::NBH ? c : 0][q] : wb[(c * 3 + q) * 64];
+                }
             }
 #pragma unroll
             for (int c = 0; c < NCH; ++c) {
@@ -1149,6 +1196,7 @@
             }
         }
     }
+    if constexpr (!su_none<MID>) mid();
     __syncthreads();
 #pragma unroll
     for (int it = 0; it < IT; ++it) {
@@ -1158,7 +1206,9 @@
             const int mt0 = min(mg * G, GM::MT - G);
             const int n = nt * 16 + li;
             if (n < GM::N) {
-                const float sc = scale[n], sh = shift[n];
+                float sc, sh;
+                if constexpr (su_none<HELD>) { sc = scale[n]; sh = shift[n]; }
+                else { sc = held.sc[it]; sh = held.sh[it]; }
 #pragma unroll
                 for (int j = 0; j < G; ++j) {
 #pragma unroll
@@ -1658,9 +1708,36 @@
     static_assert(CIN % 4 == 0 && CIN <= HALF, "float4 tile rows; pw1 runs in place over the input tile");
 };
 
-template <int H, int HO, int LDA, int CN, int PITCH = 0, int PLANE = 0>
+template <int CN, bool TAPS>
+struct SuDwHeld {
+    static constexpr bool HAS_TAPS = TAPS;
+    static constexpr int V = CN > 64 ? 2 : 1, JC = (CN + 64 * V - 1) / (64 * V);
+    typedef float vec2 __attribute__((ext_vector_type(2)));
+    using vec = typename std::conditional<(CN > 64), vec2, float>::type;
+    vec wk[JC][TAPS ? 9 : 1], s[JC], b[JC];
+};
+template <int CN, bool TAPS>
+__device__ __forceinline__ void su_request_dw(SuDwHeld<CN, TAPS>& o, const float* __restrict__ w9, const float* __restrict__ sc, const float* __restrict__ sh) {
+    using O = SuDwHeld<CN, TAPS>;
+    using vec = typename O::vec;
+    const int lane = threadIdx.x & 63;
+#pragma unroll
+    for (int jc = 0; jc < O::JC; ++jc) {
+        const int c = min(O::V * (lane + 64 * jc), CN - O::V);
+        if constexpr (TAPS) {
+#pragma unroll
+            for (int t = 0; t < 9; ++t) o.wk[jc][t] = *reinterpret_cast<const vec*>(w9 + t * CN + c);
+        }
+        o.s[jc] = *reinterpret_cast<const vec*>(sc + c);
+        o.b[jc] = *reinterpret_cast<const vec*>(sh + c);
+    }
+}
+__device__ __forceinline__ void su_request_dw(SuNone&, const float*, const float*, const float*) {}
+
+template <int H, int HO, int LDA, int CN, int PITCH = 0, int PLANE = 0, class HELD = SuNone>
 __device__ __forceinline__ void su_dw_s2(const float* __restrict__ src, float* __restrict__ dst, int iy0, int outv,
-                                         const float* __restrict__ w9, const float* __restrict__ sc, const float* __restrict__ sh) {
+                                         const float* __restrict__ w9, const float* __restrict__ sc, const float* __restrict__ sh,
+                                         const HELD& held = HELD()) {
     const int lane = threadIdx.x & 63;
     const int wave = __builtin_amdgcn_readfirstlane(threadIdx.x >> 6);
     if constexpr (CN > 64) {
@@ -1670,10 +1747,15 @@
         for (int jc = 0; jc < (CN + 127) / 128; ++jc) {
             const int c = 2 * lane + 128 * jc;
             if (c < CN) {
-                su_f2 wk[9];
-#pragma unroll
-                for (int t = 0; t < 9; ++t) wk[t] = *reinterpret_cast<const su_f2*>(w9 + t * CN + c);
-                const su_f2 s = *reinterpret_cast<const su_f2*>(sc + c), b = *reinterpret_cast<const su_f2*>(sh + c);
+                su_f2 wk[9], s, b;
+#pragma unroll
+                for (int t = 0; t < 9; ++t) {
+                    if constexpr (su_none<HELD>) wk[t] = *reinterpret_cast<const su_f2*>(w9 + t * CN + c);
+                    else if constexpr (HELD::HAS_TAPS) wk[t] = held.wk[jc][t];
+                    else wk[t] = *reinterpret_cast<const su_f2*>(w9 + t * CN + c);
+                }
+                if constexpr (su_none<HELD>) { s = *reinterpret_cast<const su_f2*>(sc + c); b = *reinterpret_cast<const su_f2*>(sh + c); }
+                else { s = held.s[jc]; b = held.b[jc]; }
                 const su_f2 zero2 = {0.f, 0.f};
                 for (int m = wave; m < outv; m += 8) {
                     const int oyl = m / HO, ox = m - oyl * HO;
@@ -1706,10 +1788,15 @@
     for (int jc = 0; jc < (CN + 63) / 64; ++jc) {
         const int c = lane + 64 * jc;
         if (c < CN) {
-            float wk[9];
-#pragma unroll
-            for (int t = 0; t < 9; ++t) wk[t] = w9[t * CN + c];
-            const float s = sc[c], b = sh[c];
+            float wk[9], s, b;
+#pragma unroll
+            for (int t = 0; t < 9; ++t) {
+                if constexpr (su_none<HELD> || CN > 64) wk[t] = w9[t * CN + c];
+                else if constexpr (HELD::HAS_TAPS) wk[t] = held.wk[jc][t];
+                else wk[t] = w9[t * CN + c];
+            }
+            if constexpr (su_none<HELD> || CN > 64) { s = sc[c]; b = sh[c]; }
+            else { s = held.s[jc]; b = held.b[jc]; }
             for (int m = wave; m < outv; m += 8) {
                 const int oyl = m / HO, ox = m - oyl * HO;
                 float acc = 0.f;
@@ -1738,11 +1825,32 @@
     }
 }
 
+constexpr int s2_ahead(bool taps, bool late_top, int nb1, int nb2, int nb3, bool w3_late = false, int waves = 4) {
+    return 1 | taps << 1 | late_top << 2 | w3_late << 3 | nb1 << 4 | nb2 << 8 | nb3 << 12 | (waves - 4) << 16;
+}
+template <int AHEAD>
+struct S2Ahead {
+    static constexpr bool ON = AHEAD & 1, TAPS = AHEAD >> 1 & 1, LATE_TOP = AHEAD >> 2 & 1, W3_LATE = AHEAD >> 3 & 1;
+    static constexpr int NB1 = AHEAD >> 4 & 7, NB2 = AHEAD >> 8 & 7, NB3 = AHEAD >> 12 & 7, WAVES = 4 + (AHEAD >> 16 & 7);
+    template <class T> using held = typename std::conditional<ON, T, SuNone>::type;
+};
+
 #define S2_STAMP(k) do { if (TIMED && threadIdx.x == 0) ts[(blockIdx.y * gridDim.x + blockIdx.x) * 10 + (k)] = wall_clock64(); } while (0)
-template <int H, int CIN, int HALF, int RO, bool TIMED>
-__global__ __launch_bounds__(512, 4) void shuffle_s2_kernel(const ShuffleS2P p, unsigned long long* __restrict__ ts) {
+template <int H, int CIN, int HALF, int RO, bool TIMED, int AHEAD>
+__global__ __launch_bounds__(512, S2Ahead<AHEAD>::WAVES) void shuffle_s2_kernel(const ShuffleS2P p, unsigned long long* __restrict__ ts) {
     using Q = S2Geo<H, CIN, HALF, RO>;
+    using A = S2Ahead<AHEAD>;
     constexpr int HO = Q::HO, KIN = Q::KIN, KH = Q::KH, LDA = Q::LDA, MTI = Q::MTI, MTO = Q::MTO, CIN4 = CIN / 4;
+    typename A::template held<SuDwHeld<CIN, A::TAPS>> d1o;
+    typename A::template held<SuDwHeld<HALF, A::TAPS>> d2o;
+    typename A::template held<SuGemmHeld<typename Q::G1, 0>> g1o;
+    typename A::template held<SuGemmHeld<typename Q::G2, 0>> g2o;
+    typename A::template held<SuGemmHeld<typename Q::G3, 0>> g3o;
+    const auto request_late = [&]() {
+        su_request_dw(d2o, p.wd, p.sd, p.bd);
+        su_request_bn<typename Q::G2>(g2o, p.sb1, p.bb1);
+        su_request_bn<typename Q::G3>(g3o, p.s2, p.b2);
+    };
     extern __shared__ __attribute__((aligned(16))) float su_smem[];
     const int tid = threadIdx.x, lane = tid & 63;
     const int wave = __builtin_amdgcn_readfirstlane(tid >> 6);
@@ -1767,6 +1875,10 @@
         const int idx = tid + 512 * i;
         xin[i] = idx < n4 ? src4[idx] : make_float4(0.f, 0.f, 0.f, 0.f);
     }
+    su_request_dw(d1o, p.wd1, p.sd1, p.bd1);
+    su_request_bn<typename Q::G1>(g1o, p.s1, p.b1);
+    if constexpr (A::LATE_TOP) request_late();
+    const auto at_mid = [&]() { if constexpr (!A::LATE_TOP) request_late(); };
 #pragma unroll
     for (int i = 0; i < NLD; ++i) {
         const int idx = tid + 512 * i;
@@ -1790,16 +1902,16 @@
     S2_STAMP(1);
     __syncthreads();
     S2_STAMP(2);
-    su_dw_s2<H, HO, LDA, CIN>(X, D1, iy0, outv, p.wd1, p.sd1, p.bd1);
+    su_dw_s2<H, HO, LDA, CIN>(X, D1, iy0, outv, p.wd1, p.sd1, p.bd1, d1o);
     S2_STAMP(3);
-    su_gemm<typename Q::G1, LDA>(X, p.w1f, p.s1, p.b1);
+    su_gemm<typename Q::G1, LDA>(X, p.w1f, p.s1, p.b1, g1o, at_mid);
     S2_STAMP(4);
-    su_dw_s2<H, HO, LDA, HALF>(X, D2, iy0, outv, p.wd, p.sd, p.bd);
+    su_dw_s2<H, HO, LDA, HALF>(X, D2, iy0, outv, p.wd, p.sd, p.bd, d2o);
     __syncthreads();
     S2_STAMP(5);
-    su_gemm<typename Q::G2, LDA>(D1, p.wb1f, p.sb1, p.bb1);
+    su_gemm<typename Q::G2, LDA>(D1, p.wb1f, p.sb1, p.bb1, g2o);
     S2_STAMP(6);
-    su_gemm<typename Q::G3, LDA>(D2, p.w2f, p.s2, p.b2);
+    su_gemm<typename Q::G3, LDA>(D2, p.w2f, p.s2, p.b2, g3o);
     S2_STAMP(7);
     float* ob = p.out + ((int64_t)f * HO + oy0) * (HO * 2 * HALF);
     for (int m = wave; m < outv; m += 8) {
@@ -1833,10 +1945,24 @@
     using G2 = SuGemm<HALF, 1, MTO>;
 };
 
-template <int H, int CIN, int HALF, int RO, bool TIMED>
-__global__ __launch_bounds__(512, 4) void shuffle_s2x_kernel(const ShuffleS2P p, unsigned long long* __restrict__ ts) {
+template <int H, int CIN, int HALF, int RO, bool TIMED, int AHEAD>
+__global__ __launch_bounds__(512, S2Ahead<AHEAD>::WAVES) void shuffle_s2x_kernel(const ShuffleS2P p, unsigned long long* __restrict__ ts) {
     using Q = S2XGeo<H, CIN, HALF, RO>;
-    constexpr int HO = Q::HO, LDA = Q::LDA, CIN4 = CIN / 4, PIN = Q::PIN, PH = Q::PH;
+    using A = S2Ahead<AHEAD>;
+    constexpr int HO = Q::HO, LDA = Q::LDA, CIN4 = CIN / 4, PIN = Q::PIN, PH = Q::PH, NCI = Q::KI32 / 32, NCH = Q::KH32 / 32;
+    typename A::template held<SuDwHeld<CIN, A::TAPS>> d1o;
+    typename A::template held<SuDwHeld<HALF, A::TAPS>> d2o;
+    typename A::template held<SuGemmHeld<typename Q::G1, A::NB1>> g1o;
+    typename A::template held<SuGemmHeld<typename Q::G2, A::NB2>> g2o;
+    typename A::template held<SuGemmHeld<typename Q::G2, A::NB3>> g3o;
+    const auto request_late = [&]() {
+        su_request_dw(d2o, p.wd, p.sd, p.bd);
+        su_request_bn<typename Q::G2>(g2o, p.sb1, p.bb1);
+        su_request_bn<typename Q::G2>(g3o, p.s2, p.b2);
+        su_request_w<typename Q::G2, NCI>(g2o, reinterpret_cast<const uint4*>(p.wb1p));
+        if constexpr (!A::W3_LATE) su_request_w<typename Q::G2, NCH>(g3o, reinterpret_cast<const uint4*>(p.w2p));
+    };
+    const auto at_mid_b1 = [&]() { if constexpr (A::W3_LATE) su_request_w<typename Q::G2, NCH>(g3o, reinterpret_cast<const uint4*>(p.w2p)); };
     extern __shared__ __attribute__((aligned(16))) float su_smem[];
     const int tid = threadIdx.x, lane = tid & 63;
     const int wave = __builtin_amdgcn_readfirstlane(tid >> 6);
@@ -1865,6 +1991,11 @@
         const int idx = tid + 512 * i;
         xin[i] = idx < n4 ? src4[idx] : make_float4(0.f, 0.f, 0.f, 0.f);
     }
+    su_request_dw(d1o, p.wd1, p.sd1, p.bd1);
+    su_request_bn<typename Q::G1>(g1o, p.s1, p.b1);
+    su_request_w<typename Q::G1, NCI>(g1o, reinterpret_cast<const uint4*>(p.w1p));
+    if constexpr (A::LATE_TOP) request_late();
+    const auto at_mid = [&]() { if constexpr (!A::LATE_TOP) request_late(); };
     for (int idx = tid; idx < (3 * Q::D1PLANE + 3 * Q::D2PLANE + Q::TAIL) / 16; idx += 512) reinterpret_cast<uint4*>(D2P)[idx] = make_uint4(0u, 0u, 0u, 0u);
 #pragma unroll
     for (int i = 0; i < NLD; ++i) {
@@ -1877,7 +2008,7 @@
     S2_STAMP(1);
     __syncthreads();
     S2_STAMP(2);
-    su_dw_s2<H, HO, LDA, CIN, PIN, Q::D1PLANE>(X, D1, iy0, outv, p.wd1, p.sd1, p.bd1);
+    su_dw_s2<H, HO, LDA, CIN, PIN, Q::D1PLANE>(X, D1, iy0, outv, p.wd1, p.sd1, p.bd1, d1o);
     __syncthreads();
 #pragma unroll
     for (int i = 0; i < NLD; ++i) {
@@ -1905,14 +2036,14 @@
     }
     S2_STAMP(3);
     __syncthreads();
-    su_gemm_x3<typename Q::G1, Q::KI32 / 32, PIN, Q::XPLANE, LDA>(XP, reinterpret_cast<const uint4*>(p.w1p), p.s1, p.b1);
+    su_gemm_x3<typename Q::G1, NCI, PIN, Q::XPLANE, LDA, false>(XP, reinterpret_cast<const uint4*>(p.w1p), p.s1, p.b1, 1 << 30, g1o, at_mid);
     S2_STAMP(4);
-    su_dw_s2<H, HO, LDA, HALF, PH, Q::D2PLANE>(X, D2, iy0, outv, p.wd, p.sd, p.bd);
+    su_dw_s2<H, HO, LDA, HALF, PH, Q::D2PLANE>(X, D2, iy0, outv, p.wd, p.sd, p.bd, d2o);
     __syncthreads();
     S2_STAMP(5);
-    su_gemm_x3<typename Q::G2, Q::KI32 / 32, PIN, Q::D1PLANE, LDA>(D1P, reinterpret_cast<const uint4*>(p.wb1p), p.sb1, p.bb1, Q::RV);
+    su_gemm_x3<typename Q::G2, NCI, PIN, Q::D1PLANE, LDA, false>(D1P, reinterpret_cast<const uint4*>(p.wb1p), p.sb1, p.bb1, Q::RV, g2o, at_mid_b1);
     S2_STAMP(6);
-    su_gemm_x3<typename Q::G2, Q::KH32 / 32, PH, Q::D2PLANE, LDA>(D2P, reinterpret_cast<const uint4*>(p.w2p), p.s2, p.b2, Q::RV);
+    su_gemm_x3<typename Q::G2, NCH, PH, Q::D2PLANE, LDA, false>(D2P, reinterpret_cast<const uint4*>(p.w2p), p.s2, p.b2, Q::RV, g3o);
     S2_STAMP(7);
     float* ob = p.out + ((int64_t)f * HO + oy0) * (HO * 2 * HALF);
     for (int m = wave; m < outv; m += 8) {
@@ -1930,65 +2061,73 @@
     if (TIMED) { __builtin_amdgcn_s_waitcnt(0); S2_STAMP(8); }
 }
 
-template <int H, int CIN, int HALF, int RO>
+template <int H, int CIN, int HALF, int RO, int AHEAD>
 static int launch_s2x_inst(const ShuffleS2P& p, hipStream_t s) {
     using Q = S2XGeo<H, CIN, HALF, RO>;
     static_assert(Q::SMEM <= 80 * 1024, "two blocks per CU");
     static bool attr_set = false;
     if (!attr_set) {
-        L2S_CHECK_HIP(hipFuncSetAttribute(reinterpret_cast<const void*>(shuffle_s2x_kernel<H, CIN, HALF, RO, false>),
+        L2S_CHECK_HIP(hipFuncSetAttribute(reinterpret_cast<const void*>(shuffle_s2x_kernel<H, CIN, HALF, RO, false, AHEAD>),
                                           hipFuncAttributeMaxDynamicSharedMemorySize, (int)Q::SMEM));
 #ifdef L2S_DIAG
-        L2S_CHECK_HIP(hipFuncSetAttribute(reinterpret_cast<const void*>(shuffle_s2x_kernel<H, CIN, HALF, RO, true>),
+        L2S_CHECK_HIP(hipFuncSetAttribute(reinterpret_cast<const void*>(shuffle_s2x_kernel<H, CIN, HALF, RO, true, AHEAD>),
                                           hipFuncAttributeMaxDynamicSharedMemorySize, (int)Q::SMEM));
 #endif
         attr_set = true;
     }
 #ifdef L2S_DIAG
-    if (g_su_ts && g_su_ts_h == -H) hipLaunchKernelGGL((shuffle_s2x_kernel<H, CIN, HALF, RO, true>), dim3(Q::B::STRIPS, p.NF), dim3(512), Q::SMEM, s, p, g_su_ts);
+    if (g_su_ts && g_su_ts_h == -H) hipLaunchKernelGGL((shuffle_s2x_kernel<H, CIN, HALF, RO, true, AHEAD>), dim3(Q::B::STRIPS, p.NF), dim3(512), Q::SMEM, s, p, g_su_ts);
     else
 #endif
-    hipLaunchKernelGGL((shuffle_s2x_kernel<H, CIN, HALF, RO, false>), dim3(Q::B::STRIPS, p.NF), dim3(512), Q::SMEM, s, p, (unsigned long long*)nullptr);
+    hipLaunchKernelGGL((shuffle_s2x_kernel<H, CIN, HALF, RO, false, AHEAD>), dim3(Q::B::STRIPS, p.NF), dim3(512), Q::SMEM, s, p, (unsigned long long*)nullptr);
     return 0;
 }
 
-template <int H, int CIN, int HALF, int RO>
+template <int H, int CIN, int HALF, int RO, int AHEAD>
 static int launch_s2_inst(const ShuffleS2P& p, hipStream_t s) {
     using Q = S2Geo<H, CIN, HALF, RO>;
     static_assert(Q::SMEM <= 80 * 1024, "two blocks per CU");
     static bool attr_set = false;
     if (!attr_set) {
-        L2S_CHECK_HIP(hipFuncSetAttribute(reinterpret_cast<const void*>(shuffle_s2_kernel<H, CIN, HALF, RO, false>),
+        L2S_CHECK_HIP(hipFuncSetAttribute(reinterpret_cast<const void*>(shuffle_s2_kernel<H, CIN, HALF, RO, false, AHEAD>),
                                           hipFuncAttributeMaxDynamicSharedMemorySize, (int)Q::SMEM));
 #ifdef L2S_DIAG
-        L2S_CHECK_HIP(hipFuncSetAttribute(reinterpret_cast<const void*>(shuffle_s2_kernel<H, CIN, HALF, RO, true>),
+        L2S_CHECK_HIP(hipFuncSetAttribute(reinterpret_cast<const void*>(shuffle_s2_kernel<H, CIN, HALF, RO, true, AHEAD>),
                                           hipFuncAttributeMaxDynamicSharedMemorySize, (int)Q::SMEM));
 #endif
         attr_set = true;
     }
 #ifdef L2S_DIAG
-    if (g_su_ts && g_su_ts_h == -H) hipLaunchKernelGGL((shuffle_s2_kernel<H, CIN, HALF, RO, true>), dim3(Q::STRIPS, p.NF), dim3(512), Q::SMEM, s, p, g_su_ts);
+    if (g_su_ts && g_su_ts_h == -H) hipLaunchKernelGGL((shuffle_s2_kernel<H, CIN, HALF, RO, true, AHEAD>), dim3(Q::STRIPS, p.NF), dim3(512), Q::SMEM, s, p, g_su_ts);
     else
 #endif
-    hipLaunchKernelGGL((shuffle_s2_kernel<H, CIN, HALF, RO, false>), dim3(Q::STRIPS, p.NF), dim3(512), Q::SMEM, s, p, (unsigned long long*)nullptr);
+    hipLaunchKernelGGL((shuffle_s2_kernel<H, CIN, HALF, RO, false, AHEAD>), dim3(Q::STRIPS, p.NF), dim3(512), Q::SMEM, s, p, (unsigned long long*)nullptr);
     return 0;
 }
 
-int launch_shuffle_s2(const ShuffleS2P& p, hipStream_t s) {
+constexpr int S2_AHEAD_ST2 = s2_ahead(true, false, 1, 1, 2, true);
+constexpr int S2_AHEAD_ST3 = s2_ahead(true, false, 0, 0, 4, true, 5);
+constexpr int S2_AHEAD_ST4 = s2_ahead(true, false, 0, 0, 0);
+#ifdef L2S_DIAG
+#define S2_FORM(fn, H, CIN, HALF, RO, A) (ahead ? fn<H, CIN, HALF, RO, A>(p, s) : fn<H, CIN, HALF, RO, 0>(p, s))
+#else
+#define S2_FORM(fn, H, CIN, HALF, RO, A) fn<H, CIN, HALF, RO, A>(p, s)
+#endif
+int launch_shuffle_s2(const ShuffleS2P& p, hipStream_t s, int ahead) {
     L2S_REQUIRE(p.Kin == su_pad16(p.cin) && p.Kh == su_pad16(p.half) && p.ho == (p.h + 1) / 2, "shuffle_s2: fragment packing / geometry mismatch");
     L2S_REQUIRE((reinterpret_cast<uintptr_t>(p.x) & 15u) == 0, "shuffle_s2 input must be 16-byte aligned");
     ProfScope ps(p.cin == 24 ? "shuffle_unit_s2_fused_st2" : p.cin == 116 ? "shuffle_unit_s2_fused_st3" : "shuffle_unit_s2_fused_st4", s);
     int rc = 1;
     const bool x3 = p.w1p && p.w2p && p.wb1p && p.cin != 232;
-    if (x3 && p.h == 24 && p.cin == 24 && p.half == 58) rc = launch_s2x_inst<24, 24, 58, 2>(p, s);
-    else if (x3 && p.h == 22 && p.cin == 24 && p.half == 58) rc = launch_s2x_inst<22, 24, 58, 2>(p, s);
-    else if (x3 && p.h == 12 && p.cin == 116 && p.half == 116) rc = launch_s2x_inst<12, 116, 116, 2>(p, s);
-    else if (x3 && p.h == 11 && p.cin == 116 && p.half == 116) rc = launch_s2x_inst<11, 116, 116, 2>(p, s);
-    else if (p.h == 24 && p.cin == 24 && p.half == 58) rc = launch_s2_inst<24, 24, 58, 2>(p, s);
-    else if (p.h == 22 && p.cin == 24 && p.half == 58) rc = launch_s2_inst<22, 24, 58, 2>(p, s);
-    else if (p.h == 12 && p.cin == 116 && p.half == 116) rc = launch_s2_inst<12, 116, 116, 2>(p, s);
-    else if (p.h == 11 && p.cin == 116 && p.half == 116) rc = launch_s2_inst<11, 116, 116, 2>(p, s);
-    else if (p.h == 6 && p.cin == 232 && p.half == 232) rc = launch_s2_inst<6, 232, 232, 3>(p, s);
+    if (x3 && p.h == 24 && p.cin == 24 && p.half == 58) rc = S2_FORM(launch_s2x_inst, 24, 24, 58, 2, S2_AHEAD_ST2);
+    else if (x3 && p.h == 22 && p.cin == 24 && p.half == 58) rc = S2_FORM(launch_s2x_inst, 22, 24, 58, 2, S2_AHEAD_ST2);
+    else if (x3 && p.h == 12 && p.cin == 116 && p.half == 116) rc = S2_FORM(launch_s2x_inst, 12, 116, 116, 2, S2_AHEAD_ST3);
+    else if (x3 && p.h == 11 && p.cin == 116 && p.half == 116) rc = S2_FORM(launch_s2x_inst, 11, 116, 116, 2, S2_AHEAD_ST3);
+    else if (p.h == 24 && p.cin == 24 && p.half == 58) rc = launch_s2_inst<24, 24, 58, 2, 0>(p, s);
+    else if (p.h == 22 && p.cin == 24 && p.half == 58) rc = launch_s2_inst<22, 24, 58, 2, 0>(p, s);
+    else if (p.h == 12 && p.cin == 116 && p.half == 116) rc = launch_s2_inst<12, 116, 116, 2, 0>(p, s);
+    else if (p.h == 11 && p.cin == 116 && p.half == 116) rc = launch_s2_inst<11, 116, 116, 2, 0>(p, s);
+    else if (p.h == 6 && p.cin == 232 && p.half == 232) rc = S2_FORM(launch_s2_inst, 6, 232, 232, 3, S2_AHEAD_ST4);
     else set_error("shuffle_s2: unsupported unit geometry");
     if (rc) return 1;
     L2S_CHECK_HIP(hipGetLastError());
diff --git a/lip2speech_amd/csrc/l2s_api.hip b/lip2speech_amd/csrc/l2s_api.hip
--- a/lip2speech_amd/csrc/l2s_api.hip
+++ b/lip2speech_amd/csrc/l2s_api.hip
@@ -44,7 +44,7 @@
         {"skinny_static", &Options::skinny_static}, {"skinny_sized", &Options::skinny_sized}, {"skinny_split", &Options::skinny_split},
         {"skinny_split8", &Options::skinny_split8}, {"skinny_rc", &Options::rc_shape}, {"skinny_rc_jb", &Options::rc_jb}, {"skinny_rc_multi", &Options::rc_shape_multi},
         {"skinny_flat", &Options::skinny_flat}, {"hoist_vproj", &Options::hoist_vproj}, {"attn_lds", &Options::attn_lds}, {"flat_half", &Options::flat_half},
-        {"half_min_mts", &Options::half_min_mts}, {"gemm_x3_dma", &Options::gemm_x3_dma}, {"trunk_chain", &Options::trunk_chain}, {"frontend_solo", &Options::frontend_solo}, {"flat_xcd", &Options::flat_xcd}, {"attn_skip0", &Options::attn_skip0}};
+        {"half_min_mts", &Options::half_min_mts}, {"gemm_x3_dma", &Options::gemm_x3_dma}, {"trunk_chain", &Options::trunk_chain}, {"s2_ahead", &Options::s2_ahead}, {"frontend_solo", &Options::frontend_solo}, {"flat_xcd", &Options::flat_xcd}, {"attn_skip0", &Options::attn_skip0}};
     for (auto& t : diag)
         if (!std::strcmp(name, t.name)) { o.*(t.field) = value; return 0; }
 #endif
@@ -251,7 +251,7 @@
             sp.NF = NF; sp.h = h; sp.ho = (h + 1) / 2; sp.cin = U.cin; sp.half = half; sp.Kin = U.kin; sp.Kh = U.kpad;
             sp.Ro = U.cin == 232 ? 3 : 2;
             if (m->opt.trunk_x3) { sp.wb1p = U.b1_p3; sp.w1p = U.pw1_p3; sp.w2p = U.pw2_p3; }
-            if (launch_shuffle_s2(sp, s)) return 1;
+            if (launch_shuffle_s2(sp, s, m->opt.s2_ahead)) return 1;
             h = sp.ho;
         } else if (U.stride2) {
             const int cin = U.cin, ho = (h + 1) / 2;
diff --git a/lip2speech_amd/csrc/l2s_common.h b/lip2speech_amd/csrc/l2s_common.h
--- a/lip2speech_amd/csrc/l2s_common.h
+++ b/lip2speech_amd/csrc/l2s_common.h
@@ -68,6 +68,7 @@
     int persist_masked = 0;
     int frontend_solo = 0;
     int trunk_chain = 1;
+    int s2_ahead = 1;
     int flat_xcd = 1;
     int attn_skip0 = 1;
     int early_stop = 0;
@@ -253,7 +254,7 @@
     int NF, h, ho, cin, half, Kin, Kh, Ro;
     const void* wb1p; const void* w1p; const void* w2p;
 };
-int launch_shuffle_s2(const ShuffleS2P& p, hipStream_t s);
+int launch_shuffle_s2(const ShuffleS2P& p, hipStream_t s, int ahead = 1);
 int launch_copy_cols(const float* in, int ldi, int off_i, float* out, int ldo, int off_o, int cs_o,
                      int64_t rows, int cols, hipStream_t s);
 int launch_pool_norm_cat(const float* x, int NF, int P, int C, const float* emb, int E, int T,
diff --git a/lip2speech_amd/native.py b/lip2speech_amd/native.py
--- a/lip2speech_amd/native.py
+++ b/lip2speech_amd/native.py
@@ -44,7 +44,7 @@
 )
 
 DIAG_OPTIONS = frozenset(("overlap_postnet", "fuse_trunk", "fuse_s2", "skinny_static", "skinny_sized", "skinny_split", "skinny_split8", "skinny_rc", "skinny_rc_jb",
-                          "skinny_rc_multi", "skinny_flat", "hoist_vproj", "attn_lds", "flat_half", "half_min_mts", "gemm_x3_dma", "flat_xcd", "attn_skip0", "trunk_chain", "frontend_solo"))
+                          "skinny_rc_multi", "skinny_flat", "hoist_vproj", "attn_lds", "flat_half", "half_min_mts", "gemm_x3_dma", "flat_xcd", "attn_skip0", "trunk_chain", "frontend_solo", "s2_ahead"))
 
 ST_K, ST_V, ST_CKEY, ST_CVAL, ST_ECELL, ST_H, ST_C, ST_ENC, ST_STOPC = range(9)
 
```

After: 3.639 million mel-frames/s. About the same (-0.1%).
